# kiva12138/MIMRL

Hardware: AMD Instinct MI355X
Metric: two-stage train iters/sec (higher is better)
Workload: dtype bf16

## Files before the change

include/mimrl.h:

```cpp
#ifndef MIMRL_H_
#define MIMRL_H_

#include <stdint.h>

#ifdef __cplusplus
extern "C" {
#endif

#define MIMRL_ABI_VERSION 6
#define MIMRL_MAX_BLOCKS 4
#define MIMRL_MAX_BATCH 2048
#define MIMRL_MAX_BATCH_CONCAT 1024

enum { MIMRL_OK = 0, MIMRL_ERR_ARG = -1, MIMRL_ERR_HIP = -2, MIMRL_ERR_STATE = -3, MIMRL_ERR_NODEVICE = -4 };
enum { MIMRL_GROUP_MAIN = 0, MIMRL_GROUP_CRITIC = 1 };
enum { MIMRL_CRITIC_SEPARATE = 0, MIMRL_CRITIC_CONCAT = 1 };
enum { MIMRL_BOUND_INFONCE = 0, MIMRL_BOUND_NWJ, MIMRL_BOUND_TUBA, MIMRL_BOUND_DV, MIMRL_BOUND_JS_FGAN,
       MIMRL_BOUND_JS, MIMRL_BOUND_SMILE, MIMRL_BOUND_MINE, MIMRL_BOUND_INTERPOLATE };
enum { MIMRL_ACT_NONE = 0, MIMRL_ACT_RELU = 1, MIMRL_ACT_GELU = 2, MIMRL_ACT_TANH = 3 };
enum { MIMRL_PREC_FP32 = 0, MIMRL_PREC_BF16_GEMM_FWD = 1, MIMRL_PREC_BF16_GEMM_BWD = 2, MIMRL_PREC_BF16_GRU_FWD = 4,
       MIMRL_PREC_BF16_GRU_BWD = 8, MIMRL_PREC_BF16 = 15 };

enum { MIMRL_BASELINE_CONSTANT = 0, MIMRL_BASELINE_GAUSSAIN = 1, MIMRL_BASELINE_UNNORMALIZED = 2 };
enum { MIMRL_ENCODER_GRU = 0, MIMRL_ENCODER_CONV = 1, MIMRL_ENCODER_LSTM = 2 };
enum { MIMRL_TASK_LOSS_MAE = 0, MIMRL_TASK_LOSS_MSE = 1, MIMRL_TASK_LOSS_RMSE = 2, MIMRL_TASK_LOSS_SIMSE = 3, MIMRL_TASK_LOSS_CCC = 4 };

typedef struct mimrl_cfg {
  int32_t batch;
  int32_t seq_len;
  int32_t time_len;
  int32_t d_t, d_a, d_v;
  int32_t d_common;
  int32_t n_blocks;
  int32_t d_hiddens[MIMRL_MAX_BLOCKS][3];
  int32_t d_outs[MIMRL_MAX_BLOCKS][3];
  int32_t res_project[MIMRL_MAX_BLOCKS];
  int32_t bias, ln_first;
  int32_t activation;
  int32_t compose_t_sum, compose_k_sum;
  int32_t critic_type, bound_type;
  int32_t cmi_hardtanh;
  int32_t k_neighbor;
  int32_t bank_capacity;
  float dropout[4];
  float dropout_mlp[3];
  float coef1[11];
  float coef2[8];
  float weight_decay, grad_clip;
  float beta1, beta2, adam_eps;
  int32_t precision;
  int32_t use_graph;
  int32_t device_anchors;
  int32_t baseline_type;
  int32_t encoder;
  uint64_t seed;
} mimrl_cfg;

typedef struct mimrl_buffers {
  float *main_p, *main_g, *main_m, *main_v;
  float *crit_p, *crit_g, *crit_m, *crit_v;
  const float *text, *audio, *video, *labels;
  const float *bank_c, *bank_f, *bank_t, *bank_a, *bank_v;
  int32_t* anchors;
  float *lr_main, *lr_critic;
  float *pred;
  float *feats;
  float *scalars;
  const int32_t* knn_override;
  int32_t* counters;
} mimrl_buffers;

enum {
  MIMRL_S1_LOSS = 0,
  MIMRL_S1_MIS = 1,
  MIMRL_S1_LOSSES = 12,
  MIMRL_S2_LOSS = 32,
  MIMRL_S2_TASK = 33,
  MIMRL_S2_MIS = 34,
  MIMRL_S2_LOSSES = 42,
  MIMRL_NSCALARS = 64
};

const char* mimrl_last_error(void);
int mimrl_abi_version(void);
int mimrl_deterministic(void);
int mimrl_device_check(void);

int mimrl_layout_count(const mimrl_cfg* cfg);
int mimrl_layout_entry(const mimrl_cfg* cfg, int idx, char* name, int name_cap, int* group, int64_t* offset, int* ndim,
                       int* dim0, int* dim1);
int mimrl_layout_entry_dim2(const mimrl_cfg* cfg, int idx);
int64_t mimrl_bucket_floats(const mimrl_cfg* cfg, int group);

typedef struct mimrl_handle mimrl_handle;
int mimrl_create(const mimrl_cfg* cfg, void* hip_stream, mimrl_handle** out);
int mimrl_bind(mimrl_handle* h, const mimrl_buffers* bufs);
int mimrl_set_bank_rows(mimrl_handle* h, int rows);
int mimrl_set_inputs(mimrl_handle* h, int set, const float* text, const float* audio, const float* video, const float* labels);
int mimrl_stage1_pipe_prime(mimrl_handle* h);
int mimrl_stage1_pipe(mimrl_handle* h, int next_valid);
int mimrl_stage1_step(mimrl_handle* h);
int mimrl_stage2_step(mimrl_handle* h);
int mimrl_two_stage_step(mimrl_handle* h);
int mimrl_stage_grads(mimrl_handle* h, int stage);
int mimrl_stage_apply(mimrl_handle* h, int stage);
int mimrl_stage_grads_part(mimrl_handle* h, int stage, int part);
int mimrl_forward(mimrl_handle* h, int train_mode, int with_losses);
int mimrl_estimate(mimrl_handle* h, int stage);
int mimrl_set_stage2_prefetch(mimrl_handle* h, int on);
int mimrl_stage2_forward_tail(mimrl_handle* h);
int mimrl_set_grad_scale(mimrl_handle* h, float scale);
int mimrl_params_changed(mimrl_handle* h);
int64_t mimrl_workspace_bytes(const mimrl_handle* h);
enum { MIMRL_PH_GEMM_MISC = 0, MIMRL_PH_GRU_FWD, MIMRL_PH_GRU_BWD, MIMRL_PH_CUBE_FWD, MIMRL_PH_CUBE_BWD, MIMRL_PH_EST_FWD,
       MIMRL_PH_EST_BWD, MIMRL_PH_OPT, MIMRL_PH_MODEL_MISC, MIMRL_NPHASES };
int mimrl_profile_enable(mimrl_handle* h, int on);
int mimrl_set_kernel_stamps(mimrl_handle* h, unsigned long long* ring, int slots);
int mimrl_comm_unique_id(void* out128);
int mimrl_set_comm(mimrl_handle* h, const void* unique_id128, int world, int rank);
int64_t mimrl_main_late_offset(const mimrl_handle* h);
int mimrl_set_comm_critic_bf16(mimrl_handle* h, int on);
int mimrl_set_task_loss(mimrl_handle* h, int kind);
int mimrl_profile_read(mimrl_handle* h, float* ms_sum , int32_t* launches );
int mimrl_profile_read_gemm(mimrl_handle* h, double out[4]);
void mimrl_destroy(mimrl_handle* h);

int mimrl_op_gemm(void* stream, const float* A, const float* B, float* C, int M, int N, int K, int batch,
                  const int64_t strides[9] , const float* bias_n,
                  const float* bias_m, float alpha, float beta, int act, int precision);
int mimrl_op_gemm_ex(void* stream, const float* A, const float* B, float* C, int M, int N, int K, int batch, const int64_t strides[9],
                     const float* A2, const float* B2, int K2, const int64_t strides2[6], int a_gap_at, int a_gap_rows,
                     const float* bias_n, const float* gradact_u, float* colsum, int act, int precision);
int mimrl_op_gemm16(void* stream, const void* A, const void* B, void* C, int M, int N, int K, int batch, const int64_t strides[9],
                    const void* A2, const void* B2, int K2, const int64_t strides2[6], int batch_in, const int64_t strides_bo[5],
                    const float* bias_n, int flags);
int mimrl_op_gemm_wgrad_group(void* stream, int n, const float* const* A, const float* const* B, float* const* C, const int32_t* dims,
                              const int64_t* strides, int precision);
int64_t mimrl_op_gru_saved_floats(int B, int T);
int mimrl_op_gru_forward(void* stream, const float* gx_f, const float* gx_r, const float* whh_f, const float* whh_r,
                         const float* bhh_f, const float* bhh_r, const int32_t* lens, float* out, float* saved_f,
                         float* saved_r, int B, int T, int precision);
int mimrl_op_gru_backward(void* stream, const float* whh_f, const float* whh_r, const float* saved_f,
                          const float* saved_r, const int32_t* lens, const float* out, const float* dout, float* dg_f,
                          float* dg_r, float* hprev_f, float* hprev_r, int B, int T, int precision);
int mimrl_op_recur_btv(int B, int nmod);
int mimrl_op_lstm_forward(void* stream, const float* gx_f, const float* gx_r, const float* whh_f, const float* whh_r,
                          const float* bhh_f, const float* bhh_r, const int32_t* lens, float* out, float* saved_f,
                          float* saved_r, int B, int T, int kernel);
int mimrl_op_lstm_backward(void* stream, const float* whh_f, const float* whh_r, const float* saved_f,
                           const float* saved_r, const int32_t* lens, const float* out, const float* dout, float* dg_f,
                           float* dg_r, float* hprev_f, float* hprev_r, int B, int T, int kernel);
int mimrl_op_concat_dw(void* stream, const void* dz2, const void* a1, float* dw2, const void* dz1, const void* a0, float* dw1, int E, int64_t rows,
                       int64_t dw_stride, const float* ds, const void* a2h, float* dw3, const uint32_t* m2, const float* w3, const float* P,
                       const float* Q, int B);
int mimrl_op_gru_wgrad(void* stream, const void* const* dg, const void* const* x, const void* const* hp, float* const* dw_ih,
                       float* const* dw_hh, int64_t rows, int kp);
int mimrl_op_mi_bound(void* stream, const float* scores, float* dscores, float* mi, const float* gscale, int E, int B,
                      int bound);
int mimrl_op_mi_bound_ex(void* stream, const float* scores, float* dscores, float* mi, float* mi_loss, const float* gscale,
                         int E, int B, int bound, uint32_t lossform);
#define MIMRL_NCE_WS_FLOATS 2064
int mimrl_op_mi_infonce_rows(void* stream, const float* scores, float* dscores, float* mi, float* mi_loss, const float* gscale,
                             int E, int B, float* ws);
int mimrl_op_mi_bound_baseline(void* stream, float* scores, float* dscores, float* mi, const float* gscale, const float* lb,
                               float* dlb, int E, int B, int bound);
int mimrl_op_mi_sep_infonce(void* stream, const float* tout, float* dtout, float* mi, float* mi_loss, const float* gscale, int E,
                            int B, int tiled);
int mimrl_op_knn(void* stream, const float* Z, int dz, int N, const int32_t* anchors, int m, int k, int32_t* idx_out);
int mimrl_op_sample_anchors(void* stream, int32_t* anchors_out, int ncall, int m, int N, uint64_t seed, const int32_t* step,
                            uint32_t stream_id, int step_add);
int mimrl_knn_r1_host(const float* z, int N, const int32_t* anchors, int m, int k, int32_t* idx_out);
int mimrl_set_knn_override_mask(mimrl_handle* h, int stage, unsigned call_mask);
int mimrl_op_cmi_loss(void* stream, const float* logits, float* dlogits, float* bce, float* cmi, const float* g_bce,
                      const float* g_cmi, int E, int n, int hardtanh);
int mimrl_op_task_loss(void* stream, int kind, const float* pred, const float* y, float* dpred, float* loss, int B);
int mimrl_op_mlp_stack_forward(void* stream, int nb, int rows, int brows, int nl, const int32_t* dims, const float* const* W,
                               const float* const* b, int64_t pstride, const float* in, float* const* act, float* out);
int mimrl_op_mlp_stack_backward(void* stream, int nb, int rows, int brows, int nl, const int32_t* dims, const float* const* W,
                                int64_t pstride, const float* const* act, const float* dout, float* const* dz, float* din,
                                float* const* db);
int mimrl_probe_cube(mimrl_handle* h, const float* x, float* out, const float* dout, float* dx);
int mimrl_probe_encoders(mimrl_handle* h, float* cube_x, const float* dcube, const float* dmean);
int mimrl_probe_mi(mimrl_handle* h, int stage, float* mi, float* scores, float* dtin_out);
int mimrl_probe_cmi(mimrl_handle* h, int stage, const float* cmi_in, float* logits, float* vals, float* dcin_out);
int mimrl_probe_knn(mimrl_handle* h, int stage, int32_t* idx_out);
int mimrl_op_adam(void* stream, float* p, float* g, float* m, float* v, int64_t n, const float* lr, const int32_t* step,
                  float beta1, float beta2, float eps, float weight_decay, float clip);

#ifdef __cplusplus
}
#endif
#endif
```

mimrl_amd/_lib.py:

```python
from __future__ import annotations

import ctypes as C
import os
from typing import List, Tuple

_HERE = os.path.dirname(os.path.abspath(__file__))
DETERMINISTIC = os.environ.get("MIMRL_DETERMINISTIC", "0") not in ("", "0")
LIB_PATH = os.environ.get("MIMRL_LIB_PATH") or os.path.join(_HERE, "libmimrl_hip_det.so" if DETERMINISTIC else "libmimrl_hip.so")
MAX_BLOCKS = 4
MAX_BATCH = 2048
MAX_BATCH_CONCAT = 1024
NCE_WS_FLOATS = 2064
NSCALARS = 64
PHASES = ["gemm_misc", "gru_fwd", "gru_bwd", "cube_fwd", "cube_bwd", "est_fwd", "est_bwd", "opt", "model_misc"]
S1_LOSS, S1_MIS, S1_LOSSES, S2_LOSS, S2_TASK, S2_MIS, S2_LOSSES = 0, 1, 12, 32, 33, 34, 42

BOUNDS = {"infonce": 0, "nwj": 1, "tuba": 2, "dv": 3, "js_fgan": 4, "js": 5, "smile": 6, "mine": 7, "interpolate": 8}
ACTS = {"none": 0, "relu": 1, "gelu": 2, "tanh": 3}
PREC = {"fp32": 0, "bf16": 15, "bf16_gemm_fwd": 1, "bf16_gemm_bwd": 2, "bf16_gemm": 3, "bf16_gru": 12, "bf16_nogemmbwd": 13}


class MimrlError(RuntimeError):
    pass


class Cfg(C.Structure):
    _fields_ = [
        ("batch", C.c_int32), ("seq_len", C.c_int32), ("time_len", C.c_int32),
        ("d_t", C.c_int32), ("d_a", C.c_int32), ("d_v", C.c_int32), ("d_common", C.c_int32),
        ("n_blocks", C.c_int32),
        ("d_hiddens", (C.c_int32 * 3) * MAX_BLOCKS), ("d_outs", (C.c_int32 * 3) * MAX_BLOCKS),
        ("res_project", C.c_int32 * MAX_BLOCKS),
        ("bias", C.c_int32), ("ln_first", C.c_int32), ("activation", C.c_int32),
        ("compose_t_sum", C.c_int32), ("compose_k_sum", C.c_int32),
        ("critic_type", C.c_int32), ("bound_type", C.c_int32), ("cmi_hardtanh", C.c_int32),
        ("k_neighbor", C.c_int32), ("bank_capacity", C.c_int32),
        ("dropout", C.c_float * 4), ("dropout_mlp", C.c_float * 3),
        ("coef1", C.c_float * 11), ("coef2", C.c_float * 8),
        ("weight_decay", C.c_float), ("grad_clip", C.c_float),
        ("beta1", C.c_float), ("beta2", C.c_float), ("adam_eps", C.c_float),
        ("precision", C.c_int32), ("use_graph", C.c_int32), ("device_anchors", C.c_int32), ("baseline_type", C.c_int32),
        ("encoder", C.c_int32),
        ("seed", C.c_uint64),
    ]


_FP = C.c_void_p


class Buffers(C.Structure):
    _fields_ = [(n, _FP) for n in (
        "main_p", "main_g", "main_m", "main_v", "crit_p", "crit_g", "crit_m", "crit_v",
        "text", "audio", "video", "labels", "bank_c", "bank_f", "bank_t", "bank_a", "bank_v",
        "anchors", "lr_main", "lr_critic", "pred", "feats", "scalars", "knn_override", "counters")]


_lib = None


def load() -> C.CDLL:
    global _lib
    if _lib is not None:
        return _lib
    if not os.path.exists(LIB_PATH):
        raise MimrlError(f"{LIB_PATH} is missing: build it with `python -c 'import __graft_entry__ as g; g.build()'` "
                         f"or `make -C mimrl_amd/csrc` (hipcc --offload-arch=gfx950). There is no CPU fallback.")
    try:
        import torch
    except ImportError:
        pass
    lib = C.CDLL(LIB_PATH)
    if os.environ.get("MIMRL_LIB_PATH"):
        class _Partial:
            def __init__(self, lib):
                object.__setattr__(self, "_lib", lib)

            def __getattr__(self, name):
                try:
                    return getattr(self._lib, name)
                except AttributeError:
                    return type("_Missing", (), {})()
        real, lib = lib, _Partial(lib)
    lib.mimrl_last_error.restype = C.c_char_p
    lib.mimrl_bucket_floats.restype = C.c_int64
    lib.mimrl_workspace_bytes.restype = C.c_int64
    lib.mimrl_op_gru_saved_floats.restype = C.c_int64
    lib.mimrl_destroy.restype = None
    lib.mimrl_op_gemm.argtypes = [_FP, _FP, _FP, _FP, C.c_int, C.c_int, C.c_int, C.c_int, C.POINTER(C.c_int64), _FP, _FP,
                                  C.c_float, C.c_float, C.c_int, C.c_int]
    lib.mimrl_op_gemm_ex.argtypes = [_FP, _FP, _FP, _FP, C.c_int, C.c_int, C.c_int, C.c_int, C.POINTER(C.c_int64), _FP, _FP, C.c_int,
                                     C.POINTER(C.c_int64), C.c_int, C.c_int, _FP, _FP, _FP, C.c_int, C.c_int]
    lib.mimrl_comm_unique_id.argtypes = [_FP]
    lib.mimrl_set_comm.argtypes = [_FP, _FP, C.c_int, C.c_int]
    lib.mimrl_set_comm_critic_bf16.argtypes = [_FP, C.c_int]
    lib.mimrl_set_task_loss.argtypes = [_FP, C.c_int]
    lib.mimrl_op_task_loss.argtypes = [_FP, C.c_int, _FP, _FP, _FP, _FP, C.c_int]
    lib.mimrl_main_late_offset.argtypes = [_FP]
    lib.mimrl_main_late_offset.restype = C.c_int64
    lib.mimrl_op_gemm16.argtypes = [_FP, _FP, _FP, _FP, C.c_int, C.c_int, C.c_int, C.c_int, C.POINTER(C.c_int64), _FP, _FP, C.c_int,
                                    C.POINTER(C.c_int64), C.c_int, C.POINTER(C.c_int64), _FP, C.c_int]
    lib.mimrl_op_gemm_wgrad_group.argtypes = [_FP, C.c_int, C.POINTER(C.c_void_p), C.POINTER(C.c_void_p), C.POINTER(C.c_void_p),
                                              C.POINTER(C.c_int32), C.POINTER(C.c_int64), C.c_int]
    lib.mimrl_op_adam.argtypes = [_FP, _FP, _FP, _FP, _FP, C.c_int64, _FP, _FP, C.c_float, C.c_float, C.c_float,
                                  C.c_float, C.c_float]
    lib.mimrl_op_gru_forward.argtypes = [_FP] * 11 + [C.c_int, C.c_int, C.c_int]
    lib.mimrl_op_gru_backward.argtypes = [_FP] * 12 + [C.c_int, C.c_int, C.c_int]
    lib.mimrl_op_lstm_forward.argtypes = [_FP] * 11 + [C.c_int, C.c_int, C.c_int]
    lib.mimrl_op_lstm_backward.argtypes = [_FP] * 12 + [C.c_int, C.c_int, C.c_int]
    lib.mimrl_op_recur_btv.argtypes = [C.c_int, C.c_int]
    lib.mimrl_op_concat_dw.argtypes = [C.c_void_p] * 7 + [C.c_int, C.c_int64, C.c_int64] + [C.c_void_p] * 7 + [C.c_int]
    lib.mimrl_op_gru_wgrad.argtypes = [C.c_void_p] + [C.POINTER(C.c_void_p)] * 5 + [C.c_int64, C.c_int]
    lib.mimrl_op_mi_bound.argtypes = [_FP] * 5 + [C.c_int, C.c_int, C.c_int]
    lib.mimrl_op_mi_bound_ex.argtypes = [_FP] * 6 + [C.c_int, C.c_int, C.c_int, C.c_uint32]
    lib.mimrl_op_mi_infonce_rows.argtypes = [_FP] * 6 + [C.c_int, C.c_int, _FP]
    lib.mimrl_op_mi_sep_infonce.argtypes = [_FP] * 6 + [C.c_int, C.c_int, C.c_int]
    lib.mimrl_op_mi_bound_baseline.argtypes = [_FP] * 7 + [C.c_int, C.c_int, C.c_int]
    lib.mimrl_op_knn.argtypes = [_FP, _FP, C.c_int, C.c_int, _FP, C.c_int, C.c_int, _FP]
    lib.mimrl_op_cmi_loss.argtypes = [_FP] * 7 + [C.c_int, C.c_int, C.c_int]
    lib.mimrl_op_sample_anchors.argtypes = [_FP, _FP, C.c_int, C.c_int, C.c_int, C.c_uint64, _FP, C.c_uint32, C.c_int]
    lib.mimrl_create.argtypes = [C.POINTER(Cfg), _FP, C.POINTER(_FP)]
    lib.mimrl_bind.argtypes = [_FP, C.POINTER(Buffers)]
    lib.mimrl_profile_read.argtypes = [_FP, C.POINTER(C.c_float), C.POINTER(C.c_int32)]
    lib.mimrl_profile_read_gemm.argtypes = [_FP, C.POINTER(C.c_double)]
    for fn in ("mimrl_set_bank_rows", "mimrl_stage_grads", "mimrl_stage_grads_part", "mimrl_stage_apply", "mimrl_estimate", "mimrl_profile_enable", "mimrl_set_stage2_prefetch"):
        getattr(lib, fn).argtypes = [_FP, C.c_int]
    lib.mimrl_set_grad_scale.argtypes = [_FP, C.c_float]
    lib.mimrl_stage_grads_part.argtypes = [_FP, C.c_int, C.c_int]
    lib.mimrl_set_inputs.argtypes = [_FP, C.c_int, _FP, _FP, _FP, _FP]
    lib.mimrl_knn_r1_host.argtypes = [_FP, C.c_int, _FP, C.c_int, C.c_int, _FP]
    lib.mimrl_set_knn_override_mask.argtypes = [_FP, C.c_int, C.c_uint]
    for fn in ("mimrl_stage1_step", "mimrl_stage2_step", "mimrl_two_stage_step", "mimrl_destroy", "mimrl_workspace_bytes", "mimrl_params_changed",
               "mimrl_stage2_forward_tail"):
        getattr(lib, fn).argtypes = [_FP]
    lib.mimrl_forward.argtypes = [_FP, C.c_int, C.c_int]
    lib.mimrl_set_kernel_stamps.argtypes = [_FP, _FP, C.c_int]
    lib.mimrl_probe_cube.argtypes = [_FP] * 5
    lib.mimrl_probe_mi.argtypes = [_FP, C.c_int, _FP, _FP, _FP]
    lib.mimrl_probe_cmi.argtypes = [_FP, C.c_int, _FP, _FP, _FP, _FP]
    lib.mimrl_probe_knn.argtypes = [_FP, C.c_int, _FP]
    lib.mimrl_probe_encoders.argtypes = [_FP] * 4
    lib.mimrl_layout_count.argtypes = [C.POINTER(Cfg)]
    lib.mimrl_layout_entry_dim2.argtypes = [C.POINTER(Cfg), C.c_int]
    lib.mimrl_bucket_floats.argtypes = [C.POINTER(Cfg), C.c_int]
    lib.mimrl_layout_entry.argtypes = [C.POINTER(Cfg), C.c_int, C.c_char_p, C.c_int, C.POINTER(C.c_int),
                                       C.POINTER(C.c_int64), C.POINTER(C.c_int), C.POINTER(C.c_int), C.POINTER(C.c_int)]
    if os.environ.get("MIMRL_LIB_PATH"):
        lib = real
    _lib = lib
    return lib


ENCODERS = {"gru": 0, "conv": 1, "lstm": 2}
BASELINES = {"constant": 0, "gaussain": 1, "unnormalized": 2}

EXPORTS = [
    "mimrl_last_error", "mimrl_abi_version", "mimrl_deterministic", "mimrl_device_check", "mimrl_layout_count", "mimrl_layout_entry", "mimrl_layout_entry_dim2",
    "mimrl_bucket_floats", "mimrl_create", "mimrl_bind", "mimrl_set_bank_rows", "mimrl_set_inputs", "mimrl_stage1_step", "mimrl_stage2_step", "mimrl_two_stage_step",
    "mimrl_stage_grads", "mimrl_stage_grads_part", "mimrl_stage_apply", "mimrl_forward", "mimrl_estimate", "mimrl_profile_enable", "mimrl_profile_read", "mimrl_profile_read_gemm",
    "mimrl_workspace_bytes", "mimrl_params_changed", "mimrl_set_stage2_prefetch", "mimrl_stage2_forward_tail", "mimrl_set_grad_scale", "mimrl_destroy", "mimrl_op_gemm", "mimrl_op_gemm_ex", "mimrl_op_gemm16", "mimrl_op_gemm_wgrad_group",
    "mimrl_op_gru_saved_floats", "mimrl_op_gru_forward", "mimrl_op_gru_backward", "mimrl_op_gru_wgrad", "mimrl_op_concat_dw", "mimrl_op_mi_bound", "mimrl_op_mi_bound_ex", "mimrl_op_mi_bound_baseline", "mimrl_op_mi_sep_infonce", "mimrl_op_knn",
    "mimrl_op_cmi_loss", "mimrl_op_sample_anchors", "mimrl_knn_r1_host", "mimrl_set_knn_override_mask", "mimrl_op_mlp_stack_forward", "mimrl_op_mlp_stack_backward", "mimrl_op_adam",
    "mimrl_probe_cube", "mimrl_probe_mi", "mimrl_probe_cmi", "mimrl_probe_knn", "mimrl_probe_encoders", "mimrl_set_kernel_stamps", "mimrl_comm_unique_id", "mimrl_set_comm", "mimrl_main_late_offset", "mimrl_set_comm_critic_bf16",
    "mimrl_stage1_pipe_prime", "mimrl_stage1_pipe", "mimrl_set_task_loss", "mimrl_op_task_loss",
    "mimrl_op_mi_infonce_rows", "mimrl_op_lstm_forward", "mimrl_op_lstm_backward", "mimrl_op_recur_btv",
]

TASK_LOSSES = {"MAE": 0, "MSE": 1, "RMSE": 2, "SIMSE": 3, "CCC": 4}
BATCH_COUPLED_LOSSES = ("RMSE", "SIMSE", "CCC")


def task_loss_code(opt, world: int = 1) -> int:
    loss = getattr(opt, "loss", "MAE")
    if loss in ("Focal", "CE", "BCE"):
        raise NotImplementedError(f"--loss {loss}: classification losses are not on the MI355X path (regression only: "
                                  f"{', '.join(TASK_LOSSES)})")
    if loss not in TASK_LOSSES:
        raise NotImplementedError(f"--loss {loss}: unknown task loss (choose one of {', '.join(TASK_LOSSES)})")
    if int(world) > 1 and loss in BATCH_COUPLED_LOSSES:
        raise NotImplementedError(f"--loss {loss} couples the whole batch: with {int(world)} ranks each would see only its shard, not the "
                                  f"reference's global batch; run it on one rank, or use MAE / MSE")
    return TASK_LOSSES[loss]


def check(rc: int) -> int:
    if rc < 0:
        raise MimrlError(f"libmimrl_hip error {rc}: {load().mimrl_last_error().decode()}")
    return rc


def make_cfg(opt, d_t: int, d_a: int, d_v: int, seq_len: int = None, bank_capacity: int = 0, precision: str = "fp32",
             use_graph: bool = False, seed: int = 0, device_anchors: bool = False, batch: int = None) -> Cfg:
    c = Cfg()
    c.batch = int(batch if batch is not None else opt.batch_size)
    c.time_len = int(opt.time_len)
    c.seq_len = int(seq_len if seq_len is not None else opt.time_len)
    c.d_t, c.d_a, c.d_v, c.d_common = int(d_t), int(d_a), int(d_v), int(opt.d_common)
    enc = getattr(opt, "encoders", "gru")
    if enc not in ENCODERS:
        raise MimrlError(f"--encoders {enc}: choose gru, conv or lstm (Model.py:237)")
    c.encoder = ENCODERS[enc]
    nb = len(opt.d_hiddens)
    if nb > MAX_BLOCKS or len(opt.d_outs) != nb or len(opt.res_project) != nb:
        raise MimrlError("d_hiddens / d_outs / res_project must have the same length (<= 4)")
    c.n_blocks = nb
    for i in range(nb):
        for ax in range(3):
            c.d_hiddens[i][ax] = int(opt.d_hiddens[i][ax])
            c.d_outs[i][ax] = int(opt.d_outs[i][ax])
        c.res_project[i] = int(bool(opt.res_project[i]))
    c.bias, c.ln_first = int(bool(opt.bias)), int(bool(opt.ln_first))
    if opt.activate not in ACTS:
        raise MimrlError(f"--activate {opt.activate} not supported on the HIP path (gelu/relu/tanh)")
    c.activation = ACTS[opt.activate]
    for name, attr in (("features_compose_t", "compose_t_sum"), ("features_compose_k", "compose_k_sum")):
        v = getattr(opt, name, "mean")
        if v not in ("mean", "sum"):
            raise MimrlError(f"--{name} {v}: only mean/sum supported")
        setattr(c, attr, int(v == "sum"))
    if opt.critic_type not in ("separate", "concat"):
        raise NotImplementedError(opt.critic_type)
    c.critic_type = 0 if opt.critic_type == "separate" else 1
    bl = getattr(opt, "baseline_type", "constant")
    if bl not in BASELINES:
        raise NotImplementedError(f"--baseline_type {bl}")
    c.baseline_type = BASELINES[bl]
    if opt.bound_type not in BOUNDS:
        raise NotImplementedError(opt.bound_type)
    c.bound_type = BOUNDS[opt.bound_type]
    if opt.cmi_last_acticate not in ("sigmoid", "hardtanh"):
        raise NotImplementedError(opt.cmi_last_acticate)
    c.cmi_hardtanh = int(opt.cmi_last_acticate == "hardtanh")
    c.k_neighbor = int(opt.k_neighbor)
    c.bank_capacity = int(bank_capacity)
    for i in range(4):
        c.dropout[i] = float(opt.dropout[i])
    for i in range(3):
        c.dropout_mlp[i] = float(opt.dropout_mlp[i])
    if len(opt.loss_mi_coefficient1) != 11 or len(opt.loss_mi_coefficient2) != 8:
        raise MimrlError("loss_mi_coefficient1/2 need 11 / 8 entries")
    for i in range(11):
        c.coef1[i] = float(opt.loss_mi_coefficient1[i])
    for i in range(8):
        c.coef2[i] = float(opt.loss_mi_coefficient2[i])
    c.weight_decay, c.grad_clip = float(opt.weight_decay), float(opt.gradient_clip)
    c.beta1, c.beta2, c.adam_eps = 0.9, 0.999, 1e-8
    c.precision = PREC[precision]
    c.use_graph = int(bool(use_graph))
    c.device_anchors = int(bool(device_anchors))
    c.seed = int(seed) & 0xFFFFFFFFFFFFFFFF
    return c


def layout_entries(cfg: Cfg) -> Tuple[List[Tuple[str, int, int, Tuple[int, ...]]], Tuple[int, int]]:
    lib = load()
    n = check(lib.mimrl_layout_count(C.byref(cfg)))
    out = []
    name = C.create_string_buffer(256)
    g, nd, d0, d1 = C.c_int(), C.c_int(), C.c_int(), C.c_int()
    off = C.c_int64()
    for i in range(n):
        check(lib.mimrl_layout_entry(C.byref(cfg), i, name, 256, C.byref(g), C.byref(off), C.byref(nd), C.byref(d0), C.byref(d1)))
        shape = (d0.value, d1.value) if nd.value == 2 else (d0.value,)
        if nd.value == 3:
            shape = (d0.value, d1.value, check(lib.mimrl_layout_entry_dim2(C.byref(cfg), i)))
        out.append((name.value.decode(), g.value, off.value, shape))
    sizes = (check(lib.mimrl_bucket_floats(C.byref(cfg), 0)), check(lib.mimrl_bucket_floats(C.byref(cfg), 1)))
    return out, sizes


def knn_r1_host(z, anchors, k: int):
    import numpy as np
    z = np.ascontiguousarray(np.asarray(z, dtype=np.float32).reshape(-1))
    a = np.ascontiguousarray(np.asarray(anchors, dtype=np.int32).reshape(-1))
    if int(k) >= (len(z) - len(a)) // 2:
        return None
    out = np.empty((len(a), int(k)), dtype=np.int32)
    check(load().mimrl_knn_r1_host(z.ctypes.data_as(C.c_void_p), len(z), a.ctypes.data_as(C.c_void_p), len(a), int(k),
                                   out.ctypes.data_as(C.c_void_p)))
    return out
```

mimrl_amd/csrc/cube_bwd_fused.h:

```cpp
#pragma once
#include "common.h"
#include "model_ops.h"

namespace mimrl {

struct LAxisBwdArgs {
  const float *dz, *y, *mean, *rstd, *gamma;
  const float* u;
  const float *w2, *w1, *wr;
  float *dy, *du, *dx;
  float *db2, *db1;
  int B, il, hl, ol, C, act;
};
bool laxis_bwd_supported(int il, int hl, int ol, int C);
int laxis_bwd_fused(hipStream_t s, const LAxisBwdArgs& a);

struct DAxisBwdArgs {
  const float *dz, *y, *mean, *rstd, *gamma;
  const float* u;
  const __bf16 *w2t, *w1t, *wrt;
  float *dy, *du, *dx;
  long R;
  int act;
  float *dgamma, *dbeta, *db2, *db1;
};
bool daxis_bwd_supported(int id, int hd, int od);
int daxis_bwd_fused(hipStream_t s, const DAxisBwdArgs& a);

struct WtTransposeArgs { const float* src[12]; __bf16* dst[12]; int n; };
int wt_transpose_bf16(hipStream_t s, const WtTransposeArgs& a);

int daxis_param_grads(hipStream_t s, const float* y, const float* mean, const float* rstd, const float* dz, const float* dy,
                      const float* du, float* dgamma, float* dbeta, float* db2, float* db1, long R);

#ifdef MIMRL_PHASE_PROBE
int cube_bwd_read_phases(long long* out);
#endif

}
```

mimrl_amd/csrc/cube_bwd_fused.hip:

```cpp
#include "cube_bwd_fused.h"
#include "kmix_device.h"

namespace mimrl {

namespace {

#ifdef MIMRL_PHASE_PROBE
__device__ long long g_cbwd_phase[64];
#define BPHASE(base, i) do { if (blockIdx.x == 0 && blockIdx.y == 0 && threadIdx.x == 0) g_cbwd_phase[(base) + (i)] = (long long)wall_clock64(); } while (0)
#else
#define BPHASE(base, i) do { } while (0)
#endif

constexpr int CT = 128;
constexpr int KP = 64 + 8;


template <bool LONG = false>
__global__ __launch_bounds__(256, LONG ? 2 : 1) void laxis_bwd_kernel(LAxisBwdArgs a) {
  __shared__ __attribute__((aligned(16))) __bf16 sdyu[2][CT][KP];
  auto& sdy = sdyu[0];
  auto& sdu = sdyu[1];
  __shared__ __attribute__((aligned(16))) __bf16 wts[3][64][KP];
  float (*red)[2][CT] = reinterpret_cast<float (*)[2][CT]>(&sdu[0][0]);
// ... 242 lines not shown
  const long r0 = (long)blockIdx.x * DR;
  const bool pg = a.dgamma != nullptr;
  const int pb = gridDim.x <= 200 ? 32 : 48;
  BPHASE(pb, 0);
  if (pg) for (int i = tid; i < 3 * 128; i += 256) (&spg[0][0])[i].zero();
  const int row1 = tid >> 3, part1 = tid & 7;
  const long r1 = r0 + row1;
  const bool ok1 = r1 < a.R;
  const long rc1 = ok1 ? r1 : a.R - 1;
  const float mu1 = a.mean[rc1], rs1 = a.rstd[rc1];
  float4 gz4[4], yv4[4];
#pragma unroll
  for (int q = 0; q < 4; ++q) {
    gz4[q] = *reinterpret_cast<const float4*>(a.dz + rc1 * 128 + part1 * 16 + q * 4);
    yv4[q] = *reinterpret_cast<const float4*>(a.y + rc1 * 128 + part1 * 16 + q * 4);
  }
  const int n = wave * 32 + lr;
  bf16x8 bw2[8], bw1[8], bwr[8];
#pragma unroll
  for (int ks = 0; ks < 8; ++ks) {
    bw2[ks] = *reinterpret_cast<const bf16x8*>(a.w2t + n * 128 + ks * 16 + 8 * lh);
    bw1[ks] = *reinterpret_cast<const bf16x8*>(a.w1t + n * 128 + ks * 16 + 8 * lh);
    bwr[ks] = *reinterpret_cast<const bf16x8*>(a.wrt + n * 128 + ks * 16 + 8 * lh);
  }
  float uu[16];
#pragma unroll
  for (int r = 0; r < 16; ++r) {
    const long row = min(r0 + (r & 3) + 8 * (r >> 2) + 4 * lh, a.R - 1);
    uu[r] = a.u[row * 128 + n];
  }
  BPHASE(pb, 1);
  {
    const int row = row1, part = part1;
    const long r = r1;
    const bool ok = ok1;
    float g[16], xh[16], dyk[16];
    float s1 = 0.f, s2 = 0.f;
    const float mu = mu1, rs = rs1;
#pragma unroll
    for (int q = 0; q < 4; ++q) {
      const float4 gz = gz4[q];
      const float4 yv = yv4[q];
      const float gg[4] = {gz.x, gz.y, gz.z, gz.w}, yy[4] = {yv.x, yv.y, yv.z, yv.w};
#pragma unroll
      for (int j = 0; j < 4; ++j) {
        g[q * 4 + j] = gg[j];
        xh[q * 4 + j] = (yy[j] - mu) * rs;
        const float dxh = gg[j] * a.gamma[part * 16 + q * 4 + j];
        s1 += dxh; s2 += dxh * xh[q * 4 + j];
      }
    }
    s1 = group_sum<8>(s1); s2 = group_sum<8>(s2);
    s1 *= (1.f / 128.f); s2 *= (1.f / 128.f);
#pragma unroll
    for (int q = 0; q < 4; ++q) {
      float v[4];
#pragma unroll
      for (int j = 0; j < 4; ++j) {
        const int c = part * 16 + q * 4 + j;
        v[j] = rs * (g[q * 4 + j] * a.gamma[c] - s1 - xh[q * 4 + j] * s2);
      }
      if (ok) *reinterpret_cast<float4*>(a.dy + r * 128 + part * 16 + q * 4) = make_float4(v[0], v[1], v[2], v[3]);
      bf16x4 p; p[0] = to_bf16(v[0]); p[1] = to_bf16(v[1]); p[2] = to_bf16(v[2]); p[3] = to_bf16(v[3]);
      *reinterpret_cast<bf16x4*>(&sdy[row][part * 16 + q * 4]) = p;
      if (pg) {
#pragma unroll
        for (int j = 0; j < 4; ++j) { const float gz = ok ? g[q * 4 + j] : 0.f; xh[q * 4 + j] *= gz; g[q * 4 + j] = gz; v[j] = ok ? v[j] : 0.f; }
        dyk[q * 4 + 0] = v[0]; dyk[q * 4 + 1] = v[1]; dyk[q * 4 + 2] = v[2]; dyk[q * 4 + 3] = v[3];
      }
    }
    if (pg) {
      __syncthreads();
#pragma unroll
      for (int j = 0; j < 16; ++j) {
        float sa = xh[j], sb = g[j], sc = dyk[j];
#pragma unroll
        for (int o = 8; o < 64; o <<= 1) { sa += __shfl_xor(sa, o, 64); sb += __shfl_xor(sb, o, 64); sc += __shfl_xor(sc, o, 64); }
        if (lane < 8) { spg[0][part * 16 + j].add(sa); spg[1][part * 16 + j].add(sb); spg[2][part * 16 + j].add(sc); }
      }
    }
  }
  __syncthreads();
  BPHASE(pb, 2);
  {
    f32x16 acc;
#pragma unroll
    for (int r = 0; r < 16; ++r) acc[r] = 0.f;
#pragma unroll
    for (int ks = 0; ks < 8; ++ks) {
      const bf16x8 af = *reinterpret_cast<const bf16x8*>(&sdy[lr][ks * 16 + 8 * lh]);
      acc = __builtin_amdgcn_mfma_f32_32x32x16_bf16(af, bw2[ks], acc, 0, 0, 0);
    }
    float csum = 0.f;
    act_dispatch(a.act, [&](auto AT) __attribute__((always_inline)) {
#pragma unroll
    for (int r = 0; r < 16; ++r) {
      const int m = (r & 3) + 8 * (r >> 2) + 4 * lh;
      const long row = r0 + m;
      float v = 0.f;
      if (row < a.R) {
        v = acc[r] * act_grad_c<decltype(AT)::value>(a.act, uu[r]);
        a.du[row * 128 + n] = v;
      }
      sdu[m][n] = to_bf16(v);
      csum += v;
    }
    });
    if (pg) {
      csum += __shfl_xor(csum, 32, 64);
      if (lh == 0) acc_add(&a.db1[n], csum);
    }
  }
  __syncthreads();
  BPHASE(pb, 3);
  if (pg && tid < 128) {
    acc_add(&a.dgamma[tid], spg[0][tid].get());
    acc_add(&a.dbeta[tid], spg[1][tid].get());
    acc_add(&a.db2[tid], spg[2][tid].get());
  }
  {
    f32x16 acc;
#pragma unroll
    for (int r = 0; r < 16; ++r) acc[r] = 0.f;
#pragma unroll
    for (int ks = 0; ks < 8; ++ks) {
      const bf16x8 a1 = *reinterpret_cast<const bf16x8*>(&sdu[lr][ks * 16 + 8 * lh]);
      acc = __builtin_amdgcn_mfma_f32_32x32x16_bf16(a1, bw1[ks], acc, 0, 0, 0);
      const bf16x8 a2 = *reinterpret_cast<const bf16x8*>(&sdy[lr][ks * 16 + 8 * lh]);
      acc = __builtin_amdgcn_mfma_f32_32x32x16_bf16(a2, bwr[ks], acc, 0, 0, 0);
    }
#pragma unroll
    for (int r = 0; r < 16; ++r) {
      const long row = r0 + (r & 3) + 8 * (r >> 2) + 4 * lh;
      if (row < a.R) a.dx[row * 128 + n] = acc[r];
    }
  }
  BPHASE(pb, 4);
}

__global__ void wt_transpose_kernel(WtTransposeArgs a) {
  __shared__ float t[32][33];
  const float* __restrict__ src = a.src[blockIdx.z];
  __bf16* __restrict__ dst = a.dst[blockIdx.z];
  const int k0 = blockIdx.y * 32, n0 = blockIdx.x * 32, tx = threadIdx.x & 31, ty = threadIdx.x >> 5;
  for (int j = ty; j < 32; j += 8) t[j][tx] = src[(k0 + j) * 128 + n0 + tx];
  __syncthreads();
  for (int j = ty; j < 32; j += 8) dst[(n0 + j) * 128 + k0 + tx] = to_bf16(t[tx][j]);
}

__global__ __launch_bounds__(256) void daxis_param_grads_kernel(const float* __restrict__ y, const float* __restrict__ mean,
                                                                const float* __restrict__ rstd, const float* __restrict__ dz,
                                                                const float* __restrict__ dy, const float* __restrict__ du,
                                                                float* __restrict__ dgamma, float* __restrict__ dbeta,
                                                                float* __restrict__ db2, float* __restrict__ db1, long R) {
  __shared__ float4 red[4][8][32];
  const int cq = threadIdx.x & 31, rl = threadIdx.x >> 5;
  const long r0 = (long)blockIdx.x * 64;
  float4 a0 = make_float4(0.f, 0.f, 0.f, 0.f), a1 = a0, a2 = a0, a3 = a0;
#pragma unroll
  for (int i = 0; i < 8; ++i) {
    const long r = r0 + rl + 8 * i;
    const long rc = r < R ? r : R - 1;
    const float m = r < R ? 1.f : 0.f;
    const float mu = mean[rc], rs = rstd[rc] * m;
    const float4 g = *reinterpret_cast<const float4*>(dz + rc * 128 + cq * 4);
    const float4 yv = *reinterpret_cast<const float4*>(y + rc * 128 + cq * 4);
    const float4 v = *reinterpret_cast<const float4*>(dy + rc * 128 + cq * 4);
    const float4 u = *reinterpret_cast<const float4*>(du + rc * 128 + cq * 4);
    a0.x += g.x * (yv.x - mu) * rs; a0.y += g.y * (yv.y - mu) * rs; a0.z += g.z * (yv.z - mu) * rs; a0.w += g.w * (yv.w - mu) * rs;
    a1.x += g.x * m; a1.y += g.y * m; a1.z += g.z * m; a1.w += g.w * m;
    a2.x += v.x * m; a2.y += v.y * m; a2.z += v.z * m; a2.w += v.w * m;
    a3.x += u.x * m; a3.y += u.y * m; a3.z += u.z * m; a3.w += u.w * m;
  }
  red[0][rl][cq] = a0; red[1][rl][cq] = a1; red[2][rl][cq] = a2; red[3][rl][cq] = a3;
  __syncthreads();
#pragma unroll
  for (int h = 0; h < 2; ++h) {
    const int idx = threadIdx.x + 256 * h, q = idx >> 7, c = idx & 127;
    const float* base = reinterpret_cast<const float*>(&red[q][0][0]);
    float sum = 0.f;
#pragma unroll
    for (int j = 0; j < 8; ++j) sum += base[j * 128 + c];
    float* dst = q == 0 ? dgamma : (q == 1 ? dbeta : (q == 2 ? db2 : db1));
    if (dst) acc_add(&dst[c], sum);
  }
}

}

int daxis_param_grads(hipStream_t s, const float* y, const float* mean, const float* rstd, const float* dz, const float* dy,
                      const float* du, float* dgamma, float* dbeta, float* db2, float* db1, long R) {
  if (R <= 0) return MIMRL_OK;
  hipLaunchKernelGGL(daxis_param_grads_kernel, dim3((unsigned)((R + 63) / 64)), dim3(256), 0, s, y, mean, rstd, dz, dy, du, dgamma, dbeta,
                     db2, db1, R);
  LAUNCH_CHECK();
  return MIMRL_OK;
}

bool daxis_bwd_supported(int id, int hd, int od) { return id == 128 && hd == 128 && od == 128; }

int daxis_bwd_fused(hipStream_t s, const DAxisBwdArgs& a) {
  if (!a.w2t || !a.w1t || !a.wrt) return set_error(MIMRL_ERR_ARG, "daxis_bwd_fused: needs the transposed weight images");
  if ((a.dgamma || a.dbeta || a.db2 || a.db1) && !(a.dgamma && a.dbeta && a.db2 && a.db1))
    return set_error(MIMRL_ERR_ARG, "daxis_bwd_fused: the four parameter-gradient outputs come together");
  hipLaunchKernelGGL(daxis_bwd_kernel, dim3((unsigned)((a.R + DR - 1) / DR)), dim3(256), 0, s, a);
  LAUNCH_CHECK();
  return MIMRL_OK;
}

int wt_transpose_bf16(hipStream_t s, const WtTransposeArgs& a) {
  if (a.n < 1 || a.n > 12) return set_error(MIMRL_ERR_ARG, "wt_transpose_bf16: 1..12 matrices");
  hipLaunchKernelGGL(wt_transpose_kernel, dim3(4, 4, a.n), dim3(256), 0, s, a);
  LAUNCH_CHECK();
  return MIMRL_OK;
}

}
```

mimrl_amd/csrc/det.hip:

```cpp
#include <atomic>
#include <cstring>
#include <mutex>
#include <vector>

#include "common.h"

namespace mimrl {

#ifdef MIMRL_DET
namespace {
constexpr unsigned kSlots = 1u << 23;
DetCtx h_ctx = {};
std::atomic<bool> ready{false};
bool failed = false;
std::mutex mu;
std::vector<DetSetter>& setters() { static std::vector<DetSetter> v; return v; }

__global__ __launch_bounds__(256) void det_flush_kernel(DetCtx c) {
  const unsigned n = __atomic_load_n(&c.ctl[0], __ATOMIC_RELAXED);
  const unsigned nb = min(gridDim.x, (n + 255u) / 256u);
  if (blockIdx.x >= nb) return;
  for (unsigned i = blockIdx.x * blockDim.x + threadIdx.x; i < n; i += nb * blockDim.x) {
    const unsigned h = c.list[i];
    float* p = reinterpret_cast<float*>(c.keys[h]);
    *p += (float)c.vals[h] * kDetInv;
    c.keys[h] = 0ull;
    c.vals[h] = 0ll;
  }
  __threadfence();
  __syncthreads();
  if (threadIdx.x == 0 && atomicAdd(&c.ctl[1], 1u) == nb - 1) { c.ctl[1] = 0u; __threadfence(); c.ctl[0] = 0u; }
}
}

void det_register_tu(DetSetter f) { setters().push_back(f); }

int det_init() {
  if (ready.load(std::memory_order_acquire)) return MIMRL_OK;
  std::lock_guard<std::mutex> g(mu);
  if (ready.load() || failed) return failed ? MIMRL_ERR_HIP : MIMRL_OK;
  failed = true;
  HIPX(hipMalloc(&h_ctx.keys, sizeof(unsigned long long) * kSlots));
  HIPX(hipMalloc(&h_ctx.vals, sizeof(long long) * kSlots));
  HIPX(hipMalloc(&h_ctx.list, sizeof(unsigned) * kSlots));
  HIPX(hipMalloc(&h_ctx.ctl, sizeof(unsigned) * 4));
  HIPX(hipMemset(h_ctx.keys, 0, sizeof(unsigned long long) * kSlots));
  HIPX(hipMemset(h_ctx.vals, 0, sizeof(long long) * kSlots));
  HIPX(hipMemset(h_ctx.ctl, 0, sizeof(unsigned) * 4));
  h_ctx.mask = kSlots - 1;
  for (DetSetter f : setters()) f(h_ctx);
  HIPX(hipDeviceSynchronize());
  HIPX(hipGetLastError());
  failed = false;
  ready.store(true, std::memory_order_release);
  return MIMRL_OK;
}

int det_flush(hipStream_t s) {
  if (!ready.load(std::memory_order_acquire)) return MIMRL_OK;
  det_flush_kernel<<<dim3(256), dim3(256), 0, s>>>(h_ctx);
  return MIMRL_OK;
}

namespace {
thread_local bool t_no_flush = false;
thread_local bool t_defer = false, t_pending = false, t_gemm_in_bucket = false;
thread_local const DetRanges* t_ranges = nullptr;
}
bool det_target_in_bucket(const void* p) {
  const char* c = static_cast<const char*>(p);
  if (!t_ranges) return false;
  for (int i = 0; i < t_ranges->n; ++i)
    if (t_ranges->lo[i] && c >= static_cast<const char*>(t_ranges->lo[i]) && c < static_cast<const char*>(t_ranges->lo[i]) + t_ranges->bytes[i]) return true;
  return false;
}
DetGemmTarget::DetGemmTarget(const void* c) : prev_(t_gemm_in_bucket) { t_gemm_in_bucket = det_target_in_bucket(c); }
DetGemmTarget::~DetGemmTarget() { t_gemm_in_bucket = prev_; }
DetDefer::DetDefer(hipStream_t s, const DetRanges* r) : s_(s), prev_(t_defer), prev_r_(t_ranges) { t_defer = true; t_ranges = r; }
DetDefer::~DetDefer() {
  t_defer = prev_;
  t_ranges = prev_r_;
  if (!t_defer && t_pending) { t_pending = false; (void)det_flush(s_); }
}
DetNoFlush::DetNoFlush(bool on) : on_(on), prev_(t_no_flush) { if (on_) t_no_flush = true; }
DetNoFlush::~DetNoFlush() { if (on_) t_no_flush = prev_; }

bool det_launch_accumulates(const char* name) {
  if (t_no_flush) return false;
  if (t_defer) {
    static const char* const kBucketOnly[] = {"ln_relu_drop_bwd", "head_bwd_kernel", "colln_bwd_kernel", "rowln_bwd_kernel", "kmix_bwd_kernel",
                                              "colsum_kernel", "rowsum_batched", "colln_param_grads", "daxis_param_grads",
                                              "laxis_bwd_kernel", "daxis_bwd_kernel", "gru_bwd_kernel", "top1_bwd_kernel", "concat_dw3_kernel",
                                              "mlp_frag_kernel", "gemm_group_kernel", "gemm_groupk_kernel"};
    for (const char* k : kBucketOnly)
      if (std::strstr(name, k)) { t_pending = true; return false; }
    if (t_gemm_in_bucket && std::strstr(name, "gemm_")) { t_pending = true; return false; }
  }
  static const char* const kSafe[] = {"_fwd", "adam_kernel", "images_kernel", "bf16_image", "knn_", "sample_anchors", "seq_lengths", "l0_pack", "l0_unpack",
                                      "text_post", "feat_mean", "tail_pre", "begin_stage", "task_loss_kernel", "finalize_stage", "stage_boundary",
                                      "cmi_assemble", "copy_rows", "gather_sum4", "wt_transpose", "pad_rows", "mi_bound", "cmi_loss", "pair_expand",
                                      "pair_reduce", "gauss_baseline", "dbg_spin", "det_flush", "dropout_inplace", "add_inplace",
                                      "mi_sep_fused", "gemm_tall_kernel", "concat_ws_reduce"};
  for (const char* k : kSafe)
    if (std::strstr(name, k)) return false;
  return true;
}

int det_overflowed() {
  if (!ready.load()) return 0;
  unsigned f[2] = {0, 0};
  if (hipMemcpy(f, h_ctx.ctl + 2, sizeof f, hipMemcpyDeviceToHost) != hipSuccess) return 1;
  return (f[0] != 0 ? 1 : 0) | (f[1] != 0 ? 2 : 0);
}
#endif

}

extern "C" int mimrl_deterministic(void) {
#ifdef MIMRL_DET
  const int f = ::mimrl::det_overflowed();
  return 1 | ((f & 1) ? 2 : 0) | ((f & 2) ? 4 : 0);
#else
  return 0;
#endif
}
```

mimrl_amd/csrc/engine.h:

```cpp
#pragma once
#include <cstdio>
#include <cstdlib>
#include <cstring>
#include <algorithm>
#include <vector>
#include <dlfcn.h>

#include "cube_fused.h"
#include "mlp_fused.h"
#include "concat_fused.h"
#include "cube_bwd_fused.h"
#include "cube_long.h"
#include "estimator_ops.h"
#include "gemm.h"
#include "gru.h"
#include "gru_wgrad.h"
#include "concat_dw.h"
#include "lstm.h"
#include "layout.h"
#include "comm.h"
#include "model_ops.h"

namespace mimrl {

namespace eng {


constexpr int H = 128, G = 384, HID = 256, EMB = 128;
constexpr int NE_MI = 5, NE_CMI = 6;
constexpr int ACT_SLACK = 4 * MLPF_MAX_WIDTH;

enum { FT_F = 0, FT_T = 1, FT_A = 2, FT_V = 3, FT_C = 4 };
const int kMiWire[NE_MI][2] = {{FT_F, FT_T}, {FT_F, FT_A}, {FT_F, FT_V}, {FT_T, FT_A}, {FT_T, FT_V}};
const int kCmiWire[NE_CMI][3] = {{FT_A, FT_C, FT_T}, {FT_T, FT_A, FT_C}, {FT_V, FT_C, FT_T},
                                 {FT_T, FT_V, FT_C}, {FT_T, FT_C, FT_A}, {FT_T, FT_C, FT_V}};
static const char* const kVmi[NE_MI] = {"f_t", "f_a", "f_v", "t_a", "t_v"};
static const char* const kVcmi[NE_CMI] = {"ac_t", "ta_c", "vc_t", "tv_c", "tc_a", "tc_v"};

void launch_begin_stage(hipStream_t s, int* rng_step, int* adam_step, float* scalars, int scal_off, int scal_n);
void launch_bucket_to_bf16(hipStream_t s, const float* src, void* dst, long n);
void launch_bucket_from_bf16(hipStream_t s, const void* src, float* dst, long n);
void launch_task_loss(hipStream_t s, int kind, const float* pred, const float* y, float* dpred, float* task, int B);
void launch_finalize_stage1(hipStream_t s, float* scal, const float* mi, const float* cmi, const float* bce, const float* coef1);
void launch_finalize_stage2(hipStream_t s, float* scal, const float* mi, const float* cmi, const float* coef2, int have_mi);
void launch_stage_boundary(hipStream_t s, float* scal, const float* mi, const float* cmi, const float* bce, const float* coef1, int* rng_step,
                           int* adam_step, const float* pred, const float* y, float* dpred, int B, int kind);

struct Roctx {
  int (*push)(const char*) = nullptr;
  int (*pop)() = nullptr;
  Roctx() {
    void* h = dlopen("librocprofiler-sdk-roctx.so", RTLD_LAZY | RTLD_LOCAL);
    if (!h) h = dlopen("librocprofiler-sdk-roctx.so.1", RTLD_LAZY | RTLD_LOCAL);
    if (!h) h = dlopen("libroctx64.so", RTLD_LAZY | RTLD_LOCAL);
    if (!h) h = dlopen("libroctx64.so.4", RTLD_LAZY | RTLD_LOCAL);
    if (h) {
      push = reinterpret_cast<int (*)(const char*)>(dlsym(h, "roctxRangePushA"));
      pop = reinterpret_cast<int (*)()>(dlsym(h, "roctxRangePop"));
      if (!push || !pop) push = nullptr;
    }
  }
};
inline Roctx& roctx() { static Roctx r; return r; }
struct Range {
  bool on;
  explicit Range(const char* name) : on(roctx().push != nullptr) { if (on) roctx().push(name); }
  ~Range() { if (on) roctx().pop(); }
};

struct Lin { long w = -1, b = -1; int out = 0, in = 0; };
struct GruDirW { long w_ih = 0, w_hh = 0, b_ih = 0, b_hh = 0; int din = 0; };
struct AxisW { Lin fc1, fc2; long res = -1, ln_g = -1, ln_b = -1; int in = 0, hid = 0, out = 0; };
struct BlockW { AxisW ax[3]; };
struct MixBuf { float *xn = nullptr, *xn_mean = nullptr, *xn_rstd = nullptr, *u = nullptr, *h = nullptr, *y = nullptr,
                      *z = nullptr, *mean = nullptr, *rstd = nullptr; };
struct BlockBuf { MixBuf l, k, d; };

}

using namespace eng;

}

using namespace mimrl;

struct mimrl_handle {
  mimrl_cfg cfg;
  hipStream_t stream = nullptr;
  hipStream_t user_stream = nullptr;
  hipStream_t cap_stream = nullptr;
  Layout layout;
  mimrl_buffers bufs;
  bool bound = false;
  DetRanges det_ranges;
  float* nce_ws = nullptr;
  bool grads_clean[3] = {true, true, true};
  int bank_rows = 0;
  bool bf16 = false;
  int prec = 0;

  GruDirW gru[2][2][2];
  long ln_g[2], ln_b[2], w_t;
  BlockW blk[MIMRL_MAX_BLOCKS];
  long cls_w, cls_b;
  __bf16 *crit_img = nullptr, *crit_imgT = nullptr;
  __bf16 *crit_frag = nullptr, *crit_fragT = nullptr;
  FragTable ftab;
  bool frag_side_pending = false;
  bool frag_tr_deferred = false;
  FragTable ftab_tr;
  bool adam_frag_on = true;
  bool boundary_in_adam = false;
  bool img_valid = false;
  unsigned knn_ovr_mask[2] = {0u, 0u};
  bool knn_pre = true;
  bool mi_fused_bwd_done = false;
  bool imgT_ready = false;
  TransposeTable ttab;
  int ensure_images() {
    if (img_valid || !crit_img) return MIMRL_OK;
    MX(bf16_image(user_stream, bufs.crit_p, crit_img, layout.floats[MIMRL_GROUP_CRITIC]));
    if (crit_frag && ftab.n > 0) MX(bf16_frag_images(user_stream, bufs.crit_p, crit_frag, ftab));
    img_valid = true;
    return MIMRL_OK;
  }
  long bl0 = 0, bl_stride = 0, bl_l[4][2];
  float *lbv = nullptr, *dlbv = nullptr, *bact[3] = {nullptr, nullptr, nullptr}, *bdz[3] = {nullptr, nullptr, nullptr}, *bdin = nullptr;
  bool has_baseline() const {
    return cfg.baseline_type != MIMRL_BASELINE_CONSTANT && (cfg.bound_type == MIMRL_BOUND_TUBA || cfg.bound_type == MIMRL_BOUND_INTERPOLATE);
  }
  int baseline_forward();
  int baseline_backward(int stage);
  long tower0 = 0, tower_stride = 0;
  long tower_l[4][2];
  long cmi0 = 0, cmi_stride = 0, cmi_l[4][2];

  char* ws = nullptr;
  size_t ws_bytes = 0, ws_used = 0;
  int* d_ints = nullptr;
  int* d_ints_own = nullptr;
  float* d_consts = nullptr;
  int *lens[2] = {nullptr, nullptr};
  bool kmix_pg_on_side3 = false;
  bool begin_in_pack = false;
  hipEvent_t ev_lens = nullptr;
  float *tx_raw = nullptr, *gx[2][2], *h0[2], *h1[2], *sv[2][2][2], *ln_mean[2], *ln_rstd[2];
  float* tailp_part = nullptr;
  bool pre_done = false;
  int dual_tail_pre();
  float* cube0 = nullptr;
  float *xpack = nullptr, *wpack = nullptr, *bpack = nullptr, *dwih_pack = nullptr, *dwhh_pack = nullptr;
  _Float16* h0h[2] = {nullptr, nullptr}; _Float16* w1h = nullptr; __bf16* w1b = nullptr;
  __bf16* w1bt = nullptr;
  bool h16_on = true;
  float* w2p[MIMRL_MAX_BLOCKS] = {};
  bool w2p_valid[MIMRL_MAX_BLOCKS] = {};
  bool xin_on = true;
  bool part0_done = false;
  bool l0_xin = false;
  bool xpack16 = false;
  bool laxis_bwd_long_on = true;
  bool laxis_long_on = true;
  bool rec16_on = true, dwih_h16_on = true;
  bool hp16_live = false;
  bool dh0_bf16_live = false, ds_bf16_live = false;
  bool h16_live = false;
  bool w1_img_valid = false;
  int KP() const { return ((cfg.d_a > cfg.d_v ? cfg.d_a : cfg.d_v) + 15) & ~15; }
  bool dg_bf16 = false;
  bool concat_compact = false;
  bool a0_regen_live = false;
  bool fused_concat = true;
  bool l0_packed = false;
  bool l0_bwd_pack = false;
  BlockBuf bb[MIMRL_MAX_BLOCKS];
  __bf16* wtT[MIMRL_MAX_BLOCKS][3] = {};
  struct FwdSet {
    int* lens[2] = {nullptr, nullptr};
    float *tx_raw = nullptr, *gx[2][2] = {{nullptr, nullptr}, {nullptr, nullptr}}, *h0[2] = {nullptr, nullptr}, *h1[2] = {nullptr, nullptr};
    float *ln_mean[2] = {nullptr, nullptr}, *ln_rstd[2] = {nullptr, nullptr}, *cube0 = nullptr, *feats = nullptr, *pred = nullptr;
    _Float16* h0h[2] = {nullptr, nullptr};
    BlockBuf bb[MIMRL_MAX_BLOCKS];
  } alt;
  void swap_fwd_set() {
    for (int m = 0; m < 2; ++m) {
      std::swap(lens[m], alt.lens[m]); std::swap(h0[m], alt.h0[m]); std::swap(h1[m], alt.h1[m]); std::swap(h0h[m], alt.h0h[m]);
      std::swap(ln_mean[m], alt.ln_mean[m]); std::swap(ln_rstd[m], alt.ln_rstd[m]);
      for (int d = 0; d < 2; ++d) std::swap(gx[m][d], alt.gx[m][d]);
    }
    std::swap(tx_raw, alt.tx_raw); std::swap(cube0, alt.cube0);
    std::swap(bufs.feats, alt.feats); std::swap(bufs.pred, alt.pred);
    for (int i = 0; i < MIMRL_MAX_BLOCKS; ++i) std::swap(bb[i], alt.bb[i]);
  }
  bool prefetch = false;
  bool defer_tail = false;
  bool tail2_needed = false;
  bool fwd2_pending = false;
  float grad_scale = 1.f;
  void* comm = nullptr; int comm_world = 1, comm_rank = 0;
  bool comm_crit_bf16 = false; void* comm_crit16 = nullptr;
  int task_loss = MIMRL_TASK_LOSS_MAE;
  hipStream_t comm_s = nullptr;
  bool comm_split = true;
  KernelStamp kstamp;

  int run_fwd2_tail();
  hipStream_t pre_stream = nullptr;
  int carve_fwd(size_t* gmax_out);
  float *ff = nullptr, *dpred = nullptr;
  float *tin = nullptr, *ta[3], *tout = nullptr, *scores = nullptr, *dscores = nullptr;
  float *cP = nullptr, *cQ = nullptr, *ca[3];
  int split_part = 0;
  bool fold_unpack = false, unpack_pending = false;
  bool fold_unpack_on = true;
  bool gx_f16 = false;
  int *knn_idx = nullptr, *knn_idx2 = nullptr;
  int knn_flip = 0;
  int knn_slot(int stage) const { return (stage - 1) ^ knn_flip; }
  char* knn_scr[2] = {nullptr, nullptr};
  size_t knn_scr_bytes = 0;
  float *cmi_in = nullptr, *cc[3], *logits = nullptr, *dlogits = nullptr;
  float *mi_raw = nullptr, *cmi_raw = nullptr, *bce_raw = nullptr;
  float *dfeat = nullptr, *dtout = nullptr, *dta[3], *dtin = nullptr, *dca[3], *dP = nullptr, *dQ = nullptr;
  float *dcc[3], *dcin = nullptr;
  static constexpr int NGBUF = 24;
  float* gbuf[NGBUF];
  size_t gbuf_floats = 0;
  float *dtx = nullptr, *ds[2], *dg[2][2][2], *hprev[2][2][2], *dh0[2];

  static constexpr int NSIDE = 6;
  hipStream_t side[NSIDE] = {nullptr, nullptr, nullptr, nullptr, nullptr, nullptr};
  std::vector<hipEvent_t> ev_pool;
  size_t ev_next = 0;
  bool multi_stream = true;
  bool fused_cube_bwd = true;
  bool fused_mlp = true;
  bool fused_cube = true;
  int fwd_f16 = 1;
  int next_event(hipEvent_t* e) {
    if (ev_next == ev_pool.size()) {
      hipEvent_t n;
      HIPX(hipEventCreateWithFlags(&n, hipEventDisableTiming));
      ev_pool.push_back(n);
    }
    *e = ev_pool[ev_next++];
    return MIMRL_OK;
  }
  int G_group(hipStream_t st, const GemmDesc* ds, int n) {
    if (!prof_on) return gemm_group(st, ds, n, bf16);
    for (int i = 0; i < n; ++i) MX(G_on(st, ds[i]));
    return MIMRL_OK;
  }
  unsigned side_mask = ~0u;
  bool side_on(int i) const { return multi_stream && ((side_mask >> i) & 1u); }
  hipStream_t S(int i) const { return side_on(i) ? side[i] : stream; }
  int fork(int lo, int hi) {
    if (!multi_stream) return MIMRL_OK;
    hipEvent_t e = nullptr;
    for (int i = lo; i <= hi; ++i) {
      if (!side_on(i)) continue;
      if (!e) { MX(next_event(&e)); HIPX(hipEventRecord(e, stream)); }
      HIPX(hipStreamWaitEvent(side[i], e, 0));
    }
    return MIMRL_OK;
  }
  int join(int lo, int hi) {
    if (!multi_stream) return MIMRL_OK;
    for (int i = lo; i <= hi; ++i) {
      if (!side_on(i)) continue;
      hipEvent_t e;
      MX(next_event(&e));
      HIPX(hipEventRecord(e, side[i]));
      HIPX(hipStreamWaitEvent(stream, e, 0));
    }
    return MIMRL_OK;
  }
  int chain(int i, int j) {
    if (!multi_stream || S(i) == S(j)) return MIMRL_OK;
    hipEvent_t e;
    MX(next_event(&e));
    HIPX(hipEventRecord(e, S(j)));
    HIPX(hipStreamWaitEvent(S(i), e, 0));
    return MIMRL_OK;
  }
  int reduce_bucket(int stage) {
    if (!comm) return MIMRL_OK;
    Range rg(stage == 1 ? "mimrl.stage1.allreduce(crit_g) [RCCL]" : "mimrl.stage2.allreduce(main_g) [RCCL]");
    if (stage == 1 && comm_crit_bf16) {
      const long n = layout.floats[MIMRL_GROUP_CRITIC];
      launch_bucket_to_bf16(stream, bufs.crit_g, comm_crit16, n);
      LAUNCH_CHECK();
      MX(comm_allreduce_sum_bf16(comm, comm_crit16, (size_t)n, stream));
      launch_bucket_from_bf16(stream, comm_crit16, bufs.crit_g, n);
      LAUNCH_CHECK();
      return MIMRL_OK;
    }
    return comm_allreduce_sum(comm, stage == 1 ? bufs.crit_g : bufs.main_g, (size_t)layout.floats[stage == 1 ? MIMRL_GROUP_CRITIC : MIMRL_GROUP_MAIN], stream);
  }
  int enqueue_grads2_reduced(bool skip_zero);
  struct GemmProf { hipEvent_t a, b; double flops, bytes; };
  std::vector<GemmProf> prof_gemm;
  int G_on(hipStream_t st, const GemmDesc& d) {
    if (!prof_on) return gemm(st, d, bf16);
    GemmProf g;
    if (!prof_pool.empty()) { g.a = prof_pool.back().first; g.b = prof_pool.back().second; prof_pool.pop_back(); }
    else { HIPX(hipEventCreate(&g.a)); HIPX(hipEventCreate(&g.b)); }
    auto distinct = [&](long s_b, long s_bo) -> double {
      if (d.batch_in > 0) return (double)(s_bo != 0 ? d.batch / d.batch_in : 1) * (s_b != 0 ? d.batch_in : 1);
      return s_b != 0 ? d.batch : 1;
    };
    g.flops = 2.0 * d.M * d.N * ((double)d.K + (d.A2 ? d.K2 : 0)) * d.batch;
    const double ea = d.a_bf16 ? 2.0 : 4.0, eb = d.b_bf16 ? 2.0 : 4.0;
    g.bytes = ea * d.M * d.K * distinct(d.sa_b, d.sa_bo) + eb * d.K * d.N * distinct(d.sb_b, d.sb_bo) +
              4.0 * d.M * d.N * distinct(d.sc_b, d.sc_bo) * ((d.beta != 0.f || d.atomic) ? 2 : 1);
    if (d.A2) g.bytes += ea * d.M * d.K2 * (d.sa2_b ? d.batch : 1) + eb * d.K2 * d.N * (d.sb2_b ? d.batch : 1);
    HIPX(hipEventRecord(g.a, st));
    const int r = gemm(st, d, bf16);
    HIPX(hipEventRecord(g.b, st));
    prof_gemm.push_back(g);
    return r;
  }

  bool prof_on = false;
  std::vector<std::pair<hipEvent_t, hipEvent_t>> prof_ev[MIMRL_NPHASES];
  std::vector<std::pair<hipEvent_t, hipEvent_t>> prof_pool;
  struct Scope {
    mimrl_handle* h; int ph; hipEvent_t a = nullptr, b = nullptr;
    Scope(mimrl_handle* h_, int ph_) : h(h_), ph(ph_) {
      if (!h->prof_on) return;
      if (!h->prof_pool.empty()) { a = h->prof_pool.back().first; b = h->prof_pool.back().second; h->prof_pool.pop_back(); }
      else { (void)hipEventCreate(&a); (void)hipEventCreate(&b); }
      (void)hipEventRecord(a, h->stream);
    }
    ~Scope() {
      if (!a) return;
      (void)hipEventRecord(b, h->stream);
      h->prof_ev[ph].push_back({a, b});
    }
  };

  struct GraphSet {
    hipGraphExec_t graph[3][4] = {{nullptr, nullptr, nullptr, nullptr}, {nullptr, nullptr, nullptr, nullptr}, {nullptr, nullptr, nullptr, nullptr}};
    int rows[3][4] = {{-1, -1, -1, -1}, {-1, -1, -1, -1}, {-1, -1, -1, -1}};
    hipGraphExec_t tail = nullptr; int tail_rows = -1;
    hipGraphExec_t pipe[2][4] = {{nullptr, nullptr, nullptr, nullptr}, {nullptr, nullptr, nullptr, nullptr}};
    int pipe_rows[2][4] = {{-1, -1, -1, -1}, {-1, -1, -1, -1}};
    const void* in[4] = {nullptr, nullptr, nullptr, nullptr};
  } gsets[2];
  int cur_set = 0;
  GraphSet& GS() { return gsets[cur_set]; }
  std::vector<hipGraphExec_t> retired;
  void retire(hipGraphExec_t& ex) { if (ex) { retired.push_back(ex); ex = nullptr; } }
  void drop_graphs(int set = -1) {
    for (int q = 0; q < 2; ++q) {
      if (set >= 0 && q != set) continue;
      for (int s = 0; s <= 2; ++s)
        for (int k = 0; k < 4; ++k) retire(gsets[q].graph[s][k]);
      retire(gsets[q].tail);
      for (int a_ = 0; a_ < 2; ++a_) for (int b_ = 0; b_ < 4; ++b_) retire(gsets[q].pipe[a_][b_]);
    }
  }
  float* P(long off) const { return bufs.main_p + off; }
  float* Gm(long off) const { return bufs.main_g + off; }
  float* CP(long off) const { return bufs.crit_p + off; }
  float* CG(long off) const { return bufs.crit_g + off; }
  long conv_w[2] = {0, 0}, conv_b[2] = {0, 0};
  int encoders_forward(bool save, int knn_stage);
  int conv_forward(int knn_stage);
  int conv_backward();
  int lstm_encoders_forward(bool save, int knn_stage);
  int lstm_encoders_backward();
  int rng_add = 0;
  RngKey key() const { return RngKey{(uint32_t)cfg.seed, (uint32_t)(cfg.seed >> 32), d_ints, rng_add}; }
  const float* coef1() const { return d_consts; }
  const float* coef2() const { return d_consts + 11; }
  const float* gs_mi(int stage) const { return d_consts + 19 + (stage - 1) * 5; }
  const float* g_bce(int stage) const { return d_consts + 29 + (stage - 1) * 6; }
  const float* g_cmi(int stage) const { return d_consts + 41 + (stage - 1) * 6; }
  int nprod() const { return (cfg.batch / cfg.k_neighbor) * cfg.k_neighbor; }
  int m_anchor() const { return cfg.batch / cfg.k_neighbor; }

  int resolve();
  int alloc_workspace();
  template <typename T>
  int take(T** p, size_t count) {
    const size_t bytes = (count * sizeof(T) + 255) / 256 * 256;
    if (ws) {
      if (ws_used + bytes > ws_bytes) return set_error(MIMRL_ERR_STATE, "workspace overflow");
      *p = reinterpret_cast<T*>(ws + ws_used);
    }
    ws_used += bytes;
    return MIMRL_OK;
  }
  int carve();

  int G_(const GemmDesc& d) { return G_on(stream, d); }
  static constexpr bool fp32_site(int) { return false; }
  struct PrecGuard {
    mimrl_handle* h; bool saved;
    PrecGuard(mimrl_handle* h_, bool force_fp32) : h(h_), saved(h_->bf16) { if (force_fp32) h->bf16 = false; }
    ~PrecGuard() { h->bf16 = saved; }
  };
  struct Deferred { int kind; int side; GemmDesc g; const float* src; long n0, n1, n2, n3; float* dst;
                    const float *p1 = nullptr, *p2 = nullptr, *p3 = nullptr; float* dst2 = nullptr; KMixW kw = KMixW();
                    const float *p4 = nullptr, *p5 = nullptr; float *dst3 = nullptr, *dst4 = nullptr; };
  std::vector<Deferred> deferred;
  int flush_deferred(int only_side = 0);
  int wg_helper = -1;
  int dbg_delay(hipStream_t st, int tag);
  int model_forward(bool train, bool save, int knn_stage = 0, int part = 0);
  int cube_forward(bool train, bool save);
  int cube_backward(int cur_in, int* cur_out);
  int wt_images(hipStream_t st, bool bwd_bf16, bool launch, bool* d_fused);
  int model_backward();
  int encoders_backward(float* dcube);
  int gru_layer_backward(int l);
  struct StreamGuard {
    mimrl_handle* h; hipStream_t saved;
    StreamGuard(mimrl_handle* h_, hipStream_t st) : h(h_), saved(h_->stream) { h->stream = st; }
    ~StreamGuard() { h->stream = saved; }
  };
  int knn_launch(int stage, hipStream_t st);
  bool pipe_primed = false; int fwd_parity = 0, pipe_set = 0;
  int pipe_forward_body(bool other_inputs);
  int run_stage1_pipe_prime();
  int run_stage1_pipe(bool next_valid);
  int mi_forward(int stage, bool want_grad);
  int cmi_forward(int stage, bool want_grad);
  int mi_backward(int stage);
  int cmi_backward(int stage);
  int route_feature_grads();
  GatherSum head_gather;
  bool head_gather_on = false;
  hipEvent_t ev_dmean = nullptr;
  int estimators_all(int stage, bool want_grad, bool backward);
  int mlp_stack_forward(int nb, int rows, int brows, long p0, long pstride, int nl, const long (*l_off)[2], const int* dims,
                        const float* in, float* const* act, float* out);
  int mlp_stack_backward(int nb, int rows, int brows, long p0, long pstride, int nl, const long (*l_off)[2],
                         const int* dims, const float* in, float* const* act, float* dout, float* const* dtmp, float* din,
                         bool wgrad);
  int enqueue_grads(int stage, bool skip_zero = false);
  int enqueue_apply(int stage);
  int run(int stage, int kind);
  int run_step();
  bool keep_events = false;
  bool fuse_boundary = false;
  bool imgT_valid = false;
  bool skip_imgT_refresh = false;
  bool wtT_prebuilt = false;
  bool wtT_built = false;
};
```

mimrl_amd/csrc/engine_abi.hip:

```cpp
#include "engine.h"

extern "C" {

const char* mimrl_last_error(void) { return mimrl::last_error_slot().c_str(); }
#ifdef MIMRL_PHASE_PROBE
int mimrl_dbg_cube_phases(long long* out) { return mimrl::cube_fwd_read_phases(out); }
int mimrl_dbg_cube_bwd_phases(long long* out) { return mimrl::cube_bwd_read_phases(out); }
int mimrl_dbg_kmix_phases(long long* out) { return mimrl::kmix_bwd_read_phases(out); }
int mimrl_dbg_nce_phases(long long* out) { return mimrl::nce_read_phases(out); }
int mimrl_dbg_model_ops_phases(long long* out) { return mimrl::model_ops_read_phases(out); }
int mimrl_dbg_gru_bwd_phases(long long* out) { return mimrl::gru_bwd_read_phases(out); }
int mimrl_dbg_concat_bwd_phases(long long* out) { return mimrl::concat_bwd_read_phases(out); }
#endif
int mimrl_abi_version(void) { return MIMRL_ABI_VERSION; }

int mimrl_device_check(void) {
  int n = 0;
  if (hipGetDeviceCount(&n) != hipSuccess || n <= 0) return set_error(MIMRL_ERR_NODEVICE, "no HIP device visible");
  int dev = 0;
  if (hipGetDevice(&dev) != hipSuccess) return set_error(MIMRL_ERR_NODEVICE, "hipGetDevice failed");
  hipDeviceProp_t p;
  if (hipGetDeviceProperties(&p, dev) != hipSuccess) return set_error(MIMRL_ERR_NODEVICE, "hipGetDeviceProperties failed");
  if (std::strncmp(p.gcnArchName, "gfx950", 6) != 0)
    return set_error(MIMRL_ERR_NODEVICE, "device %d is %s; this library is built for gfx950 (MI355X) only", dev, p.gcnArchName);
  return MIMRL_OK;
}

int mimrl_create(const mimrl_cfg* cfg, void* hip_stream, mimrl_handle** out) {
  if (!cfg || !out) return set_error(MIMRL_ERR_ARG, "null argument");
  *out = nullptr;
  MX(validate_cfg(*cfg));
  if (cfg->batch > MIMRL_MAX_BATCH)
    return set_error(MIMRL_ERR_ARG, "batch per rank %d exceeds MIMRL_MAX_BATCH (%d)", cfg->batch, MIMRL_MAX_BATCH);
  if (cfg->critic_type == MIMRL_CRITIC_CONCAT && cfg->batch > MIMRL_MAX_BATCH_CONCAT)
    return set_error(MIMRL_ERR_ARG, "batch per rank %d exceeds MIMRL_MAX_BATCH_CONCAT (%d): the concat critic's pair activations "
                     "grow as B^2 (6 x 5 x B^2 x 256 floats)", cfg->batch, MIMRL_MAX_BATCH_CONCAT);
#ifndef MIMRL_DEBUG_KNOBS
  for (int i = 0; kDebugKnobs[i]; ++i)
    if (getenv(kDebugKnobs[i]))
      return set_error(MIMRL_ERR_ARG, "%s is set, but result-changing debug knobs are compiled out of this build "
                       "(rebuild with `make DEBUG_KNOBS=1` for timing experiments; never for real runs)", kDebugKnobs[i]);
#endif
  MX(mimrl_device_check());
  if (knob_on("MIMRL_KNOBS")) knobs_print(stderr);
  mimrl_handle* h = new (std::nothrow) mimrl_handle();
  if (!h) return set_error(MIMRL_ERR_STATE, "out of host memory");
  h->cfg = *cfg;
  if (h->cfg.beta1 == 0.f) h->cfg.beta1 = 0.9f;
  if (h->cfg.beta2 == 0.f) h->cfg.beta2 = 0.999f;
  if (h->cfg.adam_eps == 0.f) h->cfg.adam_eps = 1e-8f;
  h->stream = h->user_stream = reinterpret_cast<hipStream_t>(hip_stream);
  h->multi_stream = knob("MIMRL_SINGLE_STREAM") == nullptr;
#ifdef MIMRL_DET
  h->multi_stream = false;
  MX(det_init());
#endif
  h->fused_cube = knob("MIMRL_NO_FUSED_CUBE") == nullptr;
  h->fused_mlp = knob("MIMRL_NO_FUSED_MLP") == nullptr;
  h->knn_pre = true;
  h->fold_unpack_on = knob("MIMRL_NO_FOLD_UNPACK") == nullptr;
  h->h16_on = knob("MIMRL_NO_H16") == nullptr;
  h->xin_on = knob("MIMRL_NO_XIN") == nullptr;
  h->fused_cube_bwd = knob("MIMRL_NO_FUSED_CUBE_BWD") == nullptr;
  h->laxis_bwd_long_on = !(knob("MIMRL_LAXIS_BWD_LONG") && atoi(knob("MIMRL_LAXIS_BWD_LONG")) == 0);
  h->laxis_long_on = !(knob("MIMRL_LAXIS_LONG") && atoi(knob("MIMRL_LAXIS_LONG")) == 0);
  h->rec16_on = !(knob("MIMRL_REC16") && atoi(knob("MIMRL_REC16")) == 0);
  h->dwih_h16_on = !(knob("MIMRL_DWIH_H16") && atoi(knob("MIMRL_DWIH_H16")) == 0);
  h->adam_frag_on = !(knob("MIMRL_ADAM_FRAG") && atoi(knob("MIMRL_ADAM_FRAG")) == 0);
  h->fused_concat = knob("MIMRL_NO_FUSED_CONCAT") == nullptr;
  h->fwd_f16 = knob("MIMRL_FWD_BF16") == nullptr;
  h->l0_packed = knob("MIMRL_L0_PACK") ? atoi(knob("MIMRL_L0_PACK")) != 0 : true;
  h->dg_bf16 = cfg->encoder == MIMRL_ENCODER_GRU && (cfg->precision & MIMRL_PREC_BF16_GRU_BWD) && (cfg->precision & MIMRL_PREC_BF16_GEMM_BWD) &&
               knob("MIMRL_DG_FP32") == nullptr;
  h->l0_bwd_pack = false;
  {
    const bool can = cfg->encoder == MIMRL_ENCODER_GRU && (cfg->precision & MIMRL_PREC_BF16_GRU_FWD) && (cfg->precision & MIMRL_PREC_BF16_GEMM_FWD);
    h->gx_f16 = can && knob("MIMRL_GX_F16") && atoi(knob("MIMRL_GX_F16")) != 0;
  }
  if (cfg->encoder == MIMRL_ENCODER_GRU && ((cfg->precision & MIMRL_PREC_BF16_GRU_FWD) != 0) != ((cfg->precision & MIMRL_PREC_BF16_GRU_BWD) != 0)) {
    mimrl_destroy(h);
    return set_error(MIMRL_ERR_ARG, "MIMRL_PREC_BF16_GRU_FWD and MIMRL_PREC_BF16_GRU_BWD must be set together");
  }
  for (int i = 0; i < mimrl_handle::NSIDE; ++i)
    if (hipStreamCreateWithFlags(&h->side[i], hipStreamNonBlocking) != hipSuccess) { mimrl_destroy(h); return set_error(MIMRL_ERR_HIP, "hipStreamCreate failed"); }
  gru_probe_setup();
  h->prec = cfg->precision;
  h->bf16 = (h->prec & MIMRL_PREC_BF16_GEMM_FWD) != 0;
  std::memset(&h->bufs, 0, sizeof h->bufs);
  int r = build_layout(h->cfg, &h->layout);
  if (r == 0) r = h->resolve();
  if (r == 0) r = h->alloc_workspace();
  if (r != 0) { mimrl_destroy(h); return r; }
  *out = h;
  return MIMRL_OK;
}

int mimrl_bind(mimrl_handle* h, const mimrl_buffers* b) {
  if (!h || !b) return set_error(MIMRL_ERR_ARG, "null argument");
  const void* need[] = {b->main_p, b->main_g, b->main_m, b->main_v, b->crit_p, b->crit_g, b->crit_m, b->crit_v,
                        b->text, b->audio, b->video, b->labels, b->lr_main, b->lr_critic, b->pred, b->feats, b->scalars};
  for (const void* p : need)
    if (!p) return set_error(MIMRL_ERR_ARG, "mimrl_bind: a required buffer is null");
  h->bufs = *b;
  h->bound = true;
  {
    h->det_ranges.lo[0] = b->main_g; h->det_ranges.lo[1] = b->crit_g;
    h->det_ranges.bytes[0] = sizeof(float) * (size_t)h->layout.floats[MIMRL_GROUP_MAIN];
    h->det_ranges.bytes[1] = sizeof(float) * (size_t)h->layout.floats[MIMRL_GROUP_CRITIC];
    h->det_ranges.n = 2;
  }
  h->part0_done = false;
  h->cur_set = 0;
  for (int q = 0; q < 2; ++q) for (int i = 0; i < 4; ++i) h->gsets[q].in[i] = nullptr;
  h->gsets[0].in[0] = b->text; h->gsets[0].in[1] = b->audio; h->gsets[0].in[2] = b->video; h->gsets[0].in[3] = b->labels;
  h->img_valid = false;
  h->imgT_valid = false;
  h->d_ints = b->counters ? b->counters : h->d_ints_own;
  h->drop_graphs();
  return MIMRL_OK;
}

int mimrl_set_inputs(mimrl_handle* h, int set, const float* text, const float* audio, const float* video, const float* labels) {
  if (!h || set < 0 || set > 1 || !text || !audio || !video || !labels) return set_error(MIMRL_ERR_ARG, "mimrl_set_inputs: bad argument");
  if (!h->bound) return set_error(MIMRL_ERR_STATE, "mimrl_bind must be called first");
  const void* p[4] = {text, audio, video, labels};
  mimrl_handle::GraphSet& g = h->gsets[set];
  if (g.in[0] && (g.in[0] != p[0] || g.in[1] != p[1] || g.in[2] != p[2] || g.in[3] != p[3])) {
    HIPX(hipStreamSynchronize(h->user_stream));
    h->drop_graphs(set);
  }
  for (int i = 0; i < 4; ++i) g.in[i] = p[i];
  h->cur_set = set;
  h->part0_done = false;
  h->bufs.text = text; h->bufs.audio = audio; h->bufs.video = video; h->bufs.labels = labels;
  return MIMRL_OK;
}

int mimrl_stage1_pipe_prime(mimrl_handle* h) { return h ? h->run_stage1_pipe_prime() : set_error(MIMRL_ERR_ARG, "null handle"); }
int mimrl_stage1_pipe(mimrl_handle* h, int next_valid) { return h ? h->run_stage1_pipe(next_valid != 0) : set_error(MIMRL_ERR_ARG, "null handle"); }

int mimrl_set_bank_rows(mimrl_handle* h, int rows) {
  if (!h) return set_error(MIMRL_ERR_ARG, "null handle");
  if (rows < 0 || rows > h->cfg.bank_capacity) return set_error(MIMRL_ERR_ARG, "bank rows %d outside [0,%d]", rows, h->cfg.bank_capacity);
  if (rows > 0) {
    if (!h->bufs.bank_c || !h->bufs.bank_f || !h->bufs.bank_t || !h->bufs.bank_a || !h->bufs.bank_v || !h->bufs.anchors)
      return set_error(MIMRL_ERR_STATE, "banks/anchors must be bound before enabling them");
    if (rows - h->m_anchor() < h->cfg.k_neighbor)
      return set_error(MIMRL_ERR_ARG, "bank of %d rows is too small for %d anchors and k=%d", rows, h->m_anchor(), h->cfg.k_neighbor);
  }
  h->bank_rows = rows;
  return MIMRL_OK;
}

int mimrl_stage1_step(mimrl_handle* h) { return h ? h->run(1, 0) : set_error(MIMRL_ERR_ARG, "null handle"); }
int mimrl_stage2_step(mimrl_handle* h) { return h ? h->run(2, 0) : set_error(MIMRL_ERR_ARG, "null handle"); }
int mimrl_two_stage_step(mimrl_handle* h) { return h ? h->run_step() : set_error(MIMRL_ERR_ARG, "null handle"); }
int mimrl_stage_grads(mimrl_handle* h, int stage) { return h ? h->run(stage, 1) : set_error(MIMRL_ERR_ARG, "null handle"); }
int mimrl_stage_apply(mimrl_handle* h, int stage) { return h ? h->run(stage, 2) : set_error(MIMRL_ERR_ARG, "null handle"); }
int mimrl_stage_grads_part(mimrl_handle* h, int stage, int part) {
  if (!h) return set_error(MIMRL_ERR_ARG, "null handle");
  if (stage != 2 || (part != 0 && part != 1)) return set_error(MIMRL_ERR_ARG, "mimrl_stage_grads_part: stage 2, part 0 or 1");
  if (h->cfg.encoder != MIMRL_ENCODER_GRU) return set_error(MIMRL_ERR_ARG, "mimrl_stage_grads_part: GRU encoders only");
  return h->run(2, part == 0 ? 3 : 4);
}

int mimrl_forward(mimrl_handle* h, int train_mode, int with_losses) {
  if (!h) return set_error(MIMRL_ERR_ARG, "null handle");
  if (!h->bound) return set_error(MIMRL_ERR_STATE, "mimrl_bind must be called first");
  MX(h->ensure_images());
  h->pipe_primed = false;
  launch_begin_stage(h->stream, h->d_ints, (int*)nullptr, h->bufs.scalars, 32, 32);
  LAUNCH_CHECK();
  h->ev_next = 0;
  MX(h->model_forward(train_mode != 0, false));
  if (!with_losses) return MIMRL_OK;
  launch_task_loss(h->stream, h->task_loss, h->bufs.pred, h->bufs.labels, (float*)nullptr,
                     h->bufs.scalars + MIMRL_S2_TASK, h->cfg.batch);
  LAUNCH_CHECK();
  h->ev_next = 0;
  if (h->bank_rows > 0) { MX(h->fork(4, 4)); MX(h->knn_launch(2, h->S(4))); MX(h->estimators_all(2, false, false)); }
  launch_finalize_stage2(h->stream, h->bufs.scalars, h->mi_raw, h->cmi_raw,
                     h->coef2(), h->bank_rows > 0 ? 1 : 0);
  LAUNCH_CHECK();
  return MIMRL_OK;
}

int mimrl_estimate(mimrl_handle* h, int stage) {
  if (!h) return set_error(MIMRL_ERR_ARG, "null handle");
  if (!h->bound) return set_error(MIMRL_ERR_STATE, "mimrl_bind must be called first");
  if (stage != 1 && stage != 2) return set_error(MIMRL_ERR_ARG, "stage must be 1 or 2");
  if (h->bank_rows <= 0) return set_error(MIMRL_ERR_STATE, "mimrl_estimate needs non-empty banks");
  MX(h->ensure_images());
  h->ev_next = 0;
  MX(h->fork(4, 4));
  MX(h->knn_launch(stage, h->S(4)));
  MX(h->estimators_all(stage, false, false));
  if (stage == 1) {
    launch_finalize_stage1(h->stream, h->bufs.scalars, h->mi_raw, h->cmi_raw,
                       h->bce_raw, h->coef1());
  } else {
    launch_task_loss(h->stream, h->task_loss, h->bufs.pred, h->bufs.labels, (float*)nullptr,
                       h->bufs.scalars + MIMRL_S2_TASK, h->cfg.batch);
    launch_finalize_stage2(h->stream, h->bufs.scalars, h->mi_raw, h->cmi_raw,
                       h->coef2(), 1);
  }
  LAUNCH_CHECK();
  return MIMRL_OK;
}

int mimrl_probe_cube(mimrl_handle* h, const float* x, float* out, const float* dout, float* dx) {
  if (!h || !x || !out) return set_error(MIMRL_ERR_ARG, "null argument");
  if (!h->bound) return set_error(MIMRL_ERR_STATE, "mimrl_bind must be called first");
  if (dout && !dx) return set_error(MIMRL_ERR_ARG, "dout without dx");
  const mimrl_cfg& c = h->cfg;
  const int nb = c.n_blocks;
  const size_t nin = (size_t)c.batch * c.time_len * 3 * c.d_common;
// ... 272 lines not shown
    if (h->side[i]) (void)hipStreamDestroy(h->side[i]);
  for (auto e : h->ev_pool) (void)hipEventDestroy(e);
  if (h->cap_stream) (void)hipStreamDestroy(h->cap_stream);
  if (h->pre_stream) (void)hipStreamDestroy(h->pre_stream);
  if (h->comm) (void)mimrl::comm_destroy(h->comm);
  if (h->comm_s) (void)hipStreamDestroy(h->comm_s);
  if (h->comm_crit16) (void)hipFree(h->comm_crit16);
  if (h->ws) (void)hipFree(h->ws);
  delete h;
}

int mimrl_op_gemm(void* stream, const float* A, const float* B, float* C, int M, int N, int K, int batch,
                  const int64_t st[9], const float* bias_n, const float* bias_m, float alpha, float beta, int act,
                  int precision) {
  if (!st) return set_error(MIMRL_ERR_ARG, "null strides");
  GemmDesc d;
  d.A = A; d.B = B; d.C = C; d.M = M; d.N = N; d.K = K; d.batch = batch;
  d.sa_m = st[0]; d.sa_k = st[1]; d.sa_b = st[2]; d.sb_k = st[3]; d.sb_n = st[4]; d.sb_b = st[5];
  d.sc_m = st[6]; d.sc_n = st[7]; d.sc_b = st[8];
  d.bias_n = bias_n; d.bias_m = bias_m; d.alpha = alpha; d.beta = beta; d.act = act & 0xff;
  d.atomic = (act >> 8) & 1;
  return gemm(reinterpret_cast<hipStream_t>(stream), d, (precision & 1) != 0);
}

int mimrl_op_gemm_ex(void* stream, const float* A, const float* B, float* C, int M, int N, int K, int batch, const int64_t st[9],
                     const float* A2, const float* B2, int K2, const int64_t st2[6], int a_gap_at, int a_gap_rows, const float* bias_n,
                     const float* gradact_u, float* colsum, int act, int precision) {
  if (!st || (A2 && !st2)) return set_error(MIMRL_ERR_ARG, "null strides");
  GemmDesc d;
  d.A = A; d.B = B; d.C = C; d.M = M; d.N = N; d.K = K; d.batch = batch;
  d.sa_m = st[0]; d.sa_k = st[1]; d.sa_b = st[2]; d.sb_k = st[3]; d.sb_n = st[4]; d.sb_b = st[5];
  d.sc_m = st[6]; d.sc_n = st[7]; d.sc_b = st[8];
  if (A2) {
    d.A2 = A2; d.B2 = B2; d.K2 = K2;
    d.sa2_m = st2[0]; d.sa2_k = st2[1]; d.sa2_b = st2[2]; d.sb2_k = st2[3]; d.sb2_n = st2[4]; d.sb2_b = st2[5];
  }
  d.a_gap_at = a_gap_at; d.a_gap_rows = a_gap_rows;
  d.bias_n = bias_n; d.gradact_u = gradact_u; d.colsum = colsum; d.act = act & 0xff; d.atomic = (act >> 8) & 1;
  return gemm(reinterpret_cast<hipStream_t>(stream), d, (precision & 1) != 0);
}

int mimrl_op_gemm16(void* stream, const void* A, const void* B, void* C, int M, int N, int K, int batch, const int64_t st[9],
                    const void* A2, const void* B2, int K2, const int64_t st2[6], int batch_in, const int64_t st_bo[5],
                    const float* bias_n, int flags) {
  if (!st || (A2 && !st2) || (batch_in > 0 && !st_bo)) return set_error(MIMRL_ERR_ARG, "null strides");
  if (batch_in < 0 || (batch_in > 0 && batch % batch_in != 0)) return set_error(MIMRL_ERR_ARG, "batch_in must divide batch");
  GemmDesc d;
  d.A = static_cast<const float*>(A); d.B = static_cast<const float*>(B); d.C = static_cast<float*>(C);
  d.M = M; d.N = N; d.K = K; d.batch = batch;
  d.sa_m = st[0]; d.sa_k = st[1]; d.sa_b = st[2]; d.sb_k = st[3]; d.sb_n = st[4]; d.sb_b = st[5];
  d.sc_m = st[6]; d.sc_n = st[7]; d.sc_b = st[8];
  if (A2) {
    d.A2 = static_cast<const float*>(A2); d.B2 = static_cast<const float*>(B2); d.K2 = K2;
    d.sa2_m = st2[0]; d.sa2_k = st2[1]; d.sa2_b = st2[2]; d.sb2_k = st2[3]; d.sb2_n = st2[4]; d.sb2_b = st2[5];
  }
  if (batch_in > 0) { d.batch_in = batch_in; d.sa_bo = st_bo[0]; d.sb_bo = st_bo[1]; d.sc_bo = st_bo[2]; d.bias_n_bo = st_bo[3]; }
  if (st_bo) d.bias_n_b = st_bo[4];
  d.bias_n = bias_n;
  d.a_bf16 = flags & 1; d.b_bf16 = (flags >> 1) & 1; d.f16 = (flags >> 2) & 1; d.c_f16 = (flags >> 3) & 1; d.atomic = (flags >> 4) & 1;
  if (flags >> 8) { d.a_gap_at = (flags >> 8) & 0xfff; d.a_gap_rows = (flags >> 20) & 0xfff; }
  return gemm(reinterpret_cast<hipStream_t>(stream), d, true);
}

int mimrl_op_gemm_wgrad_group(void* stream, int n, const float* const* A, const float* const* B, float* const* C, const int32_t* dims,
                              const int64_t* st, int precision) {
  if (n <= 0 || n > 12 || !A || !B || !C || !dims || !st) return set_error(MIMRL_ERR_ARG, "gemm_wgrad_group: 1..12 problems");
  GemmDesc d[12];
  for (int i = 0; i < n; ++i) {
    d[i].A = A[i]; d[i].B = B[i]; d[i].C = C[i];
    d[i].M = dims[4 * i]; d[i].N = dims[4 * i + 1]; d[i].K = dims[4 * i + 2]; d[i].batch = dims[4 * i + 3];
    const int64_t* q = st + 9 * i;
    d[i].sa_m = q[0]; d[i].sa_k = q[1]; d[i].sa_b = q[2]; d[i].sb_k = q[3]; d[i].sb_n = q[4]; d[i].sb_b = q[5];
    d[i].sc_m = q[6]; d[i].sc_n = q[7]; d[i].sc_b = q[8];
    d[i].atomic = 1;
  }
  return gemm_group_splitk(reinterpret_cast<hipStream_t>(stream), d, n, (precision & 1) != 0);
}

int64_t mimrl_op_gru_saved_floats(int B, int T) { return gru_saved_floats(B, T); }

int mimrl_op_gru_forward(void* stream, const float* gx_f, const float* gx_r, const float* whh_f, const float* whh_r,
                         const float* bhh_f, const float* bhh_r, const int32_t* lens, float* out, float* saved_f,
                         float* saved_r, int B, int T, int precision) {
  GruFwdArgs a;
  std::memset(&a, 0, sizeof a);
  a.B = B; a.T = T; a.out_ld = 2 * H; a.nmod = 1; a.btv = gru_pick_btv(B, 1);
  a.lens[0] = lens; a.lens[1] = lens;
  a.seq[0][0] = GruSeq{gx_f, whh_f, bhh_f, out, saved_f};
  a.seq[0][1] = GruSeq{gx_r, whh_r, bhh_r, out, saved_r};
  return gru_forward(reinterpret_cast<hipStream_t>(stream), a, (precision & 1) != 0);
}

int mimrl_op_gru_backward(void* stream, const float* whh_f, const float* whh_r, const float* saved_f,
                          const float* saved_r, const int32_t* lens, const float* out, const float* dout, float* dg_f,
                          float* dg_r, float* hprev_f, float* hprev_r, int B, int T, int precision) {
  GruBwdArgs a;
  std::memset(&a, 0, sizeof a);
  a.B = B; a.T = T; a.out_ld = 2 * H; a.dout_ld = 2 * H; a.dout_off = H; a.nmod = 1; a.btv = gru_pick_btv(B, 1);
  a.lens[0] = lens; a.lens[1] = lens;
  a.seq[0][0] = GruSeqBwd{whh_f, saved_f, out, dout, dg_f, hprev_f, nullptr, nullptr};
  a.seq[0][1] = GruSeqBwd{whh_r, saved_r, out, dout, dg_r, hprev_r, nullptr, nullptr};
  return gru_backward(reinterpret_cast<hipStream_t>(stream), a, (precision & 1) != 0);
}

int mimrl_op_recur_btv(int B, int nmod) {
  if (B < 1 || nmod < 1 || nmod > 2) return set_error(MIMRL_ERR_ARG, "mimrl_op_recur_btv: B >= 1, nmod 1 or 2");
  const int g = gru_pick_btv(B, nmod), l = lstm_btv(B, nmod);
  if (g != l) return set_error(MIMRL_ERR_STATE, "mimrl_op_recur_btv: the GRU (%d) and LSTM (%d) picks differ: give this entry point an encoder argument", g, l);
  return g;
}

int mimrl_op_lstm_forward(void* stream, const float* gx_f, const float* gx_r, const float* whh_f, const float* whh_r,
                          const float* bhh_f, const float* bhh_r, const int32_t* lens, float* out, float* saved_f,
                          float* saved_r, int B, int T, int kernel) {
  if (!gx_f || !gx_r || !whh_f || !whh_r || !bhh_f || !bhh_r || !lens || !out) return set_error(MIMRL_ERR_ARG, "mimrl_op_lstm_forward: null argument");
  if ((saved_f != nullptr) != (saved_r != nullptr)) return set_error(MIMRL_ERR_ARG, "mimrl_op_lstm_forward: both saved records or neither");
  LstmFwdArgs a;
  std::memset(&a, 0, sizeof a);
  a.B = B; a.T = T; a.out_ld = 2 * H; a.nmod = 1;
  a.lens[0] = lens; a.lens[1] = lens;
  a.seq[0][0] = LstmSeq{gx_f, whh_f, bhh_f, out, saved_f};
  a.seq[0][1] = LstmSeq{gx_r, whh_r, bhh_r, out, saved_r};
  return lstm_forward_kernels(reinterpret_cast<hipStream_t>(stream), a, kernel);
}

int mimrl_op_lstm_backward(void* stream, const float* whh_f, const float* whh_r, const float* saved_f,
                           const float* saved_r, const int32_t* lens, const float* out, const float* dout, float* dg_f,
                           float* dg_r, float* hprev_f, float* hprev_r, int B, int T, int kernel) {
  if (!whh_f || !whh_r || !saved_f || !saved_r || !lens || !out || !dout || !dg_f || !dg_r || !hprev_f || !hprev_r)
    return set_error(MIMRL_ERR_ARG, "mimrl_op_lstm_backward: null argument");
  LstmBwdArgs a;
  std::memset(&a, 0, sizeof a);
  a.B = B; a.T = T; a.out_ld = 2 * H; a.dout_ld = 2 * H; a.nmod = 1;
  a.lens[0] = lens; a.lens[1] = lens;
  a.seq[0][0] = LstmSeqBwd{whh_f, saved_f, out, dout, dg_f, hprev_f};
  a.seq[0][1] = LstmSeqBwd{whh_r, saved_r, out, dout + H, dg_r, hprev_r};
  return lstm_backward_kernels(reinterpret_cast<hipStream_t>(stream), a, kernel);
}

int mimrl_op_concat_dw(void* stream, const void* dz2, const void* a1, float* dw2, const void* dz1, const void* a0, float* dw1, int E, int64_t rows,
                       int64_t dw_stride, const float* ds, const void* a2h, float* dw3, const uint32_t* m2, const float* w3, const float* P,
                       const float* Q, int B) {
  if ((!dz2 && !m2) || !a1 || !dw2) return set_error(MIMRL_ERR_ARG, "mimrl_op_concat_dw: null argument");
  if ((dz1 != nullptr) != (a0 != nullptr || P != nullptr) || (dz1 != nullptr) != (dw1 != nullptr)) return set_error(MIMRL_ERR_ARG, "mimrl_op_concat_dw: the second layer comes as a set");
  if (!concat_dw_ok(E, rows, 256)) return set_error(MIMRL_ERR_ARG, "mimrl_op_concat_dw: E >= 1, rows >= 1");
  ConcatDwArgs a;
  a.dz[0] = static_cast<const __bf16*>(dz2); a.act[0] = static_cast<const __bf16*>(a1); a.dw[0] = dw2;
  a.dz[1] = static_cast<const __bf16*>(dz1); a.act[1] = static_cast<const __bf16*>(a0); a.dw[1] = dw1;
  a.nlayer = dz1 ? 2 : 1; a.E = E; a.rows = rows; a.dw_stride = dw_stride;
  a.ds = ds; a.a2 = static_cast<const _Float16*>(a2h); a.dw3 = dw3; a.m2 = m2; a.w3 = w3; a.P = P; a.Q = Q; a.B = B;
  return concat_dw(reinterpret_cast<hipStream_t>(stream), a);
}

int mimrl_op_gru_wgrad(void* stream, const void* const* dg, const void* const* x, const void* const* hp, float* const* dw_ih,
                       float* const* dw_hh, int64_t rows, int kp) {
  if (!dg || !x || !hp || !dw_ih || !dw_hh) return set_error(MIMRL_ERR_ARG, "mimrl_op_gru_wgrad: null argument");
  GruWgradArgs a;
  for (int s = 0; s < 4; ++s) {
    if (!dg[s] || !x[s] || !hp[s] || !dw_ih[s] || !dw_hh[s]) return set_error(MIMRL_ERR_ARG, "mimrl_op_gru_wgrad: null array for sequence %d", s);
    a.seq[s] = GruWgradSeq{static_cast<const __bf16*>(dg[s]), static_cast<const __bf16*>(x[s]), static_cast<const __bf16*>(hp[s]), dw_ih[s], dw_hh[s]};
  }
  a.rows = rows; a.kp = kp;
  return gru_wgrad(reinterpret_cast<hipStream_t>(stream), a);
}

int mimrl_op_mi_bound(void* stream, const float* scores, float* dscores, float* mi, const float* gscale, int E, int B,
                      int bound) {
  return mi_bound_fwd_bwd(reinterpret_cast<hipStream_t>(stream), scores, dscores, mi, nullptr, gscale, E, B, bound, 0u);
}
int mimrl_op_mi_bound_baseline(void* stream, float* scores, float* dscores, float* mi, const float* gscale, const float* lb,
                               float* dlb, int E, int B, int bound) {
  return mi_bound_fwd_bwd(reinterpret_cast<hipStream_t>(stream), scores, dscores, mi, nullptr, gscale, E, B, bound, 0u, lb, dlb, B);
}
int mimrl_op_mi_bound_ex(void* stream, const float* scores, float* dscores, float* mi, float* mi_loss, const float* gscale,
                         int E, int B, int bound, uint32_t lossform) {
  return mi_bound_fwd_bwd(reinterpret_cast<hipStream_t>(stream), scores, dscores, mi, mi_loss, gscale, E, B, bound, lossform);
}

int mimrl_op_mi_infonce_rows(void* stream, const float* scores, float* dscores, float* mi, float* mi_loss, const float* gscale,
                             int E, int B, float* ws) {
  static_assert(MIMRL_NCE_WS_FLOATS >= NCE_WS_WIDE_FLOATS && NCE_WS_WIDE_FLOATS >= NCE_WS_FLOATS, "MIMRL_NCE_WS_FLOATS too small");
  if (!scores || !mi || !ws || E < 1 || E > 16) return set_error(MIMRL_ERR_ARG, "mi_infonce_rows: null array or E = %d outside [1, 16]", E);
  return mi_bound_fwd_bwd(reinterpret_cast<hipStream_t>(stream), scores, dscores, mi, mi_loss, gscale, E, B, BOUND_INFONCE, 0u, nullptr,
                          nullptr, 0, ws);
}
int mimrl_op_mi_sep_infonce(void* stream, const float* tout, float* dtout, float* mi, float* mi_loss, const float* gscale, int E,
                            int B, int tiled) {
  hipStream_t st = reinterpret_cast<hipStream_t>(stream);
  if (!tiled) return mi_sep_fused(st, tout, dtout, mi, mi_loss, gscale, E, B, BOUND_INFONCE, 0x1fu, dtout ? 1 : 0);
  return mi_sep_nce_tiled(st, tout, dtout, mi, mi_loss, gscale, E, B, dtout ? 1 : 0);
}

int mimrl_op_knn(void* stream, const float* Z, int dz, int N, const int32_t* anchors, int m, int k, int32_t* idx_out) {
  KnnArgs a;
  std::memset(&a, 0, sizeof a);
  a.call[0] = KnnCall{Z, dz, anchors, idx_out};
  a.N = N; a.m = m; a.k = k; a.ncall = 1;
  return knn_sample(reinterpret_cast<hipStream_t>(stream), a);
}

int mimrl_probe_knn(mimrl_handle* h, int stage, int32_t* idx_out) {
  if (!h || !idx_out) return set_error(MIMRL_ERR_ARG, "mimrl_probe_knn: null argument");
  if (stage != 1 && stage != 2) return set_error(MIMRL_ERR_ARG, "stage must be 1 or 2");
  HIPX(hipMemcpyAsync(idx_out, stage == 2 ? h->knn_idx2 : h->knn_idx, sizeof(int32_t) * NE_CMI * h->nprod(), hipMemcpyDeviceToDevice, h->user_stream));
  return MIMRL_OK;
}

int mimrl_op_sample_anchors(void* stream, int32_t* anchors_out, int ncall, int m, int N, uint64_t seed, const int32_t* step,
                            uint32_t stream_id, int step_add) {
  if (!anchors_out || !step || ncall < 1 || ncall > KNN_MAX_CALLS) return set_error(MIMRL_ERR_ARG, "mimrl_op_sample_anchors: bad argument");
  AnchorDraws d;
  d.n = ncall;
  for (int c = 0; c < ncall; ++c) { d.out[c] = anchors_out + (size_t)c * m; d.call[c] = c; d.stream_id[c] = stream_id; d.step_add[c] = step_add; }
  return sample_anchors(reinterpret_cast<hipStream_t>(stream), d, m, N, (uint32_t)seed, (uint32_t)(seed >> 32), step);
}

int mimrl_op_cmi_loss(void* stream, const float* logits, float* dlogits, float* bce, float* cmi, const float* g_bce,
                      const float* g_cmi, int E, int n, int hardtanh) {
  return cmi_loss_fwd_bwd(reinterpret_cast<hipStream_t>(stream), logits, dlogits, bce, cmi, g_bce, g_cmi, E, n, hardtanh);
}

int mimrl_op_task_loss(void* stream, int kind, const float* pred, const float* y, float* dpred, float* loss, int B) {
  if (!pred || !y || !loss) return set_error(MIMRL_ERR_ARG, "task_loss: null argument");
  if (kind < MIMRL_TASK_LOSS_MAE || kind > MIMRL_TASK_LOSS_CCC) return set_error(MIMRL_ERR_ARG, "task loss kind %d unknown", kind);
  if (B < 1 || B > 1024) return set_error(MIMRL_ERR_ARG, "task_loss: batch %d outside [1, 1024]", B);
  launch_task_loss(reinterpret_cast<hipStream_t>(stream), kind, pred, y, dpred, loss, B);
  LAUNCH_CHECK();
  return MIMRL_OK;
}

static int fill_mlp_args(MlpFusedArgs* fa, int nb, int rows, int brows, int nl, const int32_t* dims, const float* const* W,
                         int64_t pstride) {
  if (!dims || !W || nl < 1 || nl > MLPF_MAX_LAYERS) return set_error(MIMRL_ERR_ARG, "mlp_stack: bad arguments");
  std::memset(fa, 0, sizeof *fa);
  fa->nb = nb; fa->rows = rows; fa->brows = brows; fa->nl = nl; fa->pstride = pstride;
  for (int l = 0; l <= nl; ++l) fa->dims[l] = dims[l];
  for (int l = 0; l < nl; ++l) fa->W[l] = W[l];
  return MIMRL_OK;
}

int mimrl_op_mlp_stack_forward(void* stream, int nb, int rows, int brows, int nl, const int32_t* dims, const float* const* W,
                               const float* const* b, int64_t pstride, const float* in, float* const* act, float* out) {
  MlpFusedArgs fa;
  MX(fill_mlp_args(&fa, nb, rows, brows, nl, dims, W, pstride));
  if (!b || !in || !out || (nl > 1 && !act)) return set_error(MIMRL_ERR_ARG, "mlp_stack_forward: null argument");
  for (int l = 0; l < nl; ++l) { fa.b[l] = b[l]; if (l < nl - 1) fa.act[l] = act[l]; }
  fa.in = in; fa.out = out;
  return mlp_stack_fwd_fused(reinterpret_cast<hipStream_t>(stream), fa);
}

int mimrl_op_mlp_stack_backward(void* stream, int nb, int rows, int brows, int nl, const int32_t* dims, const float* const* W,
                                int64_t pstride, const float* const* act, const float* dout, float* const* dz, float* din,
                                float* const* db) {
  MlpFusedArgs fa;
  MX(fill_mlp_args(&fa, nb, rows, brows, nl, dims, W, pstride));
  if (!dout || (nl > 1 && (!act || !dz))) return set_error(MIMRL_ERR_ARG, "mlp_stack_backward: null argument");
  for (int l = 0; l < nl - 1; ++l) { fa.act[l] = const_cast<float*>(act[l]); fa.dz[l + 1] = dz[l + 1]; fa.db[l] = db ? db[l] : nullptr; }
  fa.dout = dout; fa.din = din;
  return mlp_stack_bwd_fused(reinterpret_cast<hipStream_t>(stream), fa);
}

int mimrl_op_adam(void* stream, float* p, float* g, float* m, float* v, int64_t n, const float* lr, const int32_t* step,
                  float beta1, float beta2, float eps, float weight_decay, float clip) {
  AdamArgs a;
  a.p = p; a.g = g; a.m = m; a.v = v; a.n = n; a.lr = lr; a.step = step;
  a.beta1 = beta1; a.beta2 = beta2; a.eps = eps; a.weight_decay = weight_decay; a.clip = clip;
  return adam_step(reinterpret_cast<hipStream_t>(stream), a);
}

}
```

mimrl_amd/csrc/engine_backward.hip:

```cpp
#include "engine.h"

int mimrl_handle::cube_backward(int cur_in, int* cur_out) {
  const int B = cfg.batch;
  int dims[MIMRL_MAX_BLOCKS + 1][3];
  dims[0][0] = cfg.time_len; dims[0][1] = 3; dims[0][2] = cfg.d_common;
  for (int i = 0; i < cfg.n_blocks; ++i)
    for (int ax = 0; ax < 3; ++ax) dims[i + 1][ax] = cfg.d_outs[i][ax];
  const int per_block = 7 + (cfg.dropout_mlp[0] > 0.f) + (cfg.dropout_mlp[2] > 0.f);
  const bool defer = multi_stream && !cfg.ln_first && per_block * cfg.n_blocks + 1 <= NGBUF;
  const int npool = defer ? NGBUF : 4;
  int used[NGBUF] = {0};
  used[cur_in] = 1;
  int cur = cur_in;
  auto grab = [&]() { for (int q = 0; q < npool; ++q) if (!used[q]) { used[q] = 1; return q; } return -1; };
  auto release = [&](int q) { if (!defer) used[q] = 0; };
  auto W_gemm = [&](int sd, const GemmDesc& g) -> int {
    if (defer) { deferred.push_back(Deferred{0, sd, g, nullptr, 0, 0, 0, 0, nullptr}); return MIMRL_OK; }
    return G_on(S(sd), g);
  };
  auto W_colsum = [&](int sd, const float* src, long rows, int cols, int ld, float* dst) -> int {
    if (defer) { deferred.push_back(Deferred{1, sd, GemmDesc(), src, rows, cols, ld, 0, dst}); return MIMRL_OK; }
    return colsum(S(sd), src, rows, cols, ld, dst);
  };
  auto W_rowsum = [&](int sd, const float* src, int nb, int rows, int cols, float* dst) -> int {
    if (defer) { deferred.push_back(Deferred{2, sd, GemmDesc(), src, nb, rows, cols, 0, dst}); return MIMRL_OK; }
    return rowsum_batched(S(sd), src, nb, rows, cols, dst);
  };
  auto W_lnpar = [&](int sd, const float* y, const float* mean, const float* rstd, const float* dz, float* dgam, float* dbet,
                     int nb, int n, int cols) -> int {
    if (defer) {
      Deferred d{3, sd, GemmDesc(), y, nb, n, cols, 0, dgam};
      d.p1 = mean; d.p2 = rstd; d.p3 = dz; d.dst2 = dbet;
      deferred.push_back(d);
      return MIMRL_OK;
    }
    return colln_param_grads(S(sd), y, mean, rstd, dz, dgam, dbet, nb, n, cols);
  };
  auto W_dpg = [&](int sd, const float* y, const float* mean, const float* rstd, const float* dz, const float* dy, const float* du,
                   float* dgam, float* dbet, float* db2, float* db1, long rows) -> int {
    if (defer) {
      Deferred d{6, sd, GemmDesc(), y, rows, 0, 0, 0, dgam};
      d.p1 = mean; d.p2 = rstd; d.p3 = dz; d.p4 = dy; d.p5 = du; d.dst2 = dbet; d.dst3 = db2; d.dst4 = db1;
      deferred.push_back(d);
      return MIMRL_OK;
    }
    return daxis_param_grads(S(sd), y, mean, rstd, dz, dy, du, dgam, dbet, db2, db1, rows);
  };
  auto W_fork = [&](int lo, int hi) -> int { return defer ? MIMRL_OK : fork(lo, hi); };
  bool d_fused[MIMRL_MAX_BLOCKS] = {};
  MX(wt_images(stream, bf16, !(wtT_prebuilt && wtT_built), d_fused));
  auto W_join = [&](int lo, int hi) -> int { return defer ? MIMRL_OK : join(lo, hi); };
#define GRAB(var)                                                                                   \
  const int var = grab();                                                                           \
  if (var < 0) return set_error(MIMRL_ERR_STATE, "cube_backward: out of gradient buffers (line %d)", __LINE__)

  for (int i = cfg.n_blocks - 1; i >= 0; --i) {
    const BlockW& w = blk[i];
    BlockBuf& b = bb[i];
    const int il = dims[i][0], ik = dims[i][1], id = dims[i][2];
    const int hl = w.ax[0].hid, ol = w.ax[0].out, hk = w.ax[1].hid, ok = w.ax[1].out, hd = w.ax[2].hid, od = w.ax[2].out;
    const float* xblk = i == 0 ? cube0 : bb[i - 1].d.z;
    const float pl = cfg.dropout_mlp[0], pk = cfg.dropout_mlp[1], pd = cfg.dropout_mlp[2];
    if (d_fused[i]) {
      const AxisW& a = w.ax[2];
      const long R2 = (long)B * ol * ok;
      GRAB(i_dy); GRAB(i_du); GRAB(i_dx);
      DAxisBwdArgs fa;
      fa.dz = gbuf[cur]; fa.y = b.d.y; fa.mean = b.d.mean; fa.rstd = b.d.rstd; fa.gamma = P(a.ln_g); fa.u = b.d.u;
      fa.w2t = wtT[i][0]; fa.w1t = wtT[i][1]; fa.wrt = wtT[i][2];
      fa.dy = gbuf[i_dy]; fa.du = gbuf[i_du]; fa.dx = gbuf[i_dx];
      fa.R = R2; fa.act = cfg.activation;
      fa.dgamma = fa.dbeta = fa.db2 = fa.db1 = nullptr;
      MX(daxis_bwd_fused(stream, fa));
      MX(W_fork(1, 3));
      MX(W_dpg(2, b.d.y, b.d.mean, b.d.rstd, gbuf[cur], gbuf[i_dy], gbuf[i_du], Gm(a.ln_g), Gm(a.ln_b),
               a.fc2.b >= 0 ? Gm(a.fc2.b) : nullptr, a.fc1.b >= 0 ? Gm(a.fc1.b) : nullptr, R2));
      { GemmDesc g = gemm_tn(gbuf[i_dy], od, b.d.h, hd, Gm(a.fc2.w), hd, od, hd, (int)R2); g.atomic = 1; MX(W_gemm(1, g)); }
      { GemmDesc g = gemm_tn(gbuf[i_dy], od, b.k.z, id, Gm(a.res), id, od, id, (int)R2); g.atomic = 1; MX(W_gemm(2, g)); }
      { GemmDesc g = gemm_tn(gbuf[i_du], hd, b.k.z, id, Gm(a.fc1.w), id, hd, id, (int)R2); g.atomic = 1; MX(W_gemm(3, g)); }
      MX(W_join(1, 3));
      release(cur); release(i_dy); release(i_du);
      cur = i_dx;
    } else {
      const AxisW& a = w.ax[2];
      const long R2 = (long)B * ol * ok;
      const float* xin = b.k.z;
      const float* xmlp = cfg.ln_first ? b.d.xn : b.k.z;
      int i_dy = cur;
      if (!cfg.ln_first) {
        GRAB(q);
        MX(rowln_bwd(stream, b.d.y, P(a.ln_g), b.d.mean, b.d.rstd, gbuf[cur], gbuf[q], Gm(a.ln_g), Gm(a.ln_b), R2, od));
        release(cur);
        i_dy = q;
      }
      const float* dy = gbuf[i_dy];
      int i_dym = i_dy;
      if (pd > 0.f) {
        GRAB(q);
        HIPX(hipMemcpyAsync(gbuf[q], dy, sizeof(float) * R2 * od, hipMemcpyDeviceToDevice, stream));
        MX(dropout_inplace(stream, gbuf[q], R2 * od, pd, key(), 12 + 3 * i));
        i_dym = q;
      }
      const float* dym = gbuf[i_dym];
      MX(W_fork(1, 2));
      { GemmDesc g = gemm_tn(dym, od, b.d.h, hd, Gm(a.fc2.w), hd, od, hd, (int)R2); g.atomic = 1; MX(W_gemm(1, g)); }
      if (a.fc2.b >= 0) MX(W_colsum(1, dym, R2, od, od, Gm(a.fc2.b)));
      if (a.res >= 0) { GemmDesc g = gemm_tn(dy, od, xin, id, Gm(a.res), id, od, id, (int)R2); g.atomic = 1; MX(W_gemm(2, g)); }
      GRAB(i_du);
      { GemmDesc g = gemm_nn(dym, od, P(a.fc2.w), hd, gbuf[i_du], hd, (int)R2, hd, od); g.act = cfg.activation; g.gradact_u = b.d.u;
        if (a.fc1.b >= 0) g.colsum = Gm(a.fc1.b);
        MX(G_(g)); }
      MX(W_fork(3, 3));
      { GemmDesc g = gemm_tn(gbuf[i_du], hd, xmlp, id, Gm(a.fc1.w), id, hd, id, (int)R2); g.atomic = 1; MX(W_gemm(3, g)); }
      GRAB(i_dx0);
      int i_dx = i_dx0;
      const bool fuse_dx = a.res >= 0 && !cfg.ln_first;
      { GemmDesc g = gemm_nn(gbuf[i_du], hd, P(a.fc1.w), id, gbuf[i_dx], id, (int)R2, id, hd);
        if (fuse_dx) { g.A2 = dy; g.sa2_m = od; g.sa2_k = 1; g.B2 = P(a.res); g.sb2_k = id; g.sb2_n = 1; g.K2 = od; }
        MX(G_(g)); }
      if (cfg.ln_first) {
        MX(join(3, 3));
        MX(rowln_bwd(stream, b.k.z, P(a.ln_g), b.d.xn_mean, b.d.xn_rstd, gbuf[i_dx], gbuf[i_du], Gm(a.ln_g), Gm(a.ln_b), R2, id));
        release(i_dx);
        i_dx = i_du;
      } else {
        release(i_du);
      }
      if (!fuse_dx) {
        if (a.res >= 0) { GemmDesc g = gemm_nn(dy, od, P(a.res), id, gbuf[i_dx], id, (int)R2, id, od); g.beta = 1.f; MX(G_(g)); }
        else MX(add_inplace(stream, gbuf[i_dx], dy, R2 * id));
      }
      MX(W_join(1, 3));
      if (i_dym != i_dy) release(i_dym);
      release(i_dy);
      cur = i_dx;
    }
    {
      const AxisW& a = w.ax[1];
      KMixW kw;
      std::memset(&kw, 0, sizeof kw);
      kw.w1 = P(a.fc1.w); kw.b1 = a.fc1.b >= 0 ? P(a.fc1.b) : nullptr;
      kw.w2 = P(a.fc2.w); kw.b2 = a.fc2.b >= 0 ? P(a.fc2.b) : nullptr;
      kw.wr = a.res >= 0 ? P(a.res) : nullptr; kw.g = P(a.ln_g); kw.be = P(a.ln_b);
      kw.dw1 = Gm(a.fc1.w); kw.db1 = a.fc1.b >= 0 ? Gm(a.fc1.b) : nullptr;
      kw.dw2 = Gm(a.fc2.w); kw.db2 = a.fc2.b >= 0 ? Gm(a.fc2.b) : nullptr;
      kw.dwr = a.res >= 0 ? Gm(a.res) : nullptr; kw.dg = Gm(a.ln_g); kw.dbe = Gm(a.ln_b);
      kw.ik = ik; kw.hk = hk; kw.ok = ok; kw.act = cfg.activation; kw.ln_first = cfg.ln_first;
      kw.drop_p = pk; kw.key = key(); kw.stream_id = 11 + 3 * i;
      GRAB(q);
      static const int kmix_inchain = dbg_env("MIMRL_KMIX_PG_INCHAIN") ? atoi(dbg_env("MIMRL_KMIX_PG_INCHAIN")) : 1;
      if (defer && kmix_inchain) {
        MX(kmix_bwd(stream, b.l.z, gbuf[cur], gbuf[q], kw, (long)B * ol, id));
      } else if (defer) {
        MX(kmix_bwd_part(stream, b.l.z, gbuf[cur], gbuf[q], kw, (long)B * ol, id, 1));
        static const int kdbg = dbg_env("MIMRL_DBG_KMIX") ? atoi(dbg_env("MIMRL_DBG_KMIX")) : 0;
        static const bool kmix_park = dbg_env("MIMRL_KMIX_PG_PARKED") != nullptr;
        if (kmix_park) {
          Deferred d{5, 2, GemmDesc(), b.l.z, (long)B * ol, id, 0, 0, nullptr};
          d.p3 = gbuf[cur]; d.kw = kw; d.kw.dbg = kdbg;
          deferred.push_back(d);
        } else {
          KMixW kp = kw; kp.dbg = kdbg;
          MX(fork(3, 3));
          MX(kmix_bwd_part(S(3), b.l.z, gbuf[cur], nullptr, kp, (long)B * ol, id, 2));
          kmix_pg_on_side3 = true;
        }
      } else {
        MX(kmix_bwd(stream, b.l.z, gbuf[cur], gbuf[q], kw, (long)B * ol, id));
      }
      release(cur);
      cur = q;
    }
    if (bf16 && fused_cube_bwd && !cfg.ln_first && pl <= 0.f && w.ax[0].res >= 0 && laxis_bwd_supported(il, hl, ol, ik * id) &&
        (il <= 64 || laxis_bwd_long_on)) {
      const AxisW& a = w.ax[0];
      const long C = (long)ik * id;
      GRAB(i_dy); GRAB(i_du); GRAB(i_dx);
      LAxisBwdArgs fa;
      fa.dz = gbuf[cur]; fa.y = b.l.y; fa.mean = b.l.mean; fa.rstd = b.l.rstd; fa.gamma = P(a.ln_g); fa.u = b.l.u;
      fa.w2 = P(a.fc2.w); fa.w1 = P(a.fc1.w); fa.wr = P(a.res);
      fa.dy = gbuf[i_dy]; fa.du = gbuf[i_du]; fa.dx = gbuf[i_dx];
      fa.db2 = a.fc2.b >= 0 ? Gm(a.fc2.b) : nullptr; fa.db1 = a.fc1.b >= 0 ? Gm(a.fc1.b) : nullptr;
      fa.B = B; fa.il = il; fa.hl = hl; fa.ol = ol; fa.C = (int)C; fa.act = cfg.activation;
      MX(laxis_bwd_fused(stream, fa));
      MX(W_fork(1, 3));
      MX(W_lnpar(1, b.l.y, b.l.mean, b.l.rstd, gbuf[cur], Gm(a.ln_g), Gm(a.ln_b), B, ol, (int)C));
      release(cur);
      { GemmDesc g; g.A = gbuf[i_dy]; g.sa_m = C; g.sa_k = 1; g.sa_b = (long)ol * C;
        g.B = b.l.h; g.sb_k = 1; g.sb_n = C; g.sb_b = (long)hl * C;
        g.C = Gm(a.fc2.w); g.sc_m = hl; g.sc_n = 1; g.sc_b = 0; g.M = ol; g.N = hl; g.K = (int)C; g.batch = B; g.atomic = 1;
        MX(W_gemm(1, g)); }
      { GemmDesc g; g.A = gbuf[i_dy]; g.sa_m = C; g.sa_k = 1; g.sa_b = (long)ol * C;
        g.B = xblk; g.sb_k = 1; g.sb_n = C; g.sb_b = (long)il * C;
        g.C = Gm(a.res); g.sc_m = il; g.sc_n = 1; g.sc_b = 0; g.M = ol; g.N = il; g.K = (int)C; g.batch = B; g.atomic = 1;
        MX(W_gemm(2, g)); }
      { GemmDesc g; g.A = gbuf[i_du]; g.sa_m = C; g.sa_k = 1; g.sa_b = (long)hl * C;
        g.B = xblk; g.sb_k = 1; g.sb_n = C; g.sb_b = (long)il * C;
        g.C = Gm(a.fc1.w); g.sc_m = il; g.sc_n = 1; g.sc_b = 0; g.M = hl; g.N = il; g.K = (int)C; g.batch = B; g.atomic = 1;
        MX(W_gemm(3, g)); }
      MX(W_join(1, 3));
      release(i_dy); release(i_du);
      cur = i_dx;
    } else {
      const AxisW& a = w.ax[0];
      const long C = (long)ik * id;
      const float* xmlp = cfg.ln_first ? b.l.xn : xblk;
      int i_dy = cur;
      if (!cfg.ln_first) {
        GRAB(q);
        MX(colln_bwd(stream, b.l.y, P(a.ln_g), b.l.mean, b.l.rstd, gbuf[cur], gbuf[q], Gm(a.ln_g), Gm(a.ln_b), B, ol, (int)C));
        release(cur);
        i_dy = q;
      }
      const float* dy = gbuf[i_dy];
      int i_dym = i_dy;
      if (pl > 0.f) {
        GRAB(q);
        HIPX(hipMemcpyAsync(gbuf[q], dy, sizeof(float) * B * ol * C, hipMemcpyDeviceToDevice, stream));
        MX(dropout_inplace(stream, gbuf[q], (long)B * ol * C, pl, key(), 10 + 3 * i));
        i_dym = q;
      }
      const float* dym = gbuf[i_dym];
      MX(W_fork(1, 2));
      { GemmDesc g; g.A = dym; g.sa_m = C; g.sa_k = 1; g.sa_b = (long)ol * C;
        g.B = b.l.h; g.sb_k = 1; g.sb_n = C; g.sb_b = (long)hl * C;
        g.C = Gm(a.fc2.w); g.sc_m = hl; g.sc_n = 1; g.sc_b = 0; g.M = ol; g.N = hl; g.K = (int)C; g.batch = B; g.atomic = 1;
        MX(W_gemm(1, g)); }
      if (a.fc2.b >= 0) MX(W_rowsum(1, dym, B, ol, (int)C, Gm(a.fc2.b)));
      if (a.res >= 0) {
        GemmDesc g; g.A = dy; g.sa_m = C; g.sa_k = 1; g.sa_b = (long)ol * C;
        g.B = xblk; g.sb_k = 1; g.sb_n = C; g.sb_b = (long)il * C;
        g.C = Gm(a.res); g.sc_m = il; g.sc_n = 1; g.sc_b = 0; g.M = ol; g.N = il; g.K = (int)C; g.batch = B; g.atomic = 1;
        MX(W_gemm(2, g));
      }
      GRAB(i_du);
      { GemmDesc g; g.A = P(a.fc2.w); g.sa_m = 1; g.sa_k = hl; g.sa_b = 0;
        if (bf16 && w2p[i] && w2p_valid[i] && hl % 4 != 0) { g.A = w2p[i]; g.sa_k = (hl + 3) & ~3; g.a_pad4 = 1; }
        g.B = dym; g.sb_k = C; g.sb_n = 1; g.sb_b = (long)ol * C;
        g.C = gbuf[i_du]; g.sc_m = C; g.sc_n = 1; g.sc_b = (long)hl * C; g.M = hl; g.N = (int)C; g.K = ol; g.batch = B;
        g.act = cfg.activation; g.gradact_u = b.l.u;
        MX(G_(g)); }
      MX(W_fork(3, 3));
      { GemmDesc g; g.A = gbuf[i_du]; g.sa_m = C; g.sa_k = 1; g.sa_b = (long)hl * C;
        g.B = xmlp; g.sb_k = 1; g.sb_n = C; g.sb_b = (long)il * C;
        g.C = Gm(a.fc1.w); g.sc_m = il; g.sc_n = 1; g.sc_b = 0; g.M = hl; g.N = il; g.K = (int)C; g.batch = B; g.atomic = 1;
        MX(W_gemm(3, g)); }
      if (a.fc1.b >= 0) MX(W_rowsum(3, gbuf[i_du], B, hl, (int)C, Gm(a.fc1.b)));
      GRAB(i_dx0);
      int i_dx = i_dx0;
      { GemmDesc g; g.A = P(a.fc1.w); g.sa_m = 1; g.sa_k = il; g.sa_b = 0;
        g.B = gbuf[i_du]; g.sb_k = C; g.sb_n = 1; g.sb_b = (long)hl * C;
        g.C = gbuf[i_dx]; g.sc_m = C; g.sc_n = 1; g.sc_b = (long)il * C; g.M = il; g.N = (int)C; g.K = hl; g.batch = B;
        if (a.res >= 0 && !cfg.ln_first) {
          g.A2 = P(a.res); g.sa2_m = 1; g.sa2_k = il; g.sa2_b = 0;
          g.B2 = dy; g.sb2_k = C; g.sb2_n = 1; g.sb2_b = (long)ol * C; g.K2 = ol;
        }
        MX(G_(g)); }
      if (cfg.ln_first) {
        MX(join(3, 3));
        MX(colln_bwd(stream, xblk, P(a.ln_g), b.l.xn_mean, b.l.xn_rstd, gbuf[i_dx], gbuf[i_du], Gm(a.ln_g), Gm(a.ln_b), B, il, (int)C));
        release(i_dx);
        i_dx = i_du;
      } else {
        release(i_du);
      }
      if (a.res >= 0 && !cfg.ln_first) {
      } else if (a.res >= 0) {
        GemmDesc g; g.A = P(a.res); g.sa_m = 1; g.sa_k = il; g.sa_b = 0;
        g.B = dy; g.sb_k = C; g.sb_n = 1; g.sb_b = (long)ol * C;
        g.C = gbuf[i_dx]; g.sc_m = C; g.sc_n = 1; g.sc_b = (long)il * C; g.M = il; g.N = (int)C; g.K = ol; g.batch = B; g.beta = 1.f;
        MX(G_(g));
      } else {
        MX(add_inplace(stream, gbuf[i_dx], dy, (long)B * il * C));
      }
      MX(W_join(1, 3));
      if (i_dym != i_dy) release(i_dym);
      release(i_dy);
      cur = i_dx;
    }
    static const int early = dbg_env("MIMRL_EARLY_FLUSH") ? atoi(dbg_env("MIMRL_EARLY_FLUSH")) : 2;
    if (defer && (early == 2 || (early == 1 && i == cfg.n_blocks - 1))) MX(flush_deferred(1));
  }
#undef GRAB
  *cur_out = cur;
  return MIMRL_OK;
}

__global__ void dbg_spin_kernel(long ticks) {
  const long t0 = wall_clock64();
  while (wall_clock64() - t0 < ticks) __builtin_amdgcn_s_sleep(16);
}
int mimrl_handle::dbg_delay(hipStream_t st, int tag) {
  static const char* spec = knob("MIMRL_DBG_DELAY_TAG");
  static const int want = spec ? atoi(spec) : -1;
  static const int us = spec && strchr(spec, ':') ? atoi(strchr(spec, ':') + 1) : 50;
  if (tag != want) return MIMRL_OK;
  hipLaunchKernelGGL(dbg_spin_kernel, dim3(1), dim3(64), 0, st, (long)us * 100);
  LAUNCH_CHECK();
  return MIMRL_OK;
}

int mimrl_handle::flush_deferred(int only_side) {
  if (deferred.empty()) return MIMRL_OK;
  if (only_side > 0) MX(fork(only_side, only_side)); else MX(fork(1, 3));
  for (int q = 1; q <= 3; ++q) MX(dbg_delay(S(q), 9));
  constexpr int wg_sides = 3;
  static const int dbg_skip_kinds = dbg_env("MIMRL_DBG_SKIP_DEFERRED") ? atoi(dbg_env("MIMRL_DBG_SKIP_DEFERRED")) : 0;
  const bool groupk = !prof_on && bf16 && !((dbg_skip_kinds >> 0) & 1) && cfg.seq_len <= 128;
  if (groupk) {
    std::vector<GemmDesc> cls[2];
    for (const Deferred& d : deferred) if (d.kind == 0) cls[d.g.sa_k == 1 ? 0 : 1].push_back(d.g);
    for (int c = 0; c < 2; ++c) {
      hipStream_t st = only_side > 0 ? S(only_side) : S(1 + c % wg_sides);
      for (size_t i = 0; i < cls[c].size(); i += 12) MX(gemm_group_splitk(st, cls[c].data() + i, (int)std::min<size_t>(12, cls[c].size() - i), bf16));
    }
  }
  int rr = 2;
  for (const Deferred& d : deferred) {
    if ((dbg_skip_kinds >> d.kind) & 1) continue;
    if (groupk && d.kind == 0) continue;
    static const bool dbg_defer_main = dbg_env("MIMRL_DBG_DEFER_MAIN") != nullptr;
    hipStream_t st = dbg_defer_main ? stream : only_side > 0 ? S(only_side) : S(1 + (groupk ? rr++ : d.side - 1) % wg_sides);
    if (d.kind == 0) MX(G_on(st, d.g));
    else if (d.kind == 1) MX(colsum(st, d.src, d.n0, (int)d.n1, (int)d.n2, d.dst));
    else if (d.kind == 2) MX(rowsum_batched(st, d.src, (int)d.n0, (int)d.n1, (int)d.n2, d.dst));
    else if (d.kind == 3) MX(colln_param_grads(st, d.src, d.p1, d.p2, d.p3, d.dst, d.dst2, (int)d.n0, (int)d.n1, (int)d.n2));
    else if (d.kind == 6) MX(daxis_param_grads(st, d.src, d.p1, d.p2, d.p3, d.p4, d.p5, d.dst, d.dst2, d.dst3, d.dst4, d.n0));
    else MX(kmix_bwd_part(st, d.src, d.p3, nullptr, d.kw, d.n0, (int)d.n1, 2));
  }
  deferred.clear();
  return MIMRL_OK;
}

int mimrl_handle::model_backward() {
  Range rg("mimrl.model_backward");
  DetDefer det_defer(stream, &det_ranges);
  const int B = cfg.batch, T = cfg.seq_len, L = cfg.time_len, D = cfg.d_common;
  const long BT_ = (long)B * T;
  const int nb = cfg.n_blocks;
  const int ol = cfg.d_outs[nb - 1][0], ok = cfg.d_outs[nb - 1][1], od = cfg.d_outs[nb - 1][2];
  MX(head_bwd(stream, dfeat, dpred, P(cls_w), bufs.feats, gbuf[0], Gm(cls_w), Gm(cls_b), B, ol, ok, od,
              cfg.compose_t_sum, cfg.compose_k_sum, head_gather_on ? &head_gather : nullptr));
  int ci = 0;
  deferred.clear();
  { Scope sc(this, MIMRL_PH_CUBE_BWD); MX(cube_backward(0, &ci)); }
  MX(dbg_delay(stream, 7));
  return encoders_backward(gbuf[ci]);
}

int mimrl_handle::encoders_backward(float* dcube) {
  const int B = cfg.batch, T = cfg.seq_len, L = cfg.time_len, D = cfg.d_common;
  const long BT_ = (long)B * T;
  const float* dmean = dfeat + (size_t)B * D;
  if (head_gather_on && ev_dmean) { HIPX(hipStreamWaitEvent(stream, ev_dmean, 0)); ev_dmean = nullptr; }
  {
    LnSide2 sd[2];
    for (int m = 0; m < 2; ++m)
      sd[m] = LnSide2{h1[m], P(ln_g[m]), P(ln_b[m]), ln_mean[m], ln_rstd[m], ds[m], Gm(ln_g[m]), Gm(ln_b[m]), 1 + m,
                      cfg.dropout[1 + m], (uint32_t)(1 + m)};
    ds_bf16_live = rec16_on && cfg.encoder == MIMRL_ENCODER_GRU && dg_bf16 && (prec & MIMRL_PREC_BF16_GRU_BWD) != 0 && gru_bwd_io16_ok(0);
    MX(ln_relu_drop_bwd2(stream, sd[0], sd[1], dcube, B, T, L, 3, D, key(), dmean + (size_t)B * D, dmean + 2 * (size_t)B * D, ds_bf16_live ? 1 : 0));
  }
  MX(fork(0, 0));
  MX(text_post_bwd(S(0), dcube, dtx, B, T, L, 3, D, 0, cfg.dropout[0], key(), 0, dmean));
  { GemmDesc g = gemm_tn(dtx, D, bufs.text, cfg.d_t, Gm(w_t), cfg.d_t, D, cfg.d_t, (int)BT_); g.atomic = 1; MX(G_on(S(0), g)); }
  static const int dbg_join_at = dbg_env("MIMRL_DBG_JOIN_AT") ? atoi(dbg_env("MIMRL_DBG_JOIN_AT")) : 0;
  MX(flush_deferred());
  if (dbg_join_at == 1) MX(join(1, 3));
  if (cfg.encoder != MIMRL_ENCODER_GRU) kmix_pg_on_side3 = false;
  if (cfg.encoder == MIMRL_ENCODER_CONV) {
    MX(conv_backward());
    MX(join(0, 5));
    return MIMRL_OK;
  }
  if (cfg.encoder == MIMRL_ENCODER_LSTM) {
    MX(lstm_encoders_backward());
    MX(join(0, 5));
    return MIMRL_OK;
  }
  if (kmix_pg_on_side3) { MX(join(3, 3)); kmix_pg_on_side3 = false; }
  MX(gru_layer_backward(1));
  if (split_part == 1) return join(0, 5);
  MX(gru_layer_backward(0));
  return join(0, 5);
}

int mimrl_handle::gru_layer_backward(int l) {
  const int B = cfg.batch, T = cfg.seq_len;
  const long BT_ = (long)B * T;
  static const int dbg_join_at = dbg_env("MIMRL_DBG_JOIN_AT") ? atoi(dbg_env("MIMRL_DBG_JOIN_AT")) : 0;
  const float* xin[2] = {bufs.audio, bufs.video};
  {
    GruBwdArgs a;
    a.B = B; a.T = T; a.out_ld = 2 * H; a.nmod = 2;
    a.dout_ld = l == 1 ? H : 2 * H; a.dout_off = l == 1 ? 0 : H;
    a.btv = gru_pick_btv(B, 2);
    a.stamp = kstamp; a.stamp.id = l == 1 ? 2 : 3;
    const bool lbf = dg_bf16 && (l == 1 || l0_packed || l0_bwd_pack);
    a.dg_bf16 = lbf ? 1 : 0;
    a.slab_upl = l == 0 && l0_xin ? 2 : 0;
    const bool io16 = lbf && (prec & MIMRL_PREC_BF16_GRU_BWD) != 0 && gru_bwd_io16_ok(a.slab_upl);
    a.dout_bf16 = io16 && (l == 1 ? ds_bf16_live : dh0_bf16_live) ? 1 : 0;
    if ((l == 1 ? ds_bf16_live : dh0_bf16_live) && !a.dout_bf16) return set_error(MIMRL_ERR_STATE, "gru_layer_backward: dout was stored as bf16 but this BPTT launch cannot read it");
    const bool hp16 = l == 0 && io16 && hp16_live && h0h[0] && h0h[1];
    if (l == 0 && hp16_live && !hp16) return set_error(MIMRL_ERR_STATE, "gru_layer_backward: the forward pass counted on the fp16 h_prev path");
    for (int m = 0; m < 2; ++m) {
      a.lens[m] = lens[m];
      for (int d = 0; d < 2; ++d) {
        const GruDirW& g = gru[m][l][d];
        a.seq[m][d] = GruSeqBwd{P(g.w_hh), sv[l][m][d], l == 1 ? h1[m] : h0[m], l == 1 ? ds[m] : dh0[m], dg[l][m][d],
                                hprev[l][m][d], Gm(g.b_ih), Gm(g.b_hh)};
        if (hp16) a.seq[m][d].out16 = h0h[m];
      }
    }
    { Scope sc(this, MIMRL_PH_GRU_BWD); MX(gru_backward(stream, a, (prec & MIMRL_PREC_BF16_GRU_BWD) != 0)); }
    if ((l == 1 && dbg_join_at == 2) || (l == 0 && dbg_join_at == 4)) MX(join(1, 3));
    MX(dbg_delay(stream, 8));
    constexpr int l0_side = 1;
    MX(fork(1, l == 0 ? 5 : 3));
    if (l == 1) {
      dh0_bf16_live = false;
      {
        GemmDesc q = gemm_nn(dg[l][0][0], 4 * H, P(gru[0][l][0].w_ih), 2 * H, dh0[0], 2 * H, (int)BT_, 2 * H, G);
        q.A2 = dg[l][0][1]; q.sa2_m = 4 * H; q.sa2_k = 1;
        q.B2 = P(gru[0][l][1].w_ih); q.sb2_k = 2 * H; q.sb2_n = 1; q.K2 = G;
        q.batch = 2;
        q.sa_b = dg[l][1][0] - dg[l][0][0]; q.sa2_b = dg[l][1][1] - dg[l][0][1];
        q.sb_b = gru[1][l][0].w_ih - gru[0][l][0].w_ih; q.sb2_b = gru[1][l][1].w_ih - gru[0][l][1].w_ih;
        q.sc_b = dh0[1] - dh0[0];
        if (lbf) { q.a_bf16 = 1; q.sa_b *= 2; q.sa2_b *= 2; }
        if (lbf && w1_img_valid && h16_on && w1b) {
          q.B = reinterpret_cast<const float*>(w1b); q.B2 = reinterpret_cast<const float*>(w1b + (long)G * 2 * H);
          q.b_bf16 = 1; q.sb_b = 2L * G * 2 * H; q.sb2_b = 2L * G * 2 * H;
          if (w1bt) {
            GemmDesc t = q;
            t.B = reinterpret_cast<const float*>(w1bt); t.B2 = reinterpret_cast<const float*>(w1bt + G);
            t.sb_k = 1; t.sb_n = 2 * G; t.sb2_k = 1; t.sb2_n = 2 * G; t.sb_b = 2L * H * 2 * G; t.sb2_b = 2L * H * 2 * G;
            if (gemm_tall_ok(t)) {
              q = t;
              if (rec16_on && (prec & MIMRL_PREC_BF16_GRU_BWD) != 0 && (l0_packed || l0_bwd_pack) && gru_bwd_io16_ok(l0_xin ? 2 : 0)) { q.c_bf16 = 1; q.sc_b *= 2; dh0_bf16_live = true; }
            }
          }
        }
        MX(G_(q));
      }
    }
    if (l == 1 && dbg_join_at == 3) MX(join(1, 3));
    if (l == 0 && (l0_packed || l0_bwd_pack)) {
      const long s_dg = dg[0][0][1] - dg[0][0][0], o_dg = dg[0][1][0] - dg[0][0][0];
      const long s_hp = hprev[0][0][1] - hprev[0][0][0], o_hp = hprev[0][1][0] - hprev[0][0][0];
      static const bool wgrad_on = knob("MIMRL_NO_GRU_WGRAD") == nullptr;
      const bool one_pass = wgrad_on && lbf && xpack16 && BT_ >= 32768 && gru_wgrad_ok(BT_, KP());
      if (one_pass) {
        GruWgradArgs w;
        const __bf16* xb = reinterpret_cast<const __bf16*>(xpack + BT_ * KP());
        for (int m = 0; m < 2; ++m)
          for (int d = 0; d < 2; ++d)
            w.seq[m * 2 + d] = GruWgradSeq{reinterpret_cast<const __bf16*>(dg[0][m][d]), xb + (long)m * BT_ * KP(),
                                           reinterpret_cast<const __bf16*>(hprev[0][m][d]), dwih_pack + (long)(m * 2 + d) * G * KP(),
                                           dwhh_pack + (long)(m * 2 + d) * G * H};
        w.rows = BT_; w.kp = KP();
        MX(gru_wgrad(stream, w));
      } else {
      { GemmDesc q = gemm_tn(dg[0][0][0], 4 * H, xpack, KP(), dwih_pack, KP(), G, KP(), (int)BT_);
        q.batch = 4; q.batch_in = 2; q.sa_b = s_dg; q.sa_bo = o_dg; q.sb_b = 0; q.sb_bo = BT_ * KP(); q.sc_b = (long)G * KP(); q.sc_bo = 2L * G * KP();
        if (lbf) { q.a_bf16 = 1; q.sa_b *= 2; q.sa_bo *= 2; }
        if (lbf && xpack16) { q.B = reinterpret_cast<const float*>(reinterpret_cast<const __bf16*>(xpack + BT_ * KP())); q.b_bf16 = 1; }
        q.atomic = 1; MX(G_on(stream, q)); }
      { GemmDesc q = gemm_tn(dg[0][0][0], 4 * H, hprev[0][0][0], H, dwhh_pack, H, G, H, (int)BT_);
        q.a_gap_at = 2 * H; q.a_gap_rows = H;
        q.batch = 4; q.batch_in = 2; q.sa_b = s_dg; q.sa_bo = o_dg; q.sb_b = s_hp; q.sb_bo = o_hp; q.sc_b = (long)G * H; q.sc_bo = 2L * G * H;
        if (lbf) { q.a_bf16 = q.b_bf16 = 1; q.sa_b *= 2; q.sa_bo *= 2; q.sb_b *= 2; q.sb_bo *= 2; }
        q.atomic = 1; MX(G_on(S(l0_side), q)); }
      MX(join(l0_side, l0_side));
      }
      L0Unpack up;
      for (int m = 0; m < 2; ++m) {
        up.d[m] = gru[m][0][0].din;
        for (int d = 0; d < 2; ++d) { up.g_ih[m][d] = Gm(gru[m][0][d].w_ih); up.g_hh[m][d] = Gm(gru[m][0][d].w_hh); }
      }
      up.dwih_pack = dwih_pack; up.dwhh_pack = dwhh_pack; up.KP = KP();
      if (fold_unpack) unpack_pending = true;
      else MX(l0_unpack_grads(stream, up));
      return MIMRL_OK;
    }
    int rr = 0;
    for (int m = 0; m < 2; ++m) {
      const float* in = l == 0 ? xin[m] : h0[m];
      const GruDirW &gf = gru[m][l][0], &gr = gru[m][l][1];
      const long s_dg = dg[l][m][1] - dg[l][m][0], s_hp = hprev[l][m][1] - hprev[l][m][0];
      const bool both = l == 1;
      if (both && m == 1) break;
      auto two = [&](GemmDesc& q, long a_o, long b_o, long c_o) { if (both) { q.batch = 4; q.batch_in = 2; q.sa_bo = a_o; q.sb_bo = b_o; q.sc_bo = c_o; } };
      const long o_dg = dg[l][1][0] - dg[l][0][0], o_hp = hprev[l][1][0] - hprev[l][0][0], o_in = both ? h0[1] - h0[0] : 0;
      const long o_wih = gru[1][l][0].w_ih - gru[0][l][0].w_ih, o_whh = gru[1][l][0].w_hh - gru[0][l][0].w_hh;
      constexpr int wg_sides = 3;
      auto pick = [&]() { return l == 0 ? stream : S(1 + rr++ % wg_sides); };
      { GemmDesc q = gemm_tn(dg[l][m][0], 4 * H, in, gf.din, Gm(gf.w_ih), gf.din, G, gf.din, (int)BT_);
// ... 40 lines not shown
```

mimrl_amd/csrc/knobs.cpp:

```cpp
#include "knobs.h"

#include <cstdlib>
#include <cstring>
#include <mutex>
#include <set>
#include <string>

namespace mimrl {

namespace {
struct KnobDef { const char* name; const char* where; const char* dflt; const char* help; };
const KnobDef kKnobs[] = {
  {"MIMRL_KNOBS", "engine_abi.hip", "", "1: print this table (values in effect) to stderr when a handle is created"},
  {"MIMRL_ADAM_FRAG", "engine_abi.hip", "", "0: combined step with frag_images + stage_boundary as launches behind the critic Adam (round 5a) instead of inside it"},
  {"MIMRL_CONCAT_STREAMED", "concat_fused.hip", "", "1: the concat critic on the weight-streaming kernels of rounds 2-5 (concat_fused.hip) instead of the weights-stationary ones (concat_ws.hip)"},
  {"MIMRL_DBG_DELAY_TAG", "engine_backward.hip", "-1", "critical-path probe: <tag>[:<us>] -- the phase tag behind which a spin kernel of <us> (default 50) microseconds is injected (tools/critical_path.sh)"},
  {"MIMRL_DDP_SPLIT", "engine_abi.hip", "", "0: the main gradient bucket all-reduced in one piece (in-library RCCL and dist.py)"},
  {"MIMRL_DG_FP32", "engine_abi.hip", "", "BPTT outputs dg / h_prev stored as fp32 instead of bf16"},
  {"MIMRL_DWIH_H16", "engine_abi.hip", "", "0: the layer-1 dW_ih product reads the fp32 layer-0 outputs instead of the recurrence's fp16 copy"},
  {"MIMRL_FWD_BF16", "engine_abi.hip", "", "forward products round to bf16 instead of fp16"},
  {"MIMRL_GEMM_TALL_MIN_M", "gemm_tall.hip", "", "row threshold of the tall LDS-DMA GEMM (default 4096)"},
  {"MIMRL_GRAPH_DOT", "engine_step.hip", "", "dump the captured two-stage graph to this file (hipGraphDebugDotPrint)"},
  {"MIMRL_GRU_LDS_PAD", "gru.hip", "-1", "KiB of dynamic LDS a small BPTT launch reserves to keep parked kernels off its CUs (default 144 below 129 workgroups)"},
  {"MIMRL_GRU_SKIP", "gru.hip", "0", "probe build only (make probe): phase-elimination mask of the recurrence kernels; ignored by the default build"},
  {"MIMRL_GRU_WAVES", "gru.hip", "4", "8: one hidden unit per lane, two waves per SIMD, in the bf16 recurrence kernels (default 4)"},
  {"MIMRL_GX_F16", "engine_abi.hip", "", "1: hoisted GRU input projections stored as fp16 (measured slower at cfg3)"},
  {"MIMRL_L0_PACK", "engine_abi.hip", "", "0: no packed layer-0 operands (2 + 4 launches instead of 1 + 2)"},
  {"MIMRL_NO_CONCAT_DW", "engine_estimators.hip", "", "1: the concat critic's hidden-layer weight gradients as two split-K GEMMs instead of the one-launch kernel (concat_dw.hip, round 6)"},
  {"MIMRL_NO_GRU_WGRAD", "engine_backward.hip", "", "1: the layer-0 GRU weight gradients as two batched split-K GEMMs instead of the one-pass kernel (gru_wgrad.hip, round 6)"},
  {"MIMRL_LAXIS_BWD_LONG", "engine_abi.hip", "", "0: the L-axis backward of a long-sequence CubeMLP block (L > 64) as colln_bwd + GEMM chain instead of the LONG instantiation of laxis_bwd_kernel"},
  {"MIMRL_LAXIS_LONG", "engine_abi.hip", "", "0: the L-axis MLP of a long-sequence CubeMLP block (L > 64) as the GEMM chain instead of the one-pass kernel of cube_long.hip"},
  {"MIMRL_LSTM_MFMA_FP32", "lstm.hip", "", "1: fp32 precision mode runs the fp32-MFMA LSTM kernels instead of the scalar ones (measured slower)"},
  {"MIMRL_LSTM_SCALAR", "lstm.hip", "", "1: the scalar fp32 LSTM kernels of round 1 instead of the MFMA ones"},
  {"MIMRL_MLP_NO_FRAG", "mlp_fused.hip", "", "the round-2 kernels (read per call: tests/test_gpu_fused_oracle.py toggles it)"},
  {"MIMRL_NO_FOLD_UNPACK", "engine_abi.hip", "", "packed layer-0 weight gradients through l0_unpack instead of the Adam fold"},
  {"MIMRL_NO_FUSED_CONCAT", "engine_abi.hip", "", "concat critic tail as a GEMM chain instead of concat_fwd / concat_bwd"},
  {"MIMRL_NO_FUSED_CUBE", "engine_abi.hip", "", "bf16 mode: CubeMLP forward as the unfused GEMM / LayerNorm chain"},
  {"MIMRL_NO_FUSED_CUBE_BWD", "engine_abi.hip", "", "bf16 mode: CubeMLP backward as the unfused chain"},
  {"MIMRL_NO_FUSED_MI", "engine_estimators.hip", "", "separable critic: scores / bound / gradients as separate kernels instead of mi_sep_fused / mi_sep_nce"},
  {"MIMRL_NO_FUSED_MLP", "engine_abi.hip", "", "bf16 mode: estimator MLP stacks as grouped GEMMs"},
  {"MIMRL_NO_FUSED_MLP_BWD", "engine_estimators.hip", "", "estimator MLP stacks: data-gradient chain as GEMMs instead of the fused kernel"},
  {"MIMRL_NO_CONCAT_DQ", "engine_estimators.hip", "", "concat critic backward: dZ0 goes out in fp32 and pair_reduce_q sums it over the x rows (rounds 2-4) instead of the in-kernel dQ partial sums"},
  {"MIMRL_NO_DUAL_TAIL_PRE", "engine_step.hip", "", "long sequences (T > 128): each forward tail runs its own text dropout / LN + ReLU + dropout / temporal-mean launches instead of one launch for both"},
  {"MIMRL_NO_FUSED_TAIL_PRE", "engine_forward.hip", "", "forward tail: text dropout, LN + ReLU + dropout and the temporal means as separate launches"},
  {"MIMRL_NO_GEMM_TALL", "gemm_tall.hip", "", "tall LDS-DMA GEMM (gemm_tall.hip) off: the 128x128 register-staged kernels"},
  {"MIMRL_NO_H16", "engine_abi.hip", "", "fp32-stored operands for the layer-1 projection / dh0 (bit-identical results)"},
  {"MIMRL_NO_MI_NCE_TILED", "engine_estimators.hip", "", "separable InfoNCE: the one-workgroup-per-estimator kernel instead of the row-tiled one"},
  {"MIMRL_NO_SHARED_PREFIX", "engine_step.hip", "", "evaluate the prefix twice"},
  {"MIMRL_NO_STEP_GRAPH", "engine_step.hip", "", "Solver.step as two per-stage graphs instead of one combined graph"},
  {"MIMRL_NO_XIN", "engine_abi.hip", "", "layer-0 input projection as its own GEMM instead of fused into the recurrence kernel"},
  {"MIMRL_REC16", "engine_abi.hip", "", "0: the BPTT launches read fp32 dout / h_prev (round 5a): dh0 and ds stored fp32, the fused-projection forward writes its fp32 outputs"},
  {"MIMRL_SINGLE_STREAM", "engine_abi.hip", "", "enqueue everything on one stream (no side streams)"},
};
constexpr int kN = sizeof(kKnobs) / sizeof(kKnobs[0]);
}

const char* knob(const char* name) {
  bool known = false;
  for (int i = 0; i < kN && !known; ++i) known = std::strcmp(kKnobs[i].name, name) == 0;
  if (!known) {
    static std::mutex mu;
    static std::set<std::string> told;
    std::lock_guard<std::mutex> g(mu);
    if (told.insert(name).second) std::fprintf(stderr, "[mimrl] knob %s is read but not registered in csrc/knobs.cpp\n", name);
  }
  return std::getenv(name);
}

int knob_int(const char* name, int dflt) {
  const char* v = knob(name);
  return v ? std::atoi(v) : dflt;
}

void knobs_print(FILE* f) {
  std::fprintf(f, "[mimrl] environment knobs (tuning / debugging only; '-' = not set, the default applies)\n");
  for (int i = 0; i < kN; ++i) {
    const char* v = std::getenv(kKnobs[i].name);
    std::fprintf(f, "  %-28s %-10s %-16s %s%s%s\n", kKnobs[i].name, v ? v : "-", kKnobs[i].where, kKnobs[i].help,
                 kKnobs[i].dflt[0] ? " [default " : "", kKnobs[i].dflt[0] ? (std::string(kKnobs[i].dflt) + "]").c_str() : "");
  }
}

}
```

Baseline: 1228.

## Fuse head and last CubeMLP block backward into one tail kernel

Adds a single kernel that runs the classifier head backward plus the D-, K- and L-axis backward of the last CubeMLP block per batch item, with MFMA for the D-axis GEMMs and LDS staging. It replaces several per-axis launches and the separate head_bwd launch, and lets daxis_param_grads broadcast the head gradient through a row divisor. The aim is to cut launch count and the global-memory round trips between stages. In exchange it uses one workgroup per batch item with heavy LDS use and one wave per SIMD (launch_bounds 256,1), so occupancy may be low. Weight gradients stay as atomic GEMMs on side streams.

Result: slower. 1127 (-8.3%).

```diff
diff --git a/include/mimrl.h b/include/mimrl.h
--- a/include/mimrl.h
+++ b/include/mimrl.h
@@ -153,6 +153,7 @@
 int mimrl_op_concat_dw(void* stream, const void* dz2, const void* a1, float* dw2, const void* dz1, const void* a0, float* dw1, int E, int64_t rows,
                        int64_t dw_stride, const float* ds, const void* a2h, float* dw3, const uint32_t* m2, const float* w3, const float* P,
                        const float* Q, int B);
+int mimrl_op_cube_tail_bwd(void* stream, int chain, const int32_t* dims, const float* const* in, float* const* out, float* scratch);
 int mimrl_op_gru_wgrad(void* stream, const void* const* dg, const void* const* x, const void* const* hp, float* const* dw_ih,
                        float* const* dw_hh, int64_t rows, int kp);
 int mimrl_op_mi_bound(void* stream, const float* scores, float* dscores, float* mi, const float* gscale, int E, int B,
diff --git a/mimrl_amd/_lib.py b/mimrl_amd/_lib.py
--- a/mimrl_amd/_lib.py
+++ b/mimrl_amd/_lib.py
@@ -108,6 +108,7 @@
     lib.mimrl_op_lstm_forward.argtypes = [_FP] * 11 + [C.c_int, C.c_int, C.c_int]
     lib.mimrl_op_lstm_backward.argtypes = [_FP] * 12 + [C.c_int, C.c_int, C.c_int]
     lib.mimrl_op_recur_btv.argtypes = [C.c_int, C.c_int]
+    lib.mimrl_op_cube_tail_bwd.argtypes = [C.c_void_p, C.c_int, C.c_void_p, C.c_void_p, C.c_void_p, C.c_void_p]
     lib.mimrl_op_concat_dw.argtypes = [C.c_void_p] * 7 + [C.c_int, C.c_int64, C.c_int64] + [C.c_void_p] * 7 + [C.c_int]
     lib.mimrl_op_gru_wgrad.argtypes = [C.c_void_p] + [C.POINTER(C.c_void_p)] * 5 + [C.c_int64, C.c_int]
     lib.mimrl_op_mi_bound.argtypes = [_FP] * 5 + [C.c_int, C.c_int, C.c_int]
@@ -158,7 +159,7 @@
     "mimrl_bucket_floats", "mimrl_create", "mimrl_bind", "mimrl_set_bank_rows", "mimrl_set_inputs", "mimrl_stage1_step", "mimrl_stage2_step", "mimrl_two_stage_step",
     "mimrl_stage_grads", "mimrl_stage_grads_part", "mimrl_stage_apply", "mimrl_forward", "mimrl_estimate", "mimrl_profile_enable", "mimrl_profile_read", "mimrl_profile_read_gemm",
     "mimrl_workspace_bytes", "mimrl_params_changed", "mimrl_set_stage2_prefetch", "mimrl_stage2_forward_tail", "mimrl_set_grad_scale", "mimrl_destroy", "mimrl_op_gemm", "mimrl_op_gemm_ex", "mimrl_op_gemm16", "mimrl_op_gemm_wgrad_group",
-    "mimrl_op_gru_saved_floats", "mimrl_op_gru_forward", "mimrl_op_gru_backward", "mimrl_op_gru_wgrad", "mimrl_op_concat_dw", "mimrl_op_mi_bound", "mimrl_op_mi_bound_ex", "mimrl_op_mi_bound_baseline", "mimrl_op_mi_sep_infonce", "mimrl_op_knn",
+    "mimrl_op_gru_saved_floats", "mimrl_op_gru_forward", "mimrl_op_gru_backward", "mimrl_op_gru_wgrad", "mimrl_op_concat_dw", "mimrl_op_cube_tail_bwd", "mimrl_op_mi_bound", "mimrl_op_mi_bound_ex", "mimrl_op_mi_bound_baseline", "mimrl_op_mi_sep_infonce", "mimrl_op_knn",
     "mimrl_op_cmi_loss", "mimrl_op_sample_anchors", "mimrl_knn_r1_host", "mimrl_set_knn_override_mask", "mimrl_op_mlp_stack_forward", "mimrl_op_mlp_stack_backward", "mimrl_op_adam",
     "mimrl_probe_cube", "mimrl_probe_mi", "mimrl_probe_cmi", "mimrl_probe_knn", "mimrl_probe_encoders", "mimrl_set_kernel_stamps", "mimrl_comm_unique_id", "mimrl_set_comm", "mimrl_main_late_offset", "mimrl_set_comm_critic_bf16",
     "mimrl_stage1_pipe_prime", "mimrl_stage1_pipe", "mimrl_set_task_loss", "mimrl_op_task_loss",
diff --git a/mimrl_amd/csrc/cube_bwd_fused.h b/mimrl_amd/csrc/cube_bwd_fused.h
--- a/mimrl_amd/csrc/cube_bwd_fused.h
+++ b/mimrl_amd/csrc/cube_bwd_fused.h
@@ -31,7 +31,7 @@
 int wt_transpose_bf16(hipStream_t s, const WtTransposeArgs& a);
 
 int daxis_param_grads(hipStream_t s, const float* y, const float* mean, const float* rstd, const float* dz, const float* dy,
-                      const float* du, float* dgamma, float* dbeta, float* db2, float* db1, long R);
+                      const float* du, float* dgamma, float* dbeta, float* db2, float* db1, long R, long bc = 0);
 
 #ifdef MIMRL_PHASE_PROBE
 int cube_bwd_read_phases(long long* out);
diff --git a/mimrl_amd/csrc/cube_bwd_fused.hip b/mimrl_amd/csrc/cube_bwd_fused.hip
--- a/mimrl_amd/csrc/cube_bwd_fused.hip
+++ b/mimrl_amd/csrc/cube_bwd_fused.hip
@@ -418,7 +418,7 @@
                                                                 const float* __restrict__ rstd, const float* __restrict__ dz,
                                                                 const float* __restrict__ dy, const float* __restrict__ du,
                                                                 float* __restrict__ dgamma, float* __restrict__ dbeta,
-                                                                float* __restrict__ db2, float* __restrict__ db1, long R) {
+                                                                float* __restrict__ db2, float* __restrict__ db1, long R, long bc) {
   __shared__ float4 red[4][8][32];
   const int cq = threadIdx.x & 31, rl = threadIdx.x >> 5;
   const long r0 = (long)blockIdx.x * 64;
@@ -429,7 +429,7 @@
     const long rc = r < R ? r : R - 1;
     const float m = r < R ? 1.f : 0.f;
     const float mu = mean[rc], rs = rstd[rc] * m;
-    const float4 g = *reinterpret_cast<const float4*>(dz + rc * 128 + cq * 4);
+    const float4 g = *reinterpret_cast<const float4*>(dz + (bc > 0 ? rc / bc : rc) * 128 + cq * 4);
     const float4 yv = *reinterpret_cast<const float4*>(y + rc * 128 + cq * 4);
     const float4 v = *reinterpret_cast<const float4*>(dy + rc * 128 + cq * 4);
     const float4 u = *reinterpret_cast<const float4*>(du + rc * 128 + cq * 4);
@@ -455,10 +455,10 @@
 }
 
 int daxis_param_grads(hipStream_t s, const float* y, const float* mean, const float* rstd, const float* dz, const float* dy,
-                      const float* du, float* dgamma, float* dbeta, float* db2, float* db1, long R) {
+                      const float* du, float* dgamma, float* dbeta, float* db2, float* db1, long R, long bc) {
   if (R <= 0) return MIMRL_OK;
   hipLaunchKernelGGL(daxis_param_grads_kernel, dim3((unsigned)((R + 63) / 64)), dim3(256), 0, s, y, mean, rstd, dz, dy, du, dgamma, dbeta,
-                     db2, db1, R);
+                     db2, db1, R, bc);
   LAUNCH_CHECK();
   return MIMRL_OK;
 }
diff --git a/mimrl_amd/csrc/cube_tail_bwd.h b/mimrl_amd/csrc/cube_tail_bwd.h
--- /dev/null
+++ b/mimrl_amd/csrc/cube_tail_bwd.h
@@ -0,0 +1,29 @@
+#pragma once
+#include "common.h"
+#include "model_ops.h"
+
+namespace mimrl {
+
+struct CubeTailBwdArgs {
+  const float* dz_ext;
+  const float *dpred, *cls_w, *feats, *dff_ext;
+  GatherSum gs; int use_gs; float scale;
+  float* hv;
+  float *dcls_w, *dcls_b;
+  const float *d_y, *d_mean, *d_rstd, *d_gamma, *d_u;
+  const __bf16 *w2t, *w1t, *wrt;
+  float *d_dy, *d_du;
+  const float* kx;
+  KMixW kw;
+  float* k_dx;
+  const float *l_y, *l_mean, *l_rstd, *l_gamma, *l_u;
+  const float *l_w2, *l_w1, *l_wr;
+  float *l_dy, *l_du, *l_dx;
+  float *l_db2, *l_db1;
+  int B, il, hl, ol, K, act;
+};
+
+bool cube_tail_bwd_supported(int il, int hl, int ol, int ik, int hk, int ok, int id, int hd, int od);
+int cube_tail_bwd(hipStream_t s, const CubeTailBwdArgs& a);
+
+}
diff --git a/mimrl_amd/csrc/cube_tail_bwd.hip b/mimrl_amd/csrc/cube_tail_bwd.hip
--- /dev/null
+++ b/mimrl_amd/csrc/cube_tail_bwd.hip
@@ -0,0 +1,464 @@
+#include "cube_tail_bwd.h"
+#include "kmix_device.h"
+
+namespace mimrl {
+
+namespace {
+
+constexpr int CT = 128;
+constexpr int KP = 64 + 8;
+constexpr int DR = 32;
+constexpr int DP = 128 + 8;
+constexpr int KPF = 6;
+constexpr int NSW = 3 * KM * KM + 4 * KM;
+
+template <int NK, bool EXACT>
+__global__ __launch_bounds__(256, 1) void cube_tail_bwd_kernel(CubeTailBwdArgs a) {
+  __shared__ __attribute__((aligned(16))) __bf16 simg[2 * CT * KP];
+  __shared__ __attribute__((aligned(16))) __bf16 wts[3][64][KP];
+  __shared__ __attribute__((aligned(16))) float tile[64][128];
+  __shared__ __attribute__((aligned(16))) float sg[128];
+  __shared__ float acc_l2[64];
+  __shared__ LdsAcc acc_h[64];
+  __shared__ float sgam[64];
+  __shared__ float sw[NSW];
+  __shared__ LdsAcc sgk[NSW];
+  static_assert(2 * DR * DP <= 2 * CT * KP, "D-axis images must fit the L-axis image buffer");
+  __bf16 (*sdyD)[DP] = reinterpret_cast<__bf16 (*)[DP]>(&simg[0]);
+  __bf16 (*sduD)[DP] = reinterpret_cast<__bf16 (*)[DP]>(&simg[DR * DP]);
+  __bf16 (*sdy)[KP] = reinterpret_cast<__bf16 (*)[KP]>(&simg[0]);
+  __bf16 (*sdu)[KP] = reinterpret_cast<__bf16 (*)[KP]>(&simg[CT * KP]);
+  float (*red)[2][CT] = reinterpret_cast<float (*)[2][CT]>(&sdu[0][0]);
+
+  const int tid = threadIdx.x, lane = tid & 63, wave = tid >> 6, lr = lane & 31, lh = lane >> 5;
+  const int b = blockIdx.x;
+  const int il = a.il, hl = a.hl, ol = a.ol, K = a.K;
+  const int R = ol * K, C = K * 128;
+  const long row0 = (long)b * R;
+  const bool head = a.dz_ext == nullptr;
+  KMixW w = a.kw;
+  if constexpr (EXACT) { w.ik = NK; w.hk = NK; w.ok = NK; w.ln_first = 0; w.drop_p = 0.f; }
+
+  {
+    float wv[3][16];
+    const int n2 = ol * hl, n1 = hl * il, nr = ol * il;
+#pragma unroll
+    for (int j = 0; j < 16; ++j) {
+      const int idx = tid + 256 * j;
+      wv[0][j] = a.l_w2[idx < n2 ? idx : n2 - 1];
+      wv[1][j] = a.l_w1[idx < n1 ? idx : n1 - 1];
+      wv[2][j] = a.l_wr[idx < nr ? idx : nr - 1];
+    }
+    uint4* z = reinterpret_cast<uint4*>(&wts[0][0][0]);
+    for (int i = tid; i < 3 * 64 * KP * 2 / 16; i += 256) z[i] = make_uint4(0u, 0u, 0u, 0u);
+    if (tid < 64) { acc_l2[tid] = 0.f; acc_h[tid].zero(); sgam[tid] = a.l_gamma[tid < ol ? tid : ol - 1]; }
+    for (int i = tid; i < NSW; i += 256) sgk[i].zero();
+    kmix_stage_weights(w, sw);
+#pragma unroll
+    for (int j = 0; j < 16; ++j) {
+      const int idx = tid + 256 * j;
+      if (idx < n2) { const int o = idx / hl, h = idx - o * hl; wts[0][h][o] = to_bf16(wv[0][j]); }
+      if (idx < n1) { const int h = idx / il, i = idx - h * il; wts[1][i][h] = to_bf16(wv[1][j]); }
+      if (idx < nr) { const int o = idx / il, i = idx - o * il; wts[2][i][o] = to_bf16(wv[2][j]); }
+    }
+  }
+
+  float h_de = 0.f, h_dp = 0.f, h_w = 0.f, h_ff = 0.f;
+  if (head && tid < 128) {
+    h_dp = a.dpred[b];
+    if (a.use_gs) {
+      for (int q = 0; q < a.gs.n; ++q)
+        if (b < a.gs.rows[q]) h_de += a.gs.src[q][(long)b * a.gs.ld[q] + a.gs.off[q] + tid];
+    } else if (a.dff_ext) h_de = a.dff_ext[(long)b * 128 + tid];
+    h_w = a.cls_w[tid];
+    h_ff = a.feats[(long)b * 128 + tid];
+  }
+  const int row1 = tid >> 3, part1 = tid & 7;
+  const int n = wave * 32 + lr;
+  float mu1, rs1;
+  float4 gz4[4], yv4[4];
+  float uuD[16];
+  auto dreq = [&](int mt) __attribute__((always_inline)) {
+    const long rc1 = row0 + min(mt * DR + row1, R - 1);
+    mu1 = a.d_mean[rc1]; rs1 = a.d_rstd[rc1];
+#pragma unroll
+    for (int q = 0; q < 4; ++q) {
+      if (!head) gz4[q] = *reinterpret_cast<const float4*>(a.dz_ext + rc1 * 128 + part1 * 16 + q * 4);
+      yv4[q] = *reinterpret_cast<const float4*>(a.d_y + rc1 * 128 + part1 * 16 + q * 4);
+    }
+#pragma unroll
+    for (int r = 0; r < 16; ++r) {
+      const long row = row0 + min(mt * DR + (r & 3) + 8 * (r >> 2) + 4 * lh, R - 1);
+      uuD[r] = a.d_u[row * 128 + n];
+    }
+  };
+  dreq(0);
+  bf16x8 bw2[8], bw1[8], bwr[8];
+#pragma unroll
+  for (int ks = 0; ks < 8; ++ks) {
+    bw2[ks] = *reinterpret_cast<const bf16x8*>(a.w2t + n * 128 + ks * 16 + 8 * lh);
+    bw1[ks] = *reinterpret_cast<const bf16x8*>(a.w1t + n * 128 + ks * 16 + 8 * lh);
+    bwr[ks] = *reinterpret_cast<const bf16x8*>(a.wrt + n * 128 + ks * 16 + 8 * lh);
+  }
+  const int ktotal = ol * 128;
+  float xpre[KPF][NK];
+#pragma unroll
+  for (int j = 0; j < KPF; ++j) {
+    const int e = min(tid + 256 * j, ktotal - 1);
+    const long r = (long)b * ol + (e >> 7); const int d = e & 127;
+#pragma unroll
+    for (int k = 0; k < NK; ++k) xpre[j][k] = a.kx[(r * w.ik + (k < w.ik ? k : w.ik - 1)) * 128 + d];
+  }
+  const int col = tid & (CT - 1), half = tid >> 7;
+  auto lreq = [&](int kt, float (&uu)[2][16], float (&xq)[32], float& mu, float& rs) __attribute__((always_inline)) {
+    const int c0 = kt * CT;
+    const int ccu = c0 + wave * 32 + lr;
+#pragma unroll
+    for (int mt = 0; mt < 2; ++mt)
+#pragma unroll
+      for (int r = 0; r < 16; ++r) {
+        const int h = min(mt * 32 + (r & 3) + 8 * (r >> 2) + 4 * lh, hl - 1);
+        uu[mt][r] = a.l_u[((long)b * hl + h) * C + ccu];
+      }
+    const long cidx = (long)b * C + c0 + col;
+    mu = a.l_mean[cidx]; rs = a.l_rstd[cidx];
+    const float* __restrict__ yb = a.l_y + (long)b * ol * C + c0 + col;
+#pragma unroll
+    for (int j = 0; j < 32; ++j) xq[j] = yb[(long)min(half + 2 * j, ol - 1) * C];
+  };
+  float uuL[2][16], xqL[32], muL, rsL;
+  lreq(0, uuL, xqL, muL, rsL);
+
+  if (head && tid < 128) {
+    const float g = a.scale * (h_de + h_dp * h_w);
+    sg[tid] = g;
+    a.hv[(long)b * 128 + tid] = g;
+    acc_add(&a.dcls_w[tid], h_dp * h_ff);
+    if (tid == 0) acc_add(a.dcls_b, h_dp);
+  }
+  __syncthreads();
+
+  const int nmt = (R + DR - 1) / DR;
+  for (int mt = 0; mt < nmt; ++mt) {
+    if (mt > 0) dreq(mt);
+    {
+      const int row = row1, part = part1;
+      const int rr = mt * DR + row;
+      const bool ok = rr < R;
+      const long r = row0 + rr;
+      float g[16], xh[16];
+      float s1 = 0.f, s2 = 0.f;
+      const float mu = mu1, rs = rs1;
+#pragma unroll
+      for (int q = 0; q < 4; ++q) {
+        float4 gz;
+        if (head) gz = *reinterpret_cast<const float4*>(&sg[part * 16 + q * 4]); else gz = gz4[q];
+        const float4 yv = yv4[q];
+        const float gg[4] = {gz.x, gz.y, gz.z, gz.w}, yy[4] = {yv.x, yv.y, yv.z, yv.w};
+#pragma unroll
+        for (int j = 0; j < 4; ++j) {
+          g[q * 4 + j] = gg[j];
+          xh[q * 4 + j] = (yy[j] - mu) * rs;
+          const float dxh = gg[j] * a.d_gamma[part * 16 + q * 4 + j];
+          s1 += dxh; s2 += dxh * xh[q * 4 + j];
+        }
+      }
+      s1 = group_sum<8>(s1); s2 = group_sum<8>(s2);
+      s1 *= (1.f / 128.f); s2 *= (1.f / 128.f);
+#pragma unroll
+      for (int q = 0; q < 4; ++q) {
+        float v[4];
+#pragma unroll
+        for (int j = 0; j < 4; ++j) {
+          const int c = part * 16 + q * 4 + j;
+          v[j] = rs * __builtin_fmaf(-xh[q * 4 + j], s2, __builtin_fmaf(g[q * 4 + j], a.d_gamma[c], -s1));
+        }
+        if (ok) *reinterpret_cast<float4*>(a.d_dy + r * 128 + part * 16 + q * 4) = make_float4(v[0], v[1], v[2], v[3]);
+        bf16x4 p; p[0] = to_bf16(v[0]); p[1] = to_bf16(v[1]); p[2] = to_bf16(v[2]); p[3] = to_bf16(v[3]);
+        *reinterpret_cast<bf16x4*>(&sdyD[row][part * 16 + q * 4]) = p;
+      }
+    }
+    __syncthreads();
+    {
+      f32x16 acc;
+#pragma unroll
+      for (int r = 0; r < 16; ++r) acc[r] = 0.f;
+#pragma unroll
+      for (int ks = 0; ks < 8; ++ks) {
+        const bf16x8 af = *reinterpret_cast<const bf16x8*>(&sdyD[lr][ks * 16 + 8 * lh]);
+        acc = __builtin_amdgcn_mfma_f32_32x32x16_bf16(af, bw2[ks], acc, 0, 0, 0);
+      }
+      act_dispatch(a.act, [&](auto AT) __attribute__((always_inline)) {
+#pragma unroll
+      for (int r = 0; r < 16; ++r) {
+        const int m = (r & 3) + 8 * (r >> 2) + 4 * lh;
+        const int rr = mt * DR + m;
+        float v = 0.f;
+        if (rr < R) {
+          v = acc[r] * act_grad_c<decltype(AT)::value>(a.act, uuD[r]);
+          a.d_du[(row0 + rr) * 128 + n] = v;
+        }
+        sduD[m][n] = to_bf16(v);
+      }
+      });
+    }
+    __syncthreads();
+    {
+      f32x16 acc;
+#pragma unroll
+      for (int r = 0; r < 16; ++r) acc[r] = 0.f;
+#pragma unroll
+      for (int ks = 0; ks < 8; ++ks) {
+        const bf16x8 a1 = *reinterpret_cast<const bf16x8*>(&sduD[lr][ks * 16 + 8 * lh]);
+        acc = __builtin_amdgcn_mfma_f32_32x32x16_bf16(a1, bw1[ks], acc, 0, 0, 0);
+        const bf16x8 a2 = *reinterpret_cast<const bf16x8*>(&sdyD[lr][ks * 16 + 8 * lh]);
+        acc = __builtin_amdgcn_mfma_f32_32x32x16_bf16(a2, bwr[ks], acc, 0, 0, 0);
+      }
+#pragma unroll
+      for (int r = 0; r < 16; ++r) {
+        const int rr = mt * DR + (r & 3) + 8 * (r >> 2) + 4 * lh;
+        if (rr < R) tile[rr][n] = acc[r];
+      }
+    }
+    __syncthreads();
+  }
+
+  {
+    const float* w1 = sw; const float* w2 = w1 + KM * KM + KM; const float* wr = w2 + KM * KM + KM;
+    const float* g = wr + KM * KM;
+    float aw1[NK][NK], aw2[NK][NK], awr[NK][NK], ab1[NK], ab2[NK], ag[NK], abe[NK];
+#pragma unroll
+    for (int i = 0; i < NK; ++i) {
+      ab1[i] = ab2[i] = ag[i] = abe[i] = 0.f;
+#pragma unroll
+      for (int j = 0; j < NK; ++j) aw1[i][j] = aw2[i][j] = awr[i][j] = 0.f;
+    }
+    act_dispatch(w.act, [&](auto AT) __attribute__((always_inline)) {
+    auto kstep = [&](int e, const float (&xin)[NK]) __attribute__((always_inline)) {
+      const int l = e >> 7, d = e & 127;
+      const long r = (long)b * ol + l;
+      KMixVals<NK> v;
+      float dzv[NK], dyv[NK], dym[NK], du[NK], dxn[NK], dxv[NK];
+#pragma unroll
+      for (int k = 0; k < NK; ++k) v.x[k] = k < w.ik ? xin[k] : 0.f;
+#pragma unroll
+      for (int o = 0; o < NK; ++o) {
+        const float gv = tile[l * w.ok + (o < w.ok ? o : w.ok - 1)][d];
+        dzv[o] = o < w.ok ? gv : 0.f;
+        v.sc[o] = o < w.ok ? 1.f : 0.f;
+      }
+      kmix_forward_vals<NK, decltype(AT)::value>(w, sw, v);
+      {
+        float out[NK];
+        ln_small<NK>(v.y, w.ok, g, g + KM, out, v.xh, v.mu, v.rs);
+        float s1 = 0.f, s2 = 0.f;
+#pragma unroll
+        for (int o = 0; o < NK; ++o) { const float t = dzv[o] * g[o]; s1 += t; s2 += t * v.xh[o]; }
+        s1 /= w.ok; s2 /= w.ok;
+#pragma unroll
+        for (int o = 0; o < NK; ++o) {
+          dyv[o] = o < w.ok ? v.rs * (dzv[o] * g[o] - s1 - v.xh[o] * s2) : 0.f;
+          ag[o] += dzv[o] * v.xh[o]; abe[o] += dzv[o];
+        }
+      }
+#pragma unroll
+      for (int o = 0; o < NK; ++o) dym[o] = dyv[o] * v.sc[o];
+#pragma unroll
+      for (int j = 0; j < NK; ++j) {
+        float s = 0.f;
+#pragma unroll
+        for (int o = 0; o < NK; ++o) s += w2[o * KM + j] * dym[o];
+        du[j] = j < w.hk ? s * act_grad_c<decltype(AT)::value>(w.act, v.u[j]) : 0.f;
+      }
+#pragma unroll
+      for (int k = 0; k < NK; ++k) {
+        float s = 0.f, rr = 0.f;
+#pragma unroll
+        for (int j = 0; j < NK; ++j) s += w1[j * KM + k] * du[j];
+#pragma unroll
+        for (int o = 0; o < NK; ++o) rr += wr[o * KM + k] * dyv[o];
+        dxn[k] = s; dxv[k] = rr;
+      }
+#pragma unroll
+      for (int k = 0; k < NK; ++k) dxv[k] += dxn[k];
+#pragma unroll
+      for (int k = 0; k < NK; ++k)
+        if (k < w.ik) {
+          tile[l * w.ik + k][d] = dxv[k];
+          a.k_dx[(r * w.ik + k) * 128 + d] = dxv[k];
+        }
+#pragma unroll
+      for (int o = 0; o < NK; ++o) {
+        ab2[o] += dym[o];
+#pragma unroll
+        for (int j = 0; j < NK; ++j) aw2[o][j] += dym[o] * v.h[j];
+#pragma unroll
+        for (int k = 0; k < NK; ++k) awr[o][k] += dyv[o] * v.x[k];
+      }
+#pragma unroll
+      for (int j = 0; j < NK; ++j) {
+        ab1[j] += du[j];
+#pragma unroll
+        for (int k = 0; k < NK; ++k) aw1[j][k] += du[j] * v.x[k];
+      }
+    };
+#pragma unroll
+    for (int j = 0; j < KPF; ++j) {
+      const int e = tid + 256 * j;
+      if (e < ktotal) kstep(e, xpre[j]);
+    }
+    for (int e = tid + 256 * KPF; e < ktotal; e += 256) {
+      const long r = (long)b * ol + (e >> 7); const int d = e & 127;
+      float xin[NK];
+#pragma unroll
+      for (int k = 0; k < NK; ++k) xin[k] = a.kx[(r * w.ik + (k < w.ik ? k : w.ik - 1)) * 128 + d];
+      kstep(e, xin);
+    }
+    });
+    LdsAcc* gw1 = sgk; LdsAcc* gb1 = gw1 + KM * KM; LdsAcc* gw2 = gb1 + KM; LdsAcc* gb2 = gw2 + KM * KM;
+    LdsAcc* gwr = gb2 + KM; LdsAcc* gg = gwr + KM * KM; LdsAcc* gbe = gg + KM;
+#pragma unroll
+    for (int i = 0; i < NK; ++i) {
+#pragma unroll
+      for (int j = 0; j < NK; ++j) {
+        float s = wave_sum(aw1[i][j]); if (lane == 0) gw1[i * KM + j].add(s);
+        s = wave_sum(aw2[i][j]); if (lane == 0) gw2[i * KM + j].add(s);
+        s = wave_sum(awr[i][j]); if (lane == 0) gwr[i * KM + j].add(s);
+      }
+      float s = wave_sum(ab1[i]); if (lane == 0) gb1[i].add(s);
+      s = wave_sum(ab2[i]); if (lane == 0) gb2[i].add(s);
+      s = wave_sum(ag[i]); if (lane == 0) gg[i].add(s);
+      s = wave_sum(abe[i]); if (lane == 0) gbe[i].add(s);
+    }
+    __syncthreads();
+    const int t = tid;
+    if (t < w.hk * w.ik) acc_add(&w.dw1[t], gw1[(t / w.ik) * KM + t % w.ik].get());
+    if (t < w.hk && w.db1) acc_add(&w.db1[t], gb1[t].get());
+    if (t < w.ok * w.hk) acc_add(&w.dw2[t], gw2[(t / w.hk) * KM + t % w.hk].get());
+    if (t < w.ok && w.db2) acc_add(&w.db2[t], gb2[t].get());
+    if (t < w.ok * w.ik && w.dwr) acc_add(&w.dwr[t], gwr[(t / w.ik) * KM + t % w.ik].get());
+    if (t < w.ok) { acc_add(&w.dg[t], gg[t].get()); acc_add(&w.dbe[t], gbe[t].get()); }
+  }
+
+  for (int kt = 0; kt < K; ++kt) {
+    const int c0 = kt * CT;
+    const float mu = muL, rs = rsL;
+    float* __restrict__ dyb = a.l_dy + (long)b * ol * C + c0 + col;
+    float gq[32], xq[32];
+    float s1 = 0.f, s2 = 0.f;
+#pragma unroll
+    for (int j = 0; j < 32; ++j) {
+      const int l = half + 2 * j;
+      gq[j] = tile[min(l, ol - 1) * K + kt][col];
+      xq[j] = (xqL[j] - mu) * rs;
+      gq[j] = l < ol ? gq[j] * sgam[min(l, 63)] : 0.f;
+      s1 += gq[j]; s2 += gq[j] * xq[j];
+    }
+    red[0][half][col] = s1;
+    red[1][half][col] = s2;
+    __syncthreads();
+    s1 = (red[0][0][col] + red[0][1][col]) / ol;
+    s2 = (red[1][0][col] + red[1][1][col]) / ol;
+#pragma unroll
+    for (int j = 0; j < 32; ++j) {
+      const int l = half + 2 * j;
+      if (l < ol) {
+        const float v = rs * (gq[j] - s1 - xq[j] * s2);
+        dyb[(long)l * C] = v;
+        sdy[col][l] = to_bf16(v);
+      }
+    }
+    for (int l = ol + ((half ^ ol) & 1); l < 64; l += 2) sdy[col][l] = to_bf16(0.f);
+    __syncthreads();
+
+    if (a.l_db2 && tid >= 192 && tid - 192 < ol) {
+      float t = 0.f;
+      for (int c = 0; c < CT; ++c) t += (float)sdy[(c + tid) & (CT - 1)][tid - 192];
+      acc_l2[tid - 192] = t;
+    }
+    const int nt = wave;
+    const int cc = c0 + nt * 32 + lr;
+    {
+      f32x16 acc0, acc1;
+#pragma unroll
+      for (int r = 0; r < 16; ++r) { acc0[r] = 0.f; acc1[r] = 0.f; }
+#pragma unroll
+      for (int ks = 0; ks < 4; ++ks) {
+        const bf16x8 bf = *reinterpret_cast<const bf16x8*>(&sdy[nt * 32 + lr][ks * 16 + 8 * lh]);
+        const bf16x8 a0 = *reinterpret_cast<const bf16x8*>(&wts[0][lr][ks * 16 + 8 * lh]);
+        acc0 = __builtin_amdgcn_mfma_f32_32x32x16_bf16(a0, bf, acc0, 0, 0, 0);
+        const bf16x8 a1 = *reinterpret_cast<const bf16x8*>(&wts[0][32 + lr][ks * 16 + 8 * lh]);
+        acc1 = __builtin_amdgcn_mfma_f32_32x32x16_bf16(a1, bf, acc1, 0, 0, 0);
+      }
+      act_dispatch(a.act, [&](auto AT) __attribute__((always_inline)) {
+#pragma unroll
+      for (int mt = 0; mt < 2; ++mt)
+#pragma unroll
+        for (int r = 0; r < 16; ++r) {
+          const int h = mt * 32 + (r & 3) + 8 * (r >> 2) + 4 * lh;
+          float v = 0.f;
+          if (h < hl) {
+            const long ui = ((long)b * hl + h) * C + cc;
+            v = (mt == 0 ? acc0[r] : acc1[r]) * act_grad_c<decltype(AT)::value>(a.act, uuL[mt][r]);
+            a.l_du[ui] = v;
+          }
+          sdu[nt * 32 + lr][h] = to_bf16(v);
+          if (a.l_db1) {
+            const float t = half_sum_hi(v);
+            if (lr == 16 && h < hl) acc_h[h].add(t);
+          }
+        }
+      });
+    }
+    __syncthreads();
+    lreq(min(kt + 1, K - 1), uuL, xqL, muL, rsL);
+    {
+      f32x16 acc0, acc1;
+#pragma unroll
+      for (int r = 0; r < 16; ++r) { acc0[r] = 0.f; acc1[r] = 0.f; }
+#pragma unroll
+      for (int ks = 0; ks < 8; ++ks) {
+        const bool first = ks < 4;
+        const int kk = (first ? ks : ks - 4) * 16 + 8 * lh;
+        const bf16x8 bf = *reinterpret_cast<const bf16x8*>(first ? &sdu[nt * 32 + lr][kk] : &sdy[nt * 32 + lr][kk]);
+        const bf16x8 a0 = *reinterpret_cast<const bf16x8*>(&wts[first ? 1 : 2][lr][kk]);
+        acc0 = __builtin_amdgcn_mfma_f32_32x32x16_bf16(a0, bf, acc0, 0, 0, 0);
+        const bf16x8 a1 = *reinterpret_cast<const bf16x8*>(&wts[first ? 1 : 2][32 + lr][kk]);
+        acc1 = __builtin_amdgcn_mfma_f32_32x32x16_bf16(a1, bf, acc1, 0, 0, 0);
+      }
+#pragma unroll
+      for (int mt = 0; mt < 2; ++mt)
+#pragma unroll
+        for (int r = 0; r < 16; ++r) {
+          const int i = mt * 32 + (r & 3) + 8 * (r >> 2) + 4 * lh;
+          if (i < il) a.l_dx[((long)b * il + i) * C + cc] = mt == 0 ? acc0[r] : acc1[r];
+        }
+    }
+    __syncthreads();
+    if (a.l_db2 && tid < ol) acc_add(&a.l_db2[tid], acc_l2[tid]);
+    if (a.l_db1 && tid >= 64 && tid - 64 < hl) { acc_add(&a.l_db1[tid - 64], acc_h[tid - 64].get()); acc_h[tid - 64].zero(); }
+  }
+}
+
+}
+
+bool cube_tail_bwd_supported(int il, int hl, int ol, int ik, int hk, int ok, int id, int hd, int od) {
+  return id == 128 && hd == 128 && od == 128 && ik == ok && hk == ok && ok >= 1 && ok <= 4 && ol >= 1 && il >= 1 && hl >= 1 &&
+         ol * ok <= 64 && il <= 64 && hl <= 64 && ol <= 64;
+}
+
+int cube_tail_bwd(hipStream_t s, const CubeTailBwdArgs& a) {
+  const KMixW& w = a.kw;
+  if (a.B < 1 || !cube_tail_bwd_supported(a.il, a.hl, a.ol, w.ik, w.hk, w.ok, 128, 128, 128) || a.K != w.ok)
+    return set_error(MIMRL_ERR_ARG, "cube_tail_bwd: unsupported shape");
+  if (w.ln_first || w.drop_p > 0.f || !w.wr || !a.l_wr) return set_error(MIMRL_ERR_ARG, "cube_tail_bwd: LayerNorm last, no dropout, residual projections");
+  if (!a.w2t || !a.w1t || !a.wrt) return set_error(MIMRL_ERR_ARG, "cube_tail_bwd: needs the transposed weight images");
+  if (!a.dz_ext && !(a.dpred && a.cls_w && a.feats && a.hv && a.dcls_w && a.dcls_b)) return set_error(MIMRL_ERR_ARG, "cube_tail_bwd: null head argument");
+  if (a.K == 3) hipLaunchKernelGGL((cube_tail_bwd_kernel<3, true>), dim3(a.B), dim3(256), 0, s, a);
+  else if (a.K < 3) hipLaunchKernelGGL((cube_tail_bwd_kernel<3, false>), dim3(a.B), dim3(256), 0, s, a);
+  else hipLaunchKernelGGL((cube_tail_bwd_kernel<4, false>), dim3(a.B), dim3(256), 0, s, a);
+  LAUNCH_CHECK();
+  return MIMRL_OK;
+}
+
+}
diff --git a/mimrl_amd/csrc/det.hip b/mimrl_amd/csrc/det.hip
--- a/mimrl_amd/csrc/det.hip
+++ b/mimrl_amd/csrc/det.hip
@@ -90,7 +90,7 @@
   if (t_defer) {
     static const char* const kBucketOnly[] = {"ln_relu_drop_bwd", "head_bwd_kernel", "colln_bwd_kernel", "rowln_bwd_kernel", "kmix_bwd_kernel",
                                               "colsum_kernel", "rowsum_batched", "colln_param_grads", "daxis_param_grads",
-                                              "laxis_bwd_kernel", "daxis_bwd_kernel", "gru_bwd_kernel", "top1_bwd_kernel", "concat_dw3_kernel",
+                                              "laxis_bwd_kernel", "daxis_bwd_kernel", "cube_tail_bwd_kernel", "gru_bwd_kernel", "top1_bwd_kernel", "concat_dw3_kernel",
                                               "mlp_frag_kernel", "gemm_group_kernel", "gemm_groupk_kernel"};
     for (const char* k : kBucketOnly)
       if (std::strstr(name, k)) { t_pending = true; return false; }
diff --git a/mimrl_amd/csrc/engine.h b/mimrl_amd/csrc/engine.h
--- a/mimrl_amd/csrc/engine.h
+++ b/mimrl_amd/csrc/engine.h
@@ -16,6 +16,7 @@
 #include "gru.h"
 #include "gru_wgrad.h"
 #include "concat_dw.h"
+#include "cube_tail_bwd.h"
 #include "lstm.h"
 #include "layout.h"
 #include "comm.h"
@@ -234,6 +235,7 @@
   size_t ev_next = 0;
   bool multi_stream = true;
   bool fused_cube_bwd = true;
+  bool fused_cube_tail_bwd = true;
   bool fused_mlp = true;
   bool fused_cube = true;
   int fwd_f16 = 1;
@@ -410,7 +412,8 @@
   int dbg_delay(hipStream_t st, int tag);
   int model_forward(bool train, bool save, int knn_stage = 0, int part = 0);
   int cube_forward(bool train, bool save);
-  int cube_backward(int cur_in, int* cur_out);
+  bool cube_tail_fusable() const;
+  int cube_backward(int cur_in, int* cur_out, bool head_in_tail = false);
   int wt_images(hipStream_t st, bool bwd_bf16, bool launch, bool* d_fused);
   int model_backward();
   int encoders_backward(float* dcube);
diff --git a/mimrl_amd/csrc/engine_abi.hip b/mimrl_amd/csrc/engine_abi.hip
--- a/mimrl_amd/csrc/engine_abi.hip
+++ b/mimrl_amd/csrc/engine_abi.hip
@@ -61,7 +61,9 @@
   h->fold_unpack_on = knob("MIMRL_NO_FOLD_UNPACK") == nullptr;
   h->h16_on = knob("MIMRL_NO_H16") == nullptr;
   h->xin_on = knob("MIMRL_NO_XIN") == nullptr;
-  h->fused_cube_bwd = knob("MIMRL_NO_FUSED_CUBE_BWD") == nullptr;
+  const bool tail_only = knob("MIMRL_NO_FUSED_CUBE_BWD") && std::strcmp(knob("MIMRL_NO_FUSED_CUBE_BWD"), "tail") == 0;
+  h->fused_cube_bwd = knob("MIMRL_NO_FUSED_CUBE_BWD") == nullptr || tail_only;
+  h->fused_cube_tail_bwd = knob("MIMRL_NO_FUSED_CUBE_BWD") == nullptr;
   h->laxis_bwd_long_on = !(knob("MIMRL_LAXIS_BWD_LONG") && atoi(knob("MIMRL_LAXIS_BWD_LONG")) == 0);
   h->laxis_long_on = !(knob("MIMRL_LAXIS_LONG") && atoi(knob("MIMRL_LAXIS_LONG")) == 0);
   h->rec16_on = !(knob("MIMRL_REC16") && atoi(knob("MIMRL_REC16")) == 0);
@@ -640,6 +642,61 @@
   return concat_dw(reinterpret_cast<hipStream_t>(stream), a);
 }
 
+int mimrl_op_cube_tail_bwd(void* stream, int chain, const int32_t* dims, const float* const* in, float* const* out, float* scratch) {
+  if (!dims || !in || !out || !scratch) return set_error(MIMRL_ERR_ARG, "mimrl_op_cube_tail_bwd: null argument");
+  hipStream_t st = reinterpret_cast<hipStream_t>(stream);
+  const int B = dims[0], il = dims[1], hl = dims[2], ol = dims[3], K = dims[4], act = dims[5], sum_l = dims[6], sum_k = dims[7];
+  if (B < 1 || !cube_tail_bwd_supported(il, hl, ol, K, K, K, 128, 128, 128)) return set_error(MIMRL_ERR_ARG, "mimrl_op_cube_tail_bwd: unsupported shape");
+  for (int i = 5; i <= 28; ++i) if (!in[i] && i != 15 && i != 17) return set_error(MIMRL_ERR_ARG, "mimrl_op_cube_tail_bwd: null input %d", i);
+  for (int i = 0; i <= 14; ++i) if (!out[i] && i != 9 && i != 11 && !(in[0] && (i == 6 || i == 7))) return set_error(MIMRL_ERR_ARG, "mimrl_op_cube_tail_bwd: null output %d", i);
+  if (!in[0] && !(in[1] && in[2] && in[3])) return set_error(MIMRL_ERR_ARG, "mimrl_op_cube_tail_bwd: head mode needs dpred, cls_w and feats");
+  const long R2 = (long)B * ol * K;
+  __bf16* wt = reinterpret_cast<__bf16*>(scratch);
+  float* hv = scratch + 3 * 128 * 128 / 2;
+  float* ddx = hv + R2 * 128;
+  WtTransposeArgs ta;
+  std::memset(&ta, 0, sizeof ta);
+  for (int q = 0; q < 3; ++q) { ta.src[q] = in[10 + q]; ta.dst[q] = wt + (size_t)q * 128 * 128; }
+  ta.n = 3;
+  MX(wt_transpose_bf16(st, ta));
+  KMixW kw;
+  std::memset(&kw, 0, sizeof kw);
+  kw.w1 = in[14]; kw.b1 = in[15]; kw.w2 = in[16]; kw.b2 = in[17]; kw.wr = in[18]; kw.g = in[19]; kw.be = in[20];
+  kw.dw1 = out[8]; kw.db1 = in[15] ? out[9] : nullptr; kw.dw2 = out[10]; kw.db2 = in[17] ? out[11] : nullptr; kw.dwr = out[12]; kw.dg = out[13]; kw.dbe = out[14];
+  kw.ik = K; kw.hk = K; kw.ok = K; kw.act = act;
+  if (!chain) {
+    CubeTailBwdArgs a;
+    std::memset(&a, 0, sizeof a);
+    a.dz_ext = in[0]; a.dpred = in[1]; a.cls_w = in[2]; a.feats = in[3]; a.dff_ext = in[4];
+    a.scale = (sum_l ? 1.f : 1.f / ol) * (sum_k ? 1.f : 1.f / K);
+    a.hv = hv; a.dcls_w = out[6]; a.dcls_b = out[7];
+    a.d_y = in[5]; a.d_mean = in[6]; a.d_rstd = in[7]; a.d_gamma = in[8]; a.d_u = in[9];
+    a.w2t = wt; a.w1t = wt + 128 * 128; a.wrt = wt + 2 * 128 * 128;
+    a.d_dy = out[0]; a.d_du = out[1];
+    a.kx = in[13]; a.kw = kw; a.k_dx = out[2];
+    a.l_y = in[21]; a.l_mean = in[22]; a.l_rstd = in[23]; a.l_gamma = in[24]; a.l_u = in[25]; a.l_w2 = in[26]; a.l_w1 = in[27]; a.l_wr = in[28];
+    a.l_dy = out[3]; a.l_du = out[4]; a.l_dx = out[5]; a.l_db2 = out[15]; a.l_db1 = out[16];
+    a.B = B; a.il = il; a.hl = hl; a.ol = ol; a.K = K; a.act = act;
+    return cube_tail_bwd(st, a);
+  }
+  const float* dz = in[0];
+  if (!dz) { MX(head_bwd(st, in[4], in[1], in[2], in[3], hv, out[6], out[7], B, ol, K, 128, sum_l, sum_k, nullptr)); dz = hv; }
+  DAxisBwdArgs fa;
+  std::memset(&fa, 0, sizeof fa);
+  fa.dz = dz; fa.y = in[5]; fa.mean = in[6]; fa.rstd = in[7]; fa.gamma = in[8]; fa.u = in[9];
+  fa.w2t = wt; fa.w1t = wt + 128 * 128; fa.wrt = wt + 2 * 128 * 128;
+  fa.dy = out[0]; fa.du = out[1]; fa.dx = ddx; fa.R = R2; fa.act = act;
+  MX(daxis_bwd_fused(st, fa));
+  MX(kmix_bwd(st, in[13], ddx, out[2], kw, (long)B * ol, 128));
+  LAxisBwdArgs la;
+  std::memset(&la, 0, sizeof la);
+  la.dz = out[2]; la.y = in[21]; la.mean = in[22]; la.rstd = in[23]; la.gamma = in[24]; la.u = in[25];
+  la.w2 = in[26]; la.w1 = in[27]; la.wr = in[28];
+  la.dy = out[3]; la.du = out[4]; la.dx = out[5]; la.db2 = out[15]; la.db1 = out[16];
+  la.B = B; la.il = il; la.hl = hl; la.ol = ol; la.C = K * 128; la.act = act;
+  return laxis_bwd_fused(st, la);
+}
+
 int mimrl_op_gru_wgrad(void* stream, const void* const* dg, const void* const* x, const void* const* hp, float* const* dw_ih,
                        float* const* dw_hh, int64_t rows, int kp) {
   if (!dg || !x || !hp || !dw_ih || !dw_hh) return set_error(MIMRL_ERR_ARG, "mimrl_op_gru_wgrad: null argument");
diff --git a/mimrl_amd/csrc/engine_backward.hip b/mimrl_amd/csrc/engine_backward.hip
--- a/mimrl_amd/csrc/engine_backward.hip
+++ b/mimrl_amd/csrc/engine_backward.hip
@@ -1,6 +1,16 @@
 #include "engine.h"
 
-int mimrl_handle::cube_backward(int cur_in, int* cur_out) {
+bool mimrl_handle::cube_tail_fusable() const {
+  const int i = cfg.n_blocks - 1;
+  if (i < 0 || !bf16 || !fused_cube_bwd || !fused_cube_tail_bwd || cfg.ln_first) return false;
+  if (cfg.dropout_mlp[0] > 0.f || cfg.dropout_mlp[1] > 0.f || cfg.dropout_mlp[2] > 0.f) return false;
+  const BlockW& w = blk[i];
+  if (w.ax[0].res < 0 || w.ax[1].res < 0 || w.ax[2].res < 0 || !wtT[i][0]) return false;
+  const int il = i == 0 ? cfg.time_len : cfg.d_outs[i - 1][0], ik = i == 0 ? 3 : cfg.d_outs[i - 1][1], id = i == 0 ? cfg.d_common : cfg.d_outs[i - 1][2];
+  return cube_tail_bwd_supported(il, w.ax[0].hid, w.ax[0].out, ik, w.ax[1].hid, w.ax[1].out, id, w.ax[2].hid, w.ax[2].out);
+}
+
+int mimrl_handle::cube_backward(int cur_in, int* cur_out, bool head_in_tail) {
   const int B = cfg.batch;
   int dims[MIMRL_MAX_BLOCKS + 1][3];
   dims[0][0] = cfg.time_len; dims[0][1] = 3; dims[0][2] = cfg.d_common;
@@ -8,7 +18,7 @@
     for (int ax = 0; ax < 3; ++ax) dims[i + 1][ax] = cfg.d_outs[i][ax];
   const int per_block = 7 + (cfg.dropout_mlp[0] > 0.f) + (cfg.dropout_mlp[2] > 0.f);
   const bool defer = multi_stream && !cfg.ln_first && per_block * cfg.n_blocks + 1 <= NGBUF;
-  const int npool = defer ? NGBUF : 4;
+  const int npool = defer ? NGBUF : 8;
   int used[NGBUF] = {0};
   used[cur_in] = 1;
   int cur = cur_in;
@@ -37,14 +47,14 @@
     return colln_param_grads(S(sd), y, mean, rstd, dz, dgam, dbet, nb, n, cols);
   };
   auto W_dpg = [&](int sd, const float* y, const float* mean, const float* rstd, const float* dz, const float* dy, const float* du,
-                   float* dgam, float* dbet, float* db2, float* db1, long rows) -> int {
+                   float* dgam, float* dbet, float* db2, float* db1, long rows, long bc = 0) -> int {
     if (defer) {
-      Deferred d{6, sd, GemmDesc(), y, rows, 0, 0, 0, dgam};
+      Deferred d{6, sd, GemmDesc(), y, rows, bc, 0, 0, dgam};
       d.p1 = mean; d.p2 = rstd; d.p3 = dz; d.p4 = dy; d.p5 = du; d.dst2 = dbet; d.dst3 = db2; d.dst4 = db1;
       deferred.push_back(d);
       return MIMRL_OK;
     }
-    return daxis_param_grads(S(sd), y, mean, rstd, dz, dy, du, dgam, dbet, db2, db1, rows);
+    return daxis_param_grads(S(sd), y, mean, rstd, dz, dy, du, dgam, dbet, db2, db1, rows, bc);
   };
   auto W_fork = [&](int lo, int hi) -> int { return defer ? MIMRL_OK : fork(lo, hi); };
   bool d_fused[MIMRL_MAX_BLOCKS] = {};
@@ -61,6 +71,67 @@
     const int hl = w.ax[0].hid, ol = w.ax[0].out, hk = w.ax[1].hid, ok = w.ax[1].out, hd = w.ax[2].hid, od = w.ax[2].out;
     const float* xblk = i == 0 ? cube0 : bb[i - 1].d.z;
     const float pl = cfg.dropout_mlp[0], pk = cfg.dropout_mlp[1], pd = cfg.dropout_mlp[2];
+    const bool tail = i == cfg.n_blocks - 1 && d_fused[i] && cube_tail_fusable();
+    if (head_in_tail && i == cfg.n_blocks - 1 && !tail) return set_error(MIMRL_ERR_STATE, "cube_backward: the head's gradient was left to a tail kernel that does not run");
+    if (tail) {
+      const AxisW &ad = w.ax[2], &ak = w.ax[1], &al = w.ax[0];
+      const long R2 = (long)B * ol * ok, C = (long)ik * id;
+      GRAB(d_dy); GRAB(d_du); GRAB(k_dx); GRAB(l_dy); GRAB(l_du); GRAB(l_dx);
+      CubeTailBwdArgs ta;
+      std::memset(&ta, 0, sizeof ta);
+      if (head_in_tail) {
+        ta.dpred = dpred; ta.cls_w = P(cls_w); ta.feats = bufs.feats; ta.dff_ext = dfeat;
+        if (head_gather_on) { ta.gs = head_gather; ta.use_gs = 1; }
+        ta.scale = (cfg.compose_t_sum ? 1.f : 1.f / ol) * (cfg.compose_k_sum ? 1.f : 1.f / ok);
+        ta.hv = gbuf[cur]; ta.dcls_w = Gm(cls_w); ta.dcls_b = Gm(cls_b);
+      } else {
+        ta.dz_ext = gbuf[cur];
+      }
+      ta.d_y = b.d.y; ta.d_mean = b.d.mean; ta.d_rstd = b.d.rstd; ta.d_gamma = P(ad.ln_g); ta.d_u = b.d.u;
+      ta.w2t = wtT[i][0]; ta.w1t = wtT[i][1]; ta.wrt = wtT[i][2];
+      ta.d_dy = gbuf[d_dy]; ta.d_du = gbuf[d_du];
+      ta.kx = b.l.z;
+      KMixW& kw = ta.kw;
+      kw.w1 = P(ak.fc1.w); kw.b1 = ak.fc1.b >= 0 ? P(ak.fc1.b) : nullptr;
+      kw.w2 = P(ak.fc2.w); kw.b2 = ak.fc2.b >= 0 ? P(ak.fc2.b) : nullptr;
+      kw.wr = P(ak.res); kw.g = P(ak.ln_g); kw.be = P(ak.ln_b);
+      kw.dw1 = Gm(ak.fc1.w); kw.db1 = ak.fc1.b >= 0 ? Gm(ak.fc1.b) : nullptr;
+      kw.dw2 = Gm(ak.fc2.w); kw.db2 = ak.fc2.b >= 0 ? Gm(ak.fc2.b) : nullptr;
+      kw.dwr = Gm(ak.res); kw.dg = Gm(ak.ln_g); kw.dbe = Gm(ak.ln_b);
+      kw.ik = ik; kw.hk = hk; kw.ok = ok; kw.act = cfg.activation; kw.ln_first = 0; kw.drop_p = 0.f; kw.key = key(); kw.stream_id = 11 + 3 * i;
+      ta.k_dx = gbuf[k_dx];
+      ta.l_y = b.l.y; ta.l_mean = b.l.mean; ta.l_rstd = b.l.rstd; ta.l_gamma = P(al.ln_g); ta.l_u = b.l.u;
+      ta.l_w2 = P(al.fc2.w); ta.l_w1 = P(al.fc1.w); ta.l_wr = P(al.res);
+      ta.l_dy = gbuf[l_dy]; ta.l_du = gbuf[l_du]; ta.l_dx = gbuf[l_dx];
+      ta.l_db2 = al.fc2.b >= 0 ? Gm(al.fc2.b) : nullptr; ta.l_db1 = al.fc1.b >= 0 ? Gm(al.fc1.b) : nullptr;
+      ta.B = B; ta.il = il; ta.hl = hl; ta.ol = ol; ta.K = ok; ta.act = cfg.activation;
+      MX(cube_tail_bwd(stream, ta));
+      MX(W_fork(1, 3));
+      MX(W_dpg(2, b.d.y, b.d.mean, b.d.rstd, gbuf[cur], gbuf[d_dy], gbuf[d_du], Gm(ad.ln_g), Gm(ad.ln_b),
+               ad.fc2.b >= 0 ? Gm(ad.fc2.b) : nullptr, ad.fc1.b >= 0 ? Gm(ad.fc1.b) : nullptr, R2, head_in_tail ? (long)ol * ok : 0));
+      { GemmDesc g = gemm_tn(gbuf[d_dy], od, b.d.h, hd, Gm(ad.fc2.w), hd, od, hd, (int)R2); g.atomic = 1; MX(W_gemm(1, g)); }
+      { GemmDesc g = gemm_tn(gbuf[d_dy], od, b.k.z, id, Gm(ad.res), id, od, id, (int)R2); g.atomic = 1; MX(W_gemm(2, g)); }
+      { GemmDesc g = gemm_tn(gbuf[d_du], hd, b.k.z, id, Gm(ad.fc1.w), id, hd, id, (int)R2); g.atomic = 1; MX(W_gemm(3, g)); }
+      MX(W_lnpar(1, b.l.y, b.l.mean, b.l.rstd, gbuf[k_dx], Gm(al.ln_g), Gm(al.ln_b), B, ol, (int)C));
+      { GemmDesc g; g.A = gbuf[l_dy]; g.sa_m = C; g.sa_k = 1; g.sa_b = (long)ol * C;
+        g.B = b.l.h; g.sb_k = 1; g.sb_n = C; g.sb_b = (long)hl * C;
+        g.C = Gm(al.fc2.w); g.sc_m = hl; g.sc_n = 1; g.sc_b = 0; g.M = ol; g.N = hl; g.K = (int)C; g.batch = B; g.atomic = 1;
+        MX(W_gemm(1, g)); }
+      { GemmDesc g; g.A = gbuf[l_dy]; g.sa_m = C; g.sa_k = 1; g.sa_b = (long)ol * C;
+        g.B = xblk; g.sb_k = 1; g.sb_n = C; g.sb_b = (long)il * C;
+        g.C = Gm(al.res); g.sc_m = il; g.sc_n = 1; g.sc_b = 0; g.M = ol; g.N = il; g.K = (int)C; g.batch = B; g.atomic = 1;
+        MX(W_gemm(2, g)); }
+      { GemmDesc g; g.A = gbuf[l_du]; g.sa_m = C; g.sa_k = 1; g.sa_b = (long)hl * C;
+        g.B = xblk; g.sb_k = 1; g.sb_n = C; g.sb_b = (long)il * C;
+        g.C = Gm(al.fc1.w); g.sc_m = il; g.sc_n = 1; g.sc_b = 0; g.M = hl; g.N = il; g.K = (int)C; g.batch = B; g.atomic = 1;
+        MX(W_gemm(3, g)); }
+      MX(W_join(1, 3));
+      release(cur); release(d_dy); release(d_du); release(k_dx); release(l_dy); release(l_du);
+      cur = l_dx;
+      static const int early_tail = dbg_env("MIMRL_EARLY_FLUSH") ? atoi(dbg_env("MIMRL_EARLY_FLUSH")) : 2;
+      if (defer && early_tail >= 1) MX(flush_deferred(1));
+      continue;
+    }
     if (d_fused[i]) {
       const AxisW& a = w.ax[2];
       const long R2 = (long)B * ol * ok;
@@ -325,7 +396,7 @@
     else if (d.kind == 1) MX(colsum(st, d.src, d.n0, (int)d.n1, (int)d.n2, d.dst));
     else if (d.kind == 2) MX(rowsum_batched(st, d.src, (int)d.n0, (int)d.n1, (int)d.n2, d.dst));
     else if (d.kind == 3) MX(colln_param_grads(st, d.src, d.p1, d.p2, d.p3, d.dst, d.dst2, (int)d.n0, (int)d.n1, (int)d.n2));
-    else if (d.kind == 6) MX(daxis_param_grads(st, d.src, d.p1, d.p2, d.p3, d.p4, d.p5, d.dst, d.dst2, d.dst3, d.dst4, d.n0));
+    else if (d.kind == 6) MX(daxis_param_grads(st, d.src, d.p1, d.p2, d.p3, d.p4, d.p5, d.dst, d.dst2, d.dst3, d.dst4, d.n0, d.n1));
     else MX(kmix_bwd_part(st, d.src, d.p3, nullptr, d.kw, d.n0, (int)d.n1, 2));
   }
   deferred.clear();
@@ -339,11 +410,13 @@
   const long BT_ = (long)B * T;
   const int nb = cfg.n_blocks;
   const int ol = cfg.d_outs[nb - 1][0], ok = cfg.d_outs[nb - 1][1], od = cfg.d_outs[nb - 1][2];
-  MX(head_bwd(stream, dfeat, dpred, P(cls_w), bufs.feats, gbuf[0], Gm(cls_w), Gm(cls_b), B, ol, ok, od,
-              cfg.compose_t_sum, cfg.compose_k_sum, head_gather_on ? &head_gather : nullptr));
+  const bool head_in_tail = cube_tail_fusable() && od == 128;
+  if (!head_in_tail)
+    MX(head_bwd(stream, dfeat, dpred, P(cls_w), bufs.feats, gbuf[0], Gm(cls_w), Gm(cls_b), B, ol, ok, od,
+                cfg.compose_t_sum, cfg.compose_k_sum, head_gather_on ? &head_gather : nullptr));
   int ci = 0;
   deferred.clear();
-  { Scope sc(this, MIMRL_PH_CUBE_BWD); MX(cube_backward(0, &ci)); }
+  { Scope sc(this, MIMRL_PH_CUBE_BWD); MX(cube_backward(0, &ci, head_in_tail)); }
   MX(dbg_delay(stream, 7));
   return encoders_backward(gbuf[ci]);
 }
diff --git a/mimrl_amd/csrc/knobs.cpp b/mimrl_amd/csrc/knobs.cpp
--- a/mimrl_amd/csrc/knobs.cpp
+++ b/mimrl_amd/csrc/knobs.cpp
@@ -36,7 +36,7 @@
   {"MIMRL_NO_FOLD_UNPACK", "engine_abi.hip", "", "packed layer-0 weight gradients through l0_unpack instead of the Adam fold"},
   {"MIMRL_NO_FUSED_CONCAT", "engine_abi.hip", "", "concat critic tail as a GEMM chain instead of concat_fwd / concat_bwd"},
   {"MIMRL_NO_FUSED_CUBE", "engine_abi.hip", "", "bf16 mode: CubeMLP forward as the unfused GEMM / LayerNorm chain"},
-  {"MIMRL_NO_FUSED_CUBE_BWD", "engine_abi.hip", "", "bf16 mode: CubeMLP backward as the unfused chain"},
+  {"MIMRL_NO_FUSED_CUBE_BWD", "engine_abi.hip", "", "bf16 mode: CubeMLP backward as the unfused chain; =tail: only the one-launch backward of the head and the last block (cube_tail_bwd.hip) is off, the per-axis fused kernels stay"},
   {"MIMRL_NO_FUSED_MI", "engine_estimators.hip", "", "separable critic: scores / bound / gradients as separate kernels instead of mi_sep_fused / mi_sep_nce"},
   {"MIMRL_NO_FUSED_MLP", "engine_abi.hip", "", "bf16 mode: estimator MLP stacks as grouped GEMMs"},
   {"MIMRL_NO_FUSED_MLP_BWD", "engine_estimators.hip", "", "estimator MLP stacks: data-gradient chain as GEMMs instead of the fused kernel"},
```
